# abmoRobotics/isaac_rover_orbit

Measured on NVIDIA B200. Metric: height_scan_rays_per_s, higher is better.
Workload: dtype f32

## Files before the change

include/rover_b200.h:

```cpp
#ifndef ROVER_B200_H
#define ROVER_B200_H

#include <stdint.h>

#ifdef __cplusplus
extern "C" {
#endif

#define ROVER_B200_ABI_VERSION 5
#define ROVER_MAX_LEVELS 12
#define ROVER_NUM_REWARD_TERMS 7
#define ROVER_NUM_TERMINATION_TERMS 4
#define ROVER_STATS_LEN 16

int rover_abi_version(void);
const char* rover_last_error(void);

typedef struct RoverScanLevel {
    float ox, oy;
    float cell;
    float inv_cell;
    int32_t ncx, ncy;
    int32_t start_offset;
    int32_t reserved;
} RoverScanLevel;

typedef struct RoverScanGrid {
    int32_t n_levels;
    int32_t span;
    RoverScanLevel level[ROVER_MAX_LEVELS];
    const int32_t* cell_start;
    const float* records;
    int32_t n_records;
    int32_t reserved;
} RoverScanGrid;

typedef struct RoverPlaneCells {
    const float* xs;
    const float* ys;
    const float* entries;
    int32_t nx, ny;
    float inv_dx, inv_dy;
    const float* entries_planar;
} RoverPlaneCells;

int rover_height_scan(const float* pos_w, const float* quat_w, int32_t n_envs, const float* ray_starts_local,
                      int32_t n_rays, const float* pattern_box , const RoverScanGrid* grid ,
                      const RoverPlaneCells* cells , float max_distance, float base_offset,
                      float* out_heights, int32_t out_stride, float* out_hits_w, int32_t variant, void* stream);

int rover_ray_cast(const float* pos_w, const float* quat_w, int32_t n_envs, const float* ray_starts_local,
                   const float* ray_dirs_local, int32_t n_rays, int32_t attach_yaw_only, const RoverScanGrid* grid ,
                   const RoverPlaneCells* cells , float max_distance, float base_offset, float* out_heights,
                   int32_t out_stride, float* out_hits_w, void* stream);

int64_t rover_height_scan_host_work_bytes(int32_t n_envs, int32_t out_stride);
int rover_height_scan_host(const float* pos_host, const float* quat_host, int32_t n_envs, const float* ray_starts_local,
                           int32_t n_rays, const float* pattern_box, const RoverScanGrid* grid, const RoverPlaneCells* cells,
                           float max_distance, float base_offset, float* out_host, int32_t out_stride, void* work,
                           int64_t work_bytes, int32_t n_slices, int32_t variant, void* stream);
int rover_height_scan_obs(const float* pos_w, const float* quat_w, int32_t n_envs, const float* ray_starts_local,
                          int32_t n_rays, const float* pattern_box , const RoverScanGrid* grid ,
                          const RoverPlaneCells* cells , float max_distance, float base_offset, float* obs,
                          int32_t obs_stride, int32_t head_cols, uint16_t* obs_bf16, int32_t bf16_stride, void* stream);
int rover_height_scan_obs_bf16(const float* pos_w, const float* quat_w, int32_t n_envs, const float* ray_starts_local,
                               int32_t n_rays, const float* pattern_box , const RoverScanGrid* grid,
                               const RoverPlaneCells* cells, float max_distance, float base_offset, const float* obs_head,
                               int32_t obs_stride, int32_t head_cols, uint16_t* obs_bf16, int32_t bf16_stride, void* stream);

int rover_ray_cast_obs(const float* pos_w, const float* quat_w, int32_t n_envs, const float* ray_starts_local,
                       const float* ray_dirs_local, int32_t n_rays, int32_t attach_yaw_only, const RoverScanGrid* grid ,
                       const RoverPlaneCells* cells , float max_distance, float base_offset, float* obs,
                       int32_t obs_stride, int32_t head_cols, uint16_t* obs_bf16, int32_t bf16_stride, void* stream);
int rover_ray_cast_obs_bf16(const float* pos_w, const float* quat_w, int32_t n_envs, const float* ray_starts_local,
                            const float* ray_dirs_local, int32_t n_rays, int32_t attach_yaw_only,
                            const RoverScanGrid* grid , const RoverPlaneCells* cells , float max_distance,
                            float base_offset, const float* obs_head, int32_t obs_stride, int32_t head_cols,
                            uint16_t* obs_bf16, int32_t bf16_stride, void* stream);
int rover_ray_cast_host(const float* pos_host, const float* quat_host, int32_t n_envs, const float* ray_starts_local,
                        const float* ray_dirs_local, int32_t n_rays, int32_t attach_yaw_only, const RoverScanGrid* grid,
                        const RoverPlaneCells* cells, float max_distance, float base_offset, float* out_host,
                        int32_t out_stride, void* work, int64_t work_bytes, int32_t n_slices, void* stream);

typedef struct RoverMdpParams {
    float scale_lin, scale_ang, offset_lin, offset_ang;
    float wheelbase_length, middle_wheel_distance, rear_and_front_wheel_distance, wheel_radius;
    float min_radius;
    float wheel_diameter;
    float weight[ROVER_NUM_REWARD_TERMS];
    float reached_threshold, far_threshold;
    float step_dt;
    int32_t max_episode_length;
    float obs_distance_scale, obs_heading_scale;
    float target_distance, resampling_time, heading_lo, heading_hi, spawn_z_offset;
    int32_t num_bodies;
    int32_t action_variant;
    float episode_length_s;
} RoverMdpParams;

typedef struct RoverMdpState {
    float* action;
    float* prev_action;
    float* pos_cmd_w;
    float* heading_cmd_w;
    float* pos_cmd_b;
    float* heading_cmd_b;
    float* time_left;
    int64_t* command_counter;
    int64_t* episode_length_buf;
    float* episode_sums;
    float* env_origins;
    float* err_pos;
    float* err_heading;
} RoverMdpState;

typedef struct RoverMdpOut {
    float* processed_actions;
    float* joint_pos;
    float* joint_vel;
    float* reward;
    float* term_rewards;
    float* term_values;
    uint8_t* terminated;
    uint8_t* truncated;
    uint8_t* term_flags;
    uint8_t* reset_flags;
    int32_t* block_reset_counts;
} RoverMdpOut;

#define ROVER_MDP_BLOCK 64

#define ROVER_PRE_ACTIONS 1
#define ROVER_PRE_TERMS 2
#define ROVER_PRE_ALL 3
int rover_mdp_pre_step(const float* new_actions, const float* force_matrix_w, int32_t n_envs,
                       const RoverMdpParams* params , const RoverMdpState* state ,
                       const RoverMdpOut* out , int32_t phases, void* stream);

int rover_ackermann(const float* actions , int32_t n_envs, const RoverMdpParams* params ,
                    float* processed , float* joint_pos , float* joint_vel ,
                    void* stream);

typedef struct RoverTerrainTables {
    const float* heightmap;
    const uint8_t* safe_mask;
    int32_t height, width;
    float offset_x, offset_y;
    float resolution;
    const float* spawn_table;
    int32_t n_spawns;
    int32_t reserved;
} RoverTerrainTables;

#define ROVER_PHASE_SPAWN 1
#define ROVER_PHASE_MANAGERS 2
#define ROVER_PHASE_RESAMPLE 4
#define ROVER_PHASE_METRICS 8
#define ROVER_PHASE_TIME 16
#define ROVER_PHASE_COMMAND 32
#define ROVER_PHASE_OBS 64
#define ROVER_PHASE_ALL 127

int rover_mdp_post_step(float* root_pos_w, float* root_quat_w, int32_t n_envs, const RoverMdpParams* params,
                        const RoverMdpState* state, const RoverMdpOut* out, const RoverTerrainTables* tables,
                        const int64_t* spawn_perm, const float* yaw_u, const float* heading_u, const float* theta_u,
                        int32_t n_rounds, int64_t* out_spawn_index , float* stats,
                        float* scratch ,
                        float* obs, int32_t obs_stride, int32_t phases, void* stream);

typedef struct RoverResetVariates {
    const int64_t* spawn_perm;
    const float* yaw_u;
    const float* heading_u;
    const float* theta_u;
    int32_t n_rounds;
    int32_t reserved;
    uint64_t* rng_state;
} RoverResetVariates;

int rover_mdp_post_step_v3(float* root_pos_w, float* root_quat_w, int32_t n_envs, const RoverMdpParams* params,
                           const RoverMdpState* state, const RoverMdpOut* out, const RoverTerrainTables* tables,
                           const RoverResetVariates* variates , int64_t* out_spawn_index, float* stats,
                           float* scratch, float* log_out, float* obs, int32_t obs_stride, int32_t phases,
                           const struct RoverStatsExchange* xchg , void* stream);
int rover_rng_variates(uint64_t seed, uint64_t step, int32_t n_envs, int32_t n_rounds, int32_t n_spawns,
                       int64_t* spawn_by_env, float* yaw_u, float* heading_u, float* theta_u);
int rover_philox4x32_10(const uint32_t counter[4], const uint32_t key[2], uint32_t out[4]);

int rover_mdp_step(const float* new_actions, const float* force_matrix_w, float* root_pos_w, float* root_quat_w,
                   int32_t n_envs, const RoverMdpParams* params, const RoverMdpState* state, const RoverMdpOut* out,
                   const RoverTerrainTables* tables, const int64_t* spawn_perm, const float* yaw_u, const float* heading_u,
                   const float* theta_u, int32_t n_rounds, int64_t* out_spawn_index, float* stats, float* scratch,
                   uint64_t* lookback, float* obs, int32_t obs_stride, int32_t pre_phases, int32_t phases,
                   const struct RoverStatsExchange* xchg , void* stream);
int rover_mdp_step_v3(const float* new_actions, const float* force_matrix_w, float* root_pos_w, float* root_quat_w,
                      int32_t n_envs, const RoverMdpParams* params, const RoverMdpState* state, const RoverMdpOut* out,
// ... 86 lines not shown
```

isaac_rover_orbit_b200/_lib.py:

```python
from __future__ import annotations

import ctypes as C
import os

import torch

_HERE = os.path.dirname(os.path.abspath(__file__))
LIB_PATH = os.environ.get("ROVER_B200_LIB") or os.path.join(_HERE, "librover_b200.so")

MAX_LEVELS = 12
NUM_REWARD_TERMS = 7
NUM_TERMINATION_TERMS = 4
STATS_LEN = 16
MDP_BLOCK = 64
ABI_VERSION = 5

SYMBOLS = ("rover_abi_version", "rover_last_error", "rover_height_scan", "rover_height_scan_obs", "rover_mdp_pre_step",
           "rover_mdp_post_step", "rover_mdp_post_step_x", "rover_mdp_post_step_v3", "rover_mdp_step", "rover_mdp_step_v3",
           "rover_rng_variates", "rover_philox4x32_10", "rover_stats_read", "rover_p2p_alloc", "rover_p2p_free",
           "rover_p2p_export", "rover_p2p_open", "rover_p2p_close",
           "rover_ackermann",
           "rover_height_scan_host", "rover_height_scan_host_work_bytes", "rover_stats_publish", "rover_height_scan_obs_bf16", "rover_policy_pack", "rover_policy_forward", "rover_value_forward", "rover_policy_value_forward", "rover_policy_forward_bf16",
           "rover_value_forward_bf16", "rover_gaussian_act", "rover_mesh_to_heightmap", "rover_steep_mask",
           "rover_policy_pack_fused", "rover_scan_encoder_fused", "rover_policy_mlp_forward", "rover_morph_box",
           "rover_fill_holes", "rover_step_fused", "rover_ray_cast", "rover_ray_cast_obs", "rover_ray_cast_obs_bf16",
           "rover_ray_cast_host", "rover_ppo_gae", "rover_ppo_gae_work_bytes")


class ScanLevel(C.Structure):
    _fields_ = [("ox", C.c_float), ("oy", C.c_float), ("cell", C.c_float), ("inv_cell", C.c_float),
                ("ncx", C.c_int32), ("ncy", C.c_int32), ("start_offset", C.c_int32), ("reserved", C.c_int32)]


class ScanGrid(C.Structure):
    _fields_ = [("n_levels", C.c_int32), ("span", C.c_int32), ("level", ScanLevel * MAX_LEVELS),
                ("cell_start", C.c_void_p), ("records", C.c_void_p), ("n_records", C.c_int32),
                ("reserved", C.c_int32)]


class PlaneCells(C.Structure):
    _fields_ = [("xs", C.c_void_p), ("ys", C.c_void_p), ("entries", C.c_void_p), ("nx", C.c_int32), ("ny", C.c_int32),
                ("inv_dx", C.c_float), ("inv_dy", C.c_float), ("entries_planar", C.c_void_p)]


class StatsExchange(C.Structure):
    _fields_ = [("peer_mailbox", C.c_void_p), ("cumulative", C.c_void_p), ("sequence", C.c_void_p),
                ("rank", C.c_int32), ("world", C.c_int32)]


MAILBOX_SLOT_BYTES = 512


class MdpParams(C.Structure):
    _fields_ = [("scale_lin", C.c_float), ("scale_ang", C.c_float), ("offset_lin", C.c_float),
                ("offset_ang", C.c_float), ("wheelbase_length", C.c_float), ("middle_wheel_distance", C.c_float),
                ("rear_and_front_wheel_distance", C.c_float), ("wheel_radius", C.c_float), ("min_radius", C.c_float),
                ("wheel_diameter", C.c_float),
                ("weight", C.c_float * NUM_REWARD_TERMS), ("reached_threshold", C.c_float),
                ("far_threshold", C.c_float), ("step_dt", C.c_float), ("max_episode_length", C.c_int32),
                ("obs_distance_scale", C.c_float), ("obs_heading_scale", C.c_float), ("target_distance", C.c_float),
                ("resampling_time", C.c_float), ("heading_lo", C.c_float), ("heading_hi", C.c_float),
                ("spawn_z_offset", C.c_float), ("num_bodies", C.c_int32), ("action_variant", C.c_int32),
                ("episode_length_s", C.c_float)]


class ResetVariates(C.Structure):

    _fields_ = [("spawn_perm", C.c_void_p), ("yaw_u", C.c_void_p), ("heading_u", C.c_void_p), ("theta_u", C.c_void_p),
                ("n_rounds", C.c_int32), ("reserved", C.c_int32), ("rng_state", C.c_void_p)]


_STATE_FIELDS = ("action", "prev_action", "pos_cmd_w", "heading_cmd_w", "pos_cmd_b", "heading_cmd_b", "time_left",
                 "command_counter", "episode_length_buf", "episode_sums", "env_origins", "err_pos", "err_heading")
_OUT_FIELDS = ("processed_actions", "joint_pos", "joint_vel", "reward", "term_rewards", "term_values", "terminated",
               "truncated", "term_flags", "reset_flags", "block_reset_counts")

PHASE_SPAWN, PHASE_MANAGERS, PHASE_RESAMPLE, PHASE_METRICS, PHASE_TIME, PHASE_COMMAND, PHASE_OBS = 1, 2, 4, 8, 16, 32, 64
PHASE_ALL = 127
PRE_ACTIONS, PRE_TERMS, PRE_ALL = 1, 2, 3


class MdpState(C.Structure):
    _fields_ = [(n, C.c_void_p) for n in _STATE_FIELDS]


class MdpOut(C.Structure):
    _fields_ = [(n, C.c_void_p) for n in _OUT_FIELDS]


class TerrainTables(C.Structure):
    _fields_ = [("heightmap", C.c_void_p), ("safe_mask", C.c_void_p), ("height", C.c_int32), ("width", C.c_int32),
                ("offset_x", C.c_float), ("offset_y", C.c_float), ("resolution", C.c_float),
                ("spawn_table", C.c_void_p), ("n_spawns", C.c_int32), ("reserved", C.c_int32)]


class PolicyWeights(C.Structure):
    _fields_ = [("w", C.c_void_p * 6), ("b", C.c_void_p * 6), ("in_dim", C.c_int32 * 6), ("out_dim", C.c_int32 * 6)]


_lib = None


def load() -> C.CDLL:
    global _lib
    if _lib is not None:
        return _lib
    if not os.path.exists(LIB_PATH):
        raise RuntimeError(
            f"{LIB_PATH} is missing: run `python __graft_entry__.py` (nvcc, sm_100a). There is no CPU fallback.")
    lib = C.CDLL(LIB_PATH)
    missing = [s for s in SYMBOLS if not hasattr(lib, s)]
    if missing:
        raise RuntimeError(f"librover_b200.so does not export {missing}")
    lib.rover_abi_version.restype = C.c_int
    lib.rover_last_error.restype = C.c_char_p
    if lib.rover_abi_version() != ABI_VERSION:
        raise RuntimeError(f"librover_b200.so ABI {lib.rover_abi_version()} != expected {ABI_VERSION}")
    vp, i32, f32 = C.c_void_p, C.c_int32, C.c_float
    lib.rover_height_scan.restype = C.c_int
    lib.rover_height_scan.argtypes = [vp, vp, i32, vp, i32, C.POINTER(C.c_float * 4), C.POINTER(ScanGrid),
                                      C.POINTER(PlaneCells), f32, f32, vp, i32, vp, i32, vp]
    lib.rover_ray_cast.restype = C.c_int
    lib.rover_ray_cast.argtypes = [vp, vp, i32, vp, vp, i32, i32, C.POINTER(ScanGrid), C.POINTER(PlaneCells), f32, f32, vp,
                                   i32, vp, vp]
    for fn in (lib.rover_ray_cast_obs, lib.rover_ray_cast_obs_bf16):
        fn.restype = C.c_int
        fn.argtypes = [vp, vp, i32, vp, vp, i32, i32, C.POINTER(ScanGrid), C.POINTER(PlaneCells), f32, f32, vp, i32, i32, vp,
                       i32, vp]
    lib.rover_ray_cast_host.restype = C.c_int
    lib.rover_ray_cast_host.argtypes = [vp, vp, i32, vp, vp, i32, i32, C.POINTER(ScanGrid), C.POINTER(PlaneCells), f32, f32,
                                        vp, i32, vp, C.c_int64, i32, vp]
    lib.rover_mdp_pre_step.restype = C.c_int
    lib.rover_mdp_pre_step.argtypes = [vp, vp, i32, C.POINTER(MdpParams), C.POINTER(MdpState), C.POINTER(MdpOut), i32,
                                       vp]
    lib.rover_mdp_post_step.restype = C.c_int
    lib.rover_mdp_post_step.argtypes = [vp, vp, i32, C.POINTER(MdpParams), C.POINTER(MdpState), C.POINTER(MdpOut),
                                        C.POINTER(TerrainTables), vp, vp, vp, vp, i32, vp, vp, vp, vp, i32, i32, vp]
    lib.rover_mdp_post_step_x.restype = C.c_int
    lib.rover_mdp_post_step_x.argtypes = [vp, vp, i32, C.POINTER(MdpParams), C.POINTER(MdpState), C.POINTER(MdpOut),
                                          C.POINTER(TerrainTables), vp, vp, vp, vp, i32, vp, vp, vp, vp, i32, i32,
                                          C.POINTER(StatsExchange), vp]
    lib.rover_mdp_post_step_v3.restype = C.c_int
    lib.rover_mdp_post_step_v3.argtypes = [vp, vp, i32, C.POINTER(MdpParams), C.POINTER(MdpState), C.POINTER(MdpOut),
                                           C.POINTER(TerrainTables), C.POINTER(ResetVariates), vp, vp, vp, vp, vp, i32, i32,
                                           C.POINTER(StatsExchange), vp]
    lib.rover_mdp_step_v3.restype = C.c_int
    lib.rover_mdp_step_v3.argtypes = [vp, vp, vp, vp, i32, C.POINTER(MdpParams), C.POINTER(MdpState), C.POINTER(MdpOut),
                                      C.POINTER(TerrainTables), C.POINTER(ResetVariates), vp, vp, vp, vp, vp, vp, i32, i32,
                                      i32, C.POINTER(StatsExchange), vp]
    lib.rover_step_fused.restype = C.c_int
    lib.rover_step_fused.argtypes = [vp, vp, vp, vp, i32, C.POINTER(MdpParams), C.POINTER(MdpState), C.POINTER(MdpOut),
                                     C.POINTER(TerrainTables), vp, i32, vp, vp, vp, i32, vp, vp, i32, i32, i32,
                                     C.POINTER(StatsExchange), vp, i32, C.POINTER(C.c_float * 4), C.POINTER(ScanGrid),
                                     C.POINTER(PlaneCells), f32, f32, vp]
    lib.rover_rng_variates.restype = C.c_int
    lib.rover_rng_variates.argtypes = [C.c_uint64, C.c_uint64, i32, i32, i32, vp, vp, vp, vp]
    lib.rover_philox4x32_10.restype = C.c_int
    lib.rover_philox4x32_10.argtypes = [C.POINTER(C.c_uint32 * 4), C.POINTER(C.c_uint32 * 2), C.POINTER(C.c_uint32 * 4)]
    lib.rover_mdp_step.restype = C.c_int
    lib.rover_mdp_step.argtypes = [vp, vp, vp, vp, i32, C.POINTER(MdpParams), C.POINTER(MdpState), C.POINTER(MdpOut),
                                   C.POINTER(TerrainTables), vp, vp, vp, vp, i32, vp, vp, vp, vp, vp, i32, i32, i32,
                                   C.POINTER(StatsExchange), vp]
    lib.rover_mesh_to_heightmap.restype = C.c_int
    lib.rover_mesh_to_heightmap.argtypes = [vp, vp, i32, C.c_float, C.c_float, C.c_float, C.c_float, i32, i32, vp, vp, vp]
    lib.rover_steep_mask.restype = C.c_int
    lib.rover_steep_mask.argtypes = [vp, i32, i32, C.c_double, vp, vp]
    lib.rover_morph_box.restype = C.c_int
    lib.rover_morph_box.argtypes = [vp, i32, i32, i32, i32, vp, vp, vp]
    lib.rover_fill_holes.restype = C.c_int
    lib.rover_fill_holes.argtypes = [vp, i32, i32, vp, vp, vp, vp]
    lib.rover_stats_read.restype = C.c_int
    lib.rover_stats_read.argtypes = [vp, i32, vp, vp]
    lib.rover_p2p_alloc.restype = C.c_int
    lib.rover_p2p_alloc.argtypes = [C.POINTER(C.c_void_p), C.c_int64]
    lib.rover_p2p_export.restype = C.c_int
    lib.rover_p2p_export.argtypes = [vp, C.POINTER(C.c_uint8 * 64)]
    lib.rover_p2p_open.restype = C.c_int
    lib.rover_p2p_open.argtypes = [C.POINTER(C.c_uint8 * 64), C.POINTER(C.c_void_p)]
    for fn in (lib.rover_p2p_free, lib.rover_p2p_close):
        fn.restype = C.c_int
        fn.argtypes = [vp]
    lib.rover_ackermann.restype = C.c_int
    lib.rover_ackermann.argtypes = [vp, i32, C.POINTER(MdpParams), vp, vp, vp, vp]
    lib.rover_policy_pack.restype = C.c_int64
    lib.rover_policy_pack.argtypes = [C.POINTER(PolicyWeights), vp, vp]
    lib.rover_stats_publish.restype = C.c_int
    lib.rover_stats_publish.argtypes = [C.POINTER(StatsExchange), vp]
    lib.rover_height_scan_host_work_bytes.restype = C.c_int64
    lib.rover_height_scan_host_work_bytes.argtypes = [i32, i32]
    lib.rover_height_scan_host.restype = C.c_int
    lib.rover_height_scan_host.argtypes = [vp, vp, i32, vp, i32, C.POINTER(C.c_float * 4), C.POINTER(ScanGrid),
                                           C.POINTER(PlaneCells), f32, f32, vp, i32, vp, C.c_int64, i32, i32, vp]
    for fn in (lib.rover_height_scan_obs, lib.rover_height_scan_obs_bf16):
        fn.restype = C.c_int
        fn.argtypes = [vp, vp, i32, vp, i32, C.POINTER(C.c_float * 4), C.POINTER(ScanGrid), C.POINTER(PlaneCells), f32, f32, vp,
# ... 67 lines not shown
```

isaac_rover_orbit_b200/csrc/fused_scan_policy.cu:

```cuda
#include "policy_common.cuh"
#include "scan_paired.cuh"

namespace rover {

constexpr int kFuConsumerWarps = 12;
constexpr int kFuWarps = 20;
constexpr int kFuThreads = 32 * kFuWarps;
constexpr int kFuStages = 4, kFuFullBars = 8;
constexpr int kFuBatch = 16;
constexpr int kFuRays = 961, kFuChunks = 4;
constexpr int kFuK0 = 976;
constexpr int kFuObsBytes = (kFuK0 / 8) * kOperandLbo;
constexpr int kFuActBytes = (80 / 8) * kOperandLbo;
constexpr int kFuW0Cols = kFuK0 / 2;
constexpr int kFuAccCol = kFuW0Cols;
constexpr int kFuTmemCols = 512;
constexpr int kFuEncCols = 64;
constexpr int kFuBiasFloats = 80 + 64;
constexpr int kFuW0Bytes = kFuW0Cols * 128 * 4;
constexpr int kFuW1Bytes = 10 * 64 * 16, kFuW1Lbo = 64 * 16, kFuW1Slack = 1024;
constexpr int kFuW1Ofs = kFuW0Bytes, kFuBiasOfs = kFuW0Bytes + kFuW1Bytes;
constexpr int kFuPackedBytes = kFuBiasOfs + kFuBiasFloats * 4;
constexpr int kFuRegsLaunch = 96, kFuRegsConsumer = 120, kFuRegsUtil = 64, kFuRegsEpilogue = 56;
static_assert(128 * (3 * kFuRegsConsumer + kFuRegsUtil + kFuRegsEpilogue) <= kFuThreads * kFuRegsLaunch,
              "setmaxnreg: the re-balanced budgets must fit the pool the CTA was launched with");
static_assert(kFuFullBars == 2 * kFuStages && 8 * kFuChunks - kFuConsumerWarps > 4 * kFuChunks, "phase aliasing argument");

struct FuPackArgs {
    const float* w0;
    const float* b0;
    const float* w1;
    const float* b1;
    int in0, in1;
};

__global__ void fused_pack_kernel(const __grid_constant__ FuPackArgs a, unsigned char* __restrict__ packed) {
    const int tid = blockIdx.x * blockDim.x + threadIdx.x, nthr = gridDim.x * blockDim.x;
    uint32_t* w0t = reinterpret_cast<uint32_t*>(packed);
    for (int idx = tid; idx < kFuW0Cols * 128; idx += nthr) {
        const int j = idx >> 7, t = idx & 127;
        float v[2] = {0.f, 0.f};
#pragma unroll
        for (int h = 0; h < 2; ++h) {
            const int src_k = 2 * j + h - kEncInOffset;
            if (t < 80 && src_k >= 0 && src_k < kEncIn) v[h] = a.w0[(size_t)t * a.in0 + src_k];
        }
        w0t[idx] = pack_bf16(v[0], v[1]);
    }
    __nv_bfloat16* w1 = reinterpret_cast<__nv_bfloat16*>(packed + kFuW1Ofs);
    for (int idx = tid; idx < kFuW1Bytes / 2; idx += nthr) {
        const int jj = idx & 7, r = (idx >> 3) & 63, plane = idx >> 9;
        const int k = plane * 8 + jj;
        w1[idx] = __float2bfloat16_rn((r < 60 && k < 80) ? a.w1[(size_t)r * a.in1 + k] : 0.f);
    }
    float* bias = reinterpret_cast<float*>(packed + kFuBiasOfs);
    for (int n = tid; n < kFuBiasFloats; n += nthr) bias[n] = n < 80 ? a.b0[n] : (n - 80 < 60 ? a.b1[n - 80] : 0.f);
}

struct __align__(128) FuSmem {
    PairStage stage[kFuStages];
    float vx[kPairMaxRays], vy[kPairMaxRays];
    LinePair2 xpair[kPairMaxLines], ypair[kPairMaxLines];
    unsigned char obs[2][kFuObsBytes];
    unsigned char act[kFuActBytes];
    unsigned char w1[kFuW1Bytes + kFuW1Slack];
    float bias[kFuBiasFloats];
    unsigned long long full_bar[kFuFullBars], empty_bar[kFuStages];
    unsigned long long obs_full[2], obs_empty[2];
    unsigned long long w1_full, w0_ready, acc_full, act_ready, batch_done;
    uint32_t tmem_base;
    int next_chunk;
    float vz0;
    __nv_bfloat16 head[kFuBatch][4];
};
static_assert(sizeof(FuSmem) <= 227 * 1024, "FuSmem exceeds the shared memory of one SM");
__device__ __forceinline__ float sm_vz(const FuSmem& sm, int) { return sm.vz0; }

__device__ __forceinline__ void fu_arrive(unsigned long long* b) {
    asm volatile("mbarrier.arrive.shared::cta.b64 _, [%0];" ::"r"(sptr(b)) : "memory");
}
__device__ __forceinline__ void fu_epi_sync() { asm volatile("bar.sync 1, 128;" ::: "memory"); }
__device__ __forceinline__ void fu_wait_relaxed(unsigned long long* bar, uint32_t parity) {
    uint32_t done = 0;
    while (true) {
        asm volatile(
            "{\n\t.reg .pred p;\n\tmbarrier.try_wait.parity.shared::cta.b64 p, [%1], %2;\n\tselp.u32 %0, 1, 0, p;\n\t}"
            : "=r"(done)
            : "r"(sptr(bar)), "r"(parity)
            : "memory");
        if (done) break;
        __nanosleep(256);
    }
}
__device__ __forceinline__ void fu_tmem_ld16(uint32_t taddr, uint32_t (&r)[16]) {
    asm volatile(
        "tcgen05.ld.sync.aligned.32x32b.x16.b32 {%0, %1, %2, %3, %4, %5, %6, %7, %8, %9, %10, %11, %12, %13, %14, %15}, [%16];"
        : "=r"(r[0]), "=r"(r[1]), "=r"(r[2]), "=r"(r[3]), "=r"(r[4]), "=r"(r[5]), "=r"(r[6]), "=r"(r[7]), "=r"(r[8]),
          "=r"(r[9]), "=r"(r[10]), "=r"(r[11]), "=r"(r[12]), "=r"(r[13]), "=r"(r[14]), "=r"(r[15])
        : "r"(taddr));
    asm volatile("tcgen05.wait::ld.sync.aligned;" ::: "memory");
}
__device__ __forceinline__ void fu_tmem_st8(uint32_t taddr, const uint32_t (&r)[8]) {
    asm volatile("tcgen05.st.sync.aligned.32x32b.x8.b32 [%0], {%1, %2, %3, %4, %5, %6, %7, %8};" ::"r"(taddr), "r"(r[0]),
                 "r"(r[1]), "r"(r[2]), "r"(r[3]), "r"(r[4]), "r"(r[5]), "r"(r[6]), "r"(r[7])
                 : "memory");
}
__device__ __forceinline__ void umma_ts(uint32_t d_tmem, uint32_t a_tmem, uint64_t bdesc, uint32_t idesc, bool accumulate) {
    asm volatile(
        "{\n\t.reg .pred p;\n\tsetp.ne.b32 p, %4, 0;\n\t"
        "tcgen05.mma.cta_group::1.kind::f16 [%0], [%1], %2, %3, p;\n\t}" ::"r"(d_tmem),
        "r"(a_tmem), "l"(bdesc), "r"(idesc), "r"((uint32_t)accumulate)
        : "memory");
}
template <int kRegs>
__device__ __forceinline__ void reg_dec() {
    asm volatile("setmaxnreg.dec.sync.aligned.u32 %0;" ::"n"(kRegs));
}
template <int kRegs>
__device__ __forceinline__ void reg_inc() {
    asm volatile("setmaxnreg.inc.sync.aligned.u32 %0;" ::"n"(kRegs));
}
__device__ __forceinline__ unsigned char* operand_at(unsigned char* base, int e, int k) {
    return base + (k >> 3) * kOperandLbo + (e >> 3) * 128 + (e & 7) * 16 + (k & 7) * 2;
}

template <bool kWriteObs>
__global__ void __launch_bounds__(kFuThreads, 1)
fused_scan_encoder_kernel(const float* __restrict__ pos_w, const float* __restrict__ quat_w, int n_envs,
                          const float* __restrict__ ray_local, const __grid_constant__ ScanGridDev g,
                          const __grid_constant__ PlaneCellsDev pc, const __grid_constant__ CUtensorMap tmap,
                          float pattern_radius, float max_d, float base_offset, float* __restrict__ obs, int obs_stride,
                          const unsigned char* __restrict__ packed, __nv_bfloat16* __restrict__ enc) {
    extern __shared__ __align__(128) unsigned char smem_raw[];
    FuSmem& sm = *reinterpret_cast<FuSmem*>(smem_raw);
    const int warp = threadIdx.x >> 5, lane = threadIdx.x & 31;
    const int n_iter = (n_envs - (int)blockIdx.x + (int)gridDim.x - 1) / (int)gridDim.x;
    const int n_batches = (n_iter + kFuBatch - 1) / kFuBatch;
    const bool lines_in_smem = (pc.nx <= kPairMaxLines) && (pc.ny <= kPairMaxLines);
    constexpr int n_rays = kFuRays;

    ProducerEnv cur, nxt;
    if (warp == 0) {
        producer_load(cur, lane, n_iter, pos_w, quat_w);
        if (lane == 0) {
            asm volatile("prefetch.tensormap [%0];" ::"l"(reinterpret_cast<uint64_t>(&tmap)) : "memory");
            for (int s = 0; s < kFuFullBars; ++s) bar_init(&sm.full_bar[s], 2);
            for (int s = 0; s < kFuStages; ++s) bar_init(&sm.empty_bar[s], (uint32_t)kFuChunks);
            asm volatile("fence.mbarrier_init.release.cluster;" ::: "memory");
        }
        __syncwarp();
        producer_window(cur, pc, pattern_radius);
        if (lane < n_iter && lane < kFuStages) {
            bar_arrive_expect_tx(&sm.full_bar[lane], kPairStageBytes);
            tma_load_window_planar(sm.stage[lane].p, &tmap, cur.ic0, cur.jr0, &sm.full_bar[lane]);
        }
        producer_frame(cur);
    } else if (warp == 1) {
        if (lane == 0) {
            for (int i = 0; i < 2; ++i) {
                mb_init(&sm.obs_full[i], kFuBatch * kFuChunks);
                mb_init(&sm.obs_empty[i], 1);
            }
            mb_init(&sm.w1_full, 1);
            mb_init(&sm.w0_ready, 1);
            mb_init(&sm.acc_full, 1);
            mb_init(&sm.act_ready, 1);
            mb_init(&sm.batch_done, 1);
            sm.next_chunk = 0;
            sm.vz0 = __ldg(ray_local + 2);
            asm volatile("fence.mbarrier_init.release.cluster;" ::: "memory");
            mb_expect_tx(&sm.w1_full, kFuW1Bytes);
            bulk_g2s(sm.w1, packed + kFuW1Ofs, kFuW1Bytes, &sm.w1_full);
        }
        __syncwarp();
        asm volatile("tcgen05.alloc.cta_group::1.sync.aligned.shared::cta.b32 [%0], %1;" ::"r"(sptr(&sm.tmem_base)),
                     "r"((uint32_t)kFuTmemCols)
                     : "memory");
        asm volatile("tcgen05.relinquish_alloc_permit.cta_group::1.sync.aligned;" ::: "memory");
    } else if (warp >= 4) {
        constexpr int kFill = 32 * (kFuWarps - 4);
        constexpr int kPatLoads = (2 * kPairMaxRays + kFill - 1) / kFill;
        constexpr int kLineLoads = (kPairMaxLines + kFill - 1) / kFill;
        const int ct = threadIdx.x - 128;
        float* pat_flat = sm.vx;
        float pat[kPatLoads], xl[kLineLoads], xh[kLineLoads], yl[kLineLoads], yh[kLineLoads];
#pragma unroll
        for (int k = 0; k < kPatLoads; ++k) {
            const int i = ct + k * kFill;
            const int comp = i / kPairMaxRays, r = ray_of_slot(i - comp * kPairMaxRays);
            pat[k] = (i < 2 * kPairMaxRays && r < n_rays) ? __ldg(ray_local + 3 * r + comp) : 0.f;
        }
#pragma unroll
        for (int k = 0; k < kLineLoads; ++k) {
            const int i = ct + k * kFill;
            const bool okx = lines_in_smem && i < pc.nx, oky = lines_in_smem && i < pc.ny;
            xl[k] = okx ? __ldg(pc.xs + i) : 0.f;
            xh[k] = okx ? __ldg(pc.xs + i + 1) : 0.f;
            yl[k] = oky ? __ldg(pc.ys + i) : 0.f;
            yh[k] = oky ? __ldg(pc.ys + i + 1) : 0.f;
        }
#pragma unroll
        for (int k = 0; k < kPatLoads; ++k) {
            const int i = ct + k * kFill;
            if (i < 2 * kPairMaxRays) pat_flat[i] = pat[k];
        }
#pragma unroll
        for (int k = 0; k < kLineLoads; ++k) {
            const int i = ct + k * kFill;
            if (lines_in_smem && i < pc.nx) sm.xpair[i] = {xl[k], xh[k]};
            if (lines_in_smem && i < pc.ny) sm.ypair[i] = {yl[k], yh[k]};
        }
        uint4* z = reinterpret_cast<uint4*>(&sm.obs[0][0]);
        for (int i = ct; i < 2 * kFuObsBytes / 16; i += kFill) z[i] = make_uint4(0u, 0u, 0u, 0u);
        for (int i = ct; i < kFuBiasFloats; i += kFill)
            sm.bias[i] = __ldg(reinterpret_cast<const float*>(packed + kFuBiasOfs) + i);
        fence_async_smem();
    }
    tc_fence_before();
    __syncthreads();
    tc_fence_after();
    const uint32_t tmem = sm.tmem_base;

    if (warp < 4) {
        reg_dec<kFuRegsUtil>();
        if (warp == 0) {
            for (int base = 0; base < n_iter; base += 32) {
                if (base > 0) cur = nxt;
                producer_verdict(cur, sm, pc, pattern_radius, lines_in_smem);
                const int n_here = min(32, n_iter - base);
                for (int k = 0; k < n_here; ++k) {
                    if (k == kFuStages && base + 32 < n_iter) {
                        producer_load(nxt, base + 32 + lane, n_iter, pos_w, quat_w);
                        producer_window(nxt, pc, pattern_radius);
                        producer_frame(nxt);
                    }
                    if (lane == k) {
                        const int it = base + k;
                        const int s = it % kFuStages;
                        unsigned long long* full = &sm.full_bar[it % kFuFullBars];
                        PairStage& st = sm.stage[s];
                        if (it >= kFuStages) {
                            bar_wait(&sm.empty_bar[s], ((uint32_t)(it / kFuStages) & 1u) ^ 1u);
                            if (cur.ok) {
                                bar_arrive_expect_tx(full, kPairStageBytes);
                                tma_load_window_planar(st.p, &tmap, cur.ic0, cur.jr0, full);
                            } else {
                                bar_arrive(full);
                            }
                        }
                        st.hdr = {cur.cw, cur.sz, cur.px, cur.py, cur.pz, cur.ic0, cur.jr0, cur.ncols, cur.nrows,
                                  cur.ok ? 1 : 0, 0, 0};
                        bar_arrive(full);
                    }
                    __syncwarp();
                }
            }
        } else if (warp == 2 && lane == 0) {
            const uint32_t idesc = make_idesc(kFuBatch);
            const uint32_t acc = tmem + kFuAccCol;
            fu_wait_relaxed(&sm.w1_full, 0u);
            fu_wait_relaxed(&sm.w0_ready, 0u);
            tc_fence_after();
            for (int b = 0; b < n_batches; ++b) {
                const int buf = b & 1;
                if (b == n_batches - 1) {
                    const int missing = (n_batches * kFuBatch - n_iter) * kFuChunks;
                    for (int i = 0; i < missing; ++i) fu_arrive(&sm.obs_full[buf]);
                }
                if (b > 0) fu_wait_relaxed(&sm.batch_done, (uint32_t)(b - 1) & 1u);
                fu_wait_relaxed(&sm.obs_full[buf], (uint32_t)(b >> 1) & 1u);
                tc_fence_after();
                const uint32_t b0 = sptr(sm.obs[buf]);
                for (int ks = 0; ks < kFuK0 / 16; ++ks)
                    umma_ts(acc, tmem + ks * 8, make_desc(b0 + ks * 2 * kOperandLbo, kOperandLbo), idesc, ks != 0);
                umma_commit(&sm.acc_full);
                fu_wait_relaxed(&sm.act_ready, (uint32_t)b & 1u);
                tc_fence_after();
                const uint32_t a1 = sptr(sm.w1), b1 = sptr(sm.act);
                for (int j = 0; j < 80 / 16; ++j)
                    umma(acc, make_desc(a1 + j * 2 * kFuW1Lbo, kFuW1Lbo), make_desc(b1 + j * 2 * kOperandLbo, kOperandLbo), idesc,
                         j != 0);
                umma_commit(&sm.acc_full);
            }
        }
    } else if (warp < 4 + kFuConsumerWarps) {
        reg_inc<kFuRegsConsumer>();
        while (true) {
            int chunk_id = 0;
            if (lane == 0) chunk_id = atomicAdd(&sm.next_chunk, 1);
            chunk_id = __shfl_sync(0xffffffffu, chunk_id, 0);
            const int it = chunk_id / kFuChunks, c = chunk_id - it * kFuChunks;
            if (it >= n_iter) break;
            const int env = (int)blockIdx.x + it * (int)gridDim.x;
            const int s = it % kFuStages;
            const PairStage& st = sm.stage[s];
            const int batch = it / kFuBatch, slot = it - batch * kFuBatch, buf = batch & 1;
            if (batch >= 2) bar_wait(&sm.obs_empty[buf], (uint32_t)((batch >> 1) - 1) & 1u);
            bar_wait(&sm.full_bar[it % kFuFullBars], (uint32_t)(it / kFuFullBars) & 1u);
            const PairHeader h = st.hdr;
            float* __restrict__ obs_row = obs + (size_t)env * obs_stride;
            float* __restrict__ out_row = obs_row + kOperandHead;
            unsigned char* __restrict__ operand_row = sm.obs[buf] + (slot >> 3) * 128 + (slot & 7) * 16;
            const int r_begin = c * kPairChunk, r_end = min(r_begin + kPairChunk, n_rays);
            if (c == 0 && lane < kOperandHead)
                *reinterpret_cast<__nv_bfloat16*>(operand_row + lane * 2) = __float2bfloat16_rn(obs_row[lane]);
            if (h.mode == 1) {
                const float sz2 = __fmul_rn(h.sz, 2.f);
                const PairCtx cx = make_pair_ctx(h, sm, st, smem_raw, pc.inv_dx, pc.inv_dy, base_offset, max_d, sm.vz0,
                                                 n_envs >> 31);
                constexpr int kSink = kWriteObs ? kSinkOperandAndGlobal : kSinkOperand;
                for (int b0 = r_begin; b0 < r_end; b0 += kPairBatch) {
                    const int r = b0 + lane;
                    float* __restrict__ o = out_row + r;
                    unsigned defer;
                    if (b0 + kPairBatch <= n_rays) {
                        defer = resolve_pair<true, true, false, kSink>(smem_raw, sm, cx, b0 + 2 * lane, r, n_rays, o, nullptr,
                                                                       operand_row);
                        defer |= resolve_pair<true, true, false, kSink>(smem_raw, sm, cx, b0 + 64 + 2 * lane, r + 32, n_rays,
                                                                        o + 32, nullptr, operand_row) << 2;
                    } else {
                        defer = resolve_pair<false, true, false, kSink>(smem_raw, sm, cx, b0 + 2 * lane, r, n_rays, o, nullptr,
                                                                        operand_row);
                        defer |= resolve_pair<false, true, false, kSink>(smem_raw, sm, cx, b0 + 64 + 2 * lane, r + 32, n_rays,
                                                                         o + 32, nullptr, operand_row) << 2;
                    }
                    if (defer != 0u) {
                        for (int u = 0; u < 4; ++u) {
                            if (!((defer >> u) & 1u)) continue;
                            const int rr = r + (u >> 1) * 32 + (u & 1) * 64;
                            const int sl = b0 + (u >> 1) * 64 + 2 * lane + (u & 1);
                            const float vx = sm.vx[sl], vy = sm.vy[sl];
                            const float tx = -__fmul_rn(sz2, vy), ty = __fmul_rn(sz2, vx);
                            const float X = __fadd_rn(__fadd_rn(__fadd_rn(vx, __fmul_rn(h.cw, tx)), -__fmul_rn(h.sz, ty)), h.px);
                            const float Y = __fadd_rn(__fadd_rn(__fadd_rn(vy, __fmul_rn(h.cw, ty)), __fmul_rn(h.sz, tx)), h.py);
                            float hh;
                            pair_resolve_deferred_ray(&sm, &st, g, pc.inv_dx, pc.inv_dy, X, Y, __fadd_rn(sm.vz0, h.pz), h.pz,
                                                      max_d, base_offset, &hh, nullptr);
                            operand_store(operand_row, rr, hh);
                            if (kWriteObs) out_row[rr] = hh;
                        }
                    }
                }
            } else {
                pair_resolve_chunk_from_global(&sm, lane, r_begin, r_end, h, g, pc, max_d, base_offset, out_row, nullptr);
                __syncwarp();
                for (int r = r_begin + lane; r < r_end; r += 32) operand_store(operand_row, r, out_row[r]);
            }
            fence_async_smem();
            __syncwarp();
            if (lane == 0) {
                bar_arrive(&sm.empty_bar[s]);
                fu_arrive(&sm.obs_full[buf]);
            }
        }
    } else {
        reg_dec<kFuRegsEpilogue>();
        const int t = threadIdx.x - 32 * (4 + kFuConsumerWarps);
        const uint32_t t_lane = (uint32_t)((warp & 3) * 32) << 16;
        {
            const uint32_t* __restrict__ w0t = reinterpret_cast<const uint32_t*>(packed) + t;
            static_assert(kFuW0Cols % 8 == 0, "W0 is stored 8 columns at a time");
#pragma unroll 4
            for (int c0 = 0; c0 < kFuW0Cols; c0 += 8) {
                uint32_t r[8];
#pragma unroll
                for (int i = 0; i < 8; ++i) r[i] = __ldg(w0t + (size_t)(c0 + i) * 128);
                fu_tmem_st8(tmem + t_lane + c0, r);
            }
            asm volatile("tcgen05.wait::st.sync.aligned;" ::: "memory");
            tc_fence_before();
            fu_epi_sync();
            if (t == 0) fu_arrive(&sm.w0_ready);
        }
        const float bias0 = t < 80 ? sm.bias[t] : 0.f;
        const float bias1 = t < 60 ? sm.bias[80 + t] : 0.f;
        uint32_t acc_phase = 0;
        const uint32_t acc = tmem + t_lane + kFuAccCol;
        for (int b = 0; b < n_batches; ++b) {
            const int buf = b & 1;
            fu_wait_relaxed(&sm.acc_full, acc_phase);
            acc_phase ^= 1u;
            tc_fence_after();
            if (t >= 60 && t < 64) {
#pragma unroll
                for (int e = 0; e < kFuBatch; ++e)
                    sm.head[e][t - 60] = *reinterpret_cast<const __nv_bfloat16*>(operand_at(sm.obs[buf], e, t - 60));
            }
            {
                uint32_t r[16];
                fu_tmem_ld16(acc, r);
                if (t < 80) {
#pragma unroll
                    for (int e = 0; e < kFuBatch; ++e)
                        *reinterpret_cast<__nv_bfloat16*>(operand_at(sm.act, e, t)) =
                            __float2bfloat16_rn(leaky(__uint_as_float(r[e]) + bias0));
                }
            }
            tc_fence_before();
            fence_async_smem();
            fu_epi_sync();
            if (t == 0) {
                fu_arrive(&sm.obs_empty[buf]);
                fu_arrive(&sm.act_ready);
            }
            fu_wait_relaxed(&sm.acc_full, acc_phase);
            acc_phase ^= 1u;
            tc_fence_after();
            {
                uint32_t r[16];
                fu_tmem_ld16(acc, r);
                if (t < kFuEncCols) {
#pragma unroll
                    for (int e = 0; e < kFuBatch; ++e) {
                        const int it = b * kFuBatch + e;
                        if (it < n_iter) {
                            const size_t env = (size_t)blockIdx.x + (size_t)it * gridDim.x;
                            const __nv_bfloat16 v = t < 60 ? __float2bfloat16_rn(leaky(__uint_as_float(r[e]) + bias1))
                                                           : sm.head[e][t - 60];
                            enc[env * kFuEncCols + t] = v;
                        }
                    }
                }
            }
            tc_fence_before();
            fu_epi_sync();
            if (t == 0) fu_arrive(&sm.batch_done);
        }
    }

    tc_fence_before();
    __syncthreads();
    if (warp == 1) {
        asm volatile("tcgen05.dealloc.cta_group::1.sync.aligned.b32 %0, %1;" ::"r"(tmem), "r"((uint32_t)kFuTmemCols) : "memory");
    }
}

}

extern "C" int64_t rover_policy_pack_fused(const RoverPolicyWeights* weights, void* packed, void* stream) {
    using namespace rover;
    if (packed == nullptr) return kFuPackedBytes;
    if (weights == nullptr) {
        fail("rover_policy_pack_fused: weights is NULL");
        return -1;
    }
    for (int l = 0; l < 2; ++l) {
        if (!weights->w[l] || !weights->b[l] || weights->in_dim[l] < layer_k_real(l) || weights->out_dim[l] != layer_n_real(l)) {
            fail("rover_policy_pack_fused: layer %d has shape [%d,%d], expected [%d,%d]", l, weights->out_dim[l],
                 weights->in_dim[l], layer_n_real(l), layer_k_real(l));
            return -1;
        }
    }
    FuPackArgs a{weights->w[0], weights->b[0], weights->w[1], weights->b[1], weights->in_dim[0], weights->in_dim[1]};
    fused_pack_kernel<<<64, 256, 0, static_cast<cudaStream_t>(stream)>>>(a, static_cast<unsigned char*>(packed));
    return check_launch("fused_pack_kernel") ? -1 : kFuPackedBytes;
}

extern "C" int rover_scan_encoder_fused(const float* pos_w, const float* quat_w, int32_t n_envs,
                                        const float* ray_starts_local, int32_t n_rays, const float* pattern_box,
                                        const RoverScanGrid* grid, const RoverPlaneCells* cells, float max_distance,
                                        float base_offset, float* obs, int32_t obs_stride, int32_t write_obs,
                                        const void* packed_fused, uint16_t* enc_bf16, void* stream) {
    using namespace rover;
    ROVER_CHECK(n_envs >= 0, "rover_scan_encoder_fused: negative n_envs");
    if (n_envs == 0) return 0;
    ROVER_CHECK(pos_w && quat_w && ray_starts_local && pattern_box && grid && cells && obs && packed_fused && enc_bf16,
                "rover_scan_encoder_fused: NULL argument");
    ROVER_CHECK(n_rays == kFuRays, "rover_scan_encoder_fused: the encoder reads a 961-ray scan (31 x 31 grid), got %d rays", n_rays);
    ROVER_CHECK(obs_stride >= kOperandHead + kFuRays, "rover_scan_encoder_fused: obs_stride %d < 965", obs_stride);
    ROVER_CHECK(cells->xs && cells->ys && cells->entries && cells->entries_planar && cells->nx > 0 && cells->ny > 0,
                "rover_scan_encoder_fused: needs the plane-cell table with its planar copy");
    ROVER_CHECK((reinterpret_cast<uintptr_t>(packed_fused) & 15) == 0, "rover_scan_encoder_fused: packed image not 16B aligned");
    static int n_sms = 0;
    if (n_sms == 0) {
        int dev = 0;
        ROVER_CUDA(cudaGetDevice(&dev));
        ROVER_CUDA(cudaDeviceGetAttribute(&n_sms, cudaDevAttrMultiProcessorCount, dev));
        ROVER_CUDA(cudaFuncSetAttribute(fused_scan_encoder_kernel<false>, cudaFuncAttributeMaxDynamicSharedMemorySize,
                                        (int)sizeof(FuSmem)));
        ROVER_CUDA(cudaFuncSetAttribute(fused_scan_encoder_kernel<true>, cudaFuncAttributeMaxDynamicSharedMemorySize,
                                        (int)sizeof(FuSmem)));
    }
    ScanGridDev g;
    g.n_levels = grid->n_levels;
    g.span = grid->span;
    ROVER_CHECK(grid->n_levels >= 0 && grid->n_levels <= ROVER_MAX_LEVELS, "rover_scan_encoder_fused: bad grid");
    for (int l = 0; l < grid->n_levels; ++l) {
        const RoverScanLevel& L = grid->level[l];
        g.level[l] = ScanLevelDev{L.ox, L.oy, L.cell, L.inv_cell, L.ncx, L.ncy, L.start_offset, 0};
    }
    g.cell_start = grid->cell_start;
    g.rec = reinterpret_cast<const float4*>(grid->records);
    alignas(64) CUtensorMap tmap;
    if (const int rc = encode_planar_tensor_map(&tmap, cells, kPairPitch, kPairWin, "rover_scan_encoder_fused")) return rc;
    PlaneCellsDev pc{cells->xs, cells->ys, reinterpret_cast<const float4*>(cells->entries), cells->nx, cells->ny,
                     cells->inv_dx, cells->inv_dy};
    const float rx = fmaxf(fabsf(pattern_box[0]), fabsf(pattern_box[1])), ry = fmaxf(fabsf(pattern_box[2]), fabsf(pattern_box[3]));
    const float radius = sqrtf(rx * rx + ry * ry) * 1.0001f + 1.0e-3f;
    const int grid_dim = n_envs < n_sms ? n_envs : n_sms;
    cudaStream_t s = static_cast<cudaStream_t>(stream);
    __nv_bfloat16* enc = reinterpret_cast<__nv_bfloat16*>(enc_bf16);
    if (write_obs)
        fused_scan_encoder_kernel<true><<<grid_dim, kFuThreads, sizeof(FuSmem), s>>>(
            pos_w, quat_w, n_envs, ray_starts_local, g, pc, tmap, radius, max_distance, base_offset, obs, obs_stride,
            static_cast<const unsigned char*>(packed_fused), enc);
    else
        fused_scan_encoder_kernel<false><<<grid_dim, kFuThreads, sizeof(FuSmem), s>>>(
            pos_w, quat_w, n_envs, ray_starts_local, g, pc, tmap, radius, max_distance, base_offset, obs, obs_stride,
            static_cast<const unsigned char*>(packed_fused), enc);
    return check_launch("fused_scan_encoder_kernel");
}
```

isaac_rover_orbit_b200/csrc/height_scan.cu:

```cuda
#include <cuda_bf16.h>

#include "scan_common.cuh"

namespace rover {

__device__ __forceinline__ float cast_down(const ScanGridDev& g, float X, float Y, float Z, float max_d) {
    float best = -INFINITY;
    for (int l = 0; l < g.n_levels; ++l) {
        const ScanLevelDev& L = g.level[l];
        const int i = cell_of(X, L.ox, L.inv_cell);
        const int j = cell_of(Y, L.oy, L.inv_cell);
        const int j0 = max(j - g.span, 0), j1 = min(j, L.ncy - 1);
        const int i0 = max(i - g.span, 0), i1 = min(i, L.ncx - 1);
        for (int jj = j0; jj <= j1; ++jj) {
            const float ly = __fsub_rn(Y, __fadd_rn(L.oy, __fmul_rn((float)jj, L.cell)));
            const int* __restrict__ row = g.cell_start + L.start_offset + jj * L.ncx;
            for (int ii = i0; ii <= i1; ++ii) {
                const float lx = __fsub_rn(X, __fadd_rn(L.ox, __fmul_rn((float)ii, L.cell)));
                const int b = __ldg(row + ii), e = __ldg(row + ii + 1);
                for (int r = b; r < e; ++r) {
                    const float4 r0 = __ldg(g.rec + 3 * r);
                    const float4 r1 = __ldg(g.rec + 3 * r + 1);
                    const float4 r2 = __ldg(g.rec + 3 * r + 2);
                    test_record(r0, r1, r2, lx, ly, Z, max_d, best);
// ... 135 lines not shown
        const size_t e = k / cols;
        const int c = (int)(k - e * cols);
        dst[e * dst_stride + c] = __float2bfloat16_rn(obs[e * obs_stride + c]);
    }
}

}

extern "C" int rover_height_scan(const float* pos_w, const float* quat_w, int32_t n_envs,
                                 const float* ray_starts_local, int32_t n_rays, const float* pattern_box,
                                 const RoverScanGrid* grid, const RoverPlaneCells* cells, float max_distance,
                                 float base_offset, float* out_heights, int32_t out_stride, float* out_hits_w,
                                 int32_t variant, void* stream) {
    using namespace rover;
    ROVER_CHECK(n_envs >= 0 && n_rays >= 0, "rover_height_scan: negative sizes");
    if (n_envs == 0 || n_rays == 0) return 0;
    ROVER_CHECK(pos_w && quat_w && ray_starts_local && out_heights, "rover_height_scan: NULL tensor");
    ROVER_CHECK(out_stride >= n_rays, "rover_height_scan: out_stride %d < n_rays %d", out_stride, n_rays);
    ScanGridDev g;
    if (int rc = make_dev_grid(grid, g)) return rc;
    cudaStream_t s = static_cast<cudaStream_t>(stream);
    if (variant == 0) {
        height_scan_direct_kernel<<<n_envs, kScanThreads, 0, s>>>(pos_w, quat_w, ray_starts_local, n_rays, g,
                                                                   max_distance, base_offset, out_heights, out_stride,
                                                                   out_hits_w);
        return check_launch("height_scan_direct_kernel");
    }
    ROVER_CHECK(variant != 1 && variant != 3, "rover_height_scan: variant %d was retired (use 0, 2, 4 or 5)", variant);
    if (variant == 2 || variant == 4 || variant == 5) {
        ROVER_CHECK(cells != nullptr, "rover_height_scan: variants 2, 4, 5 need the plane-cell table");
        ROVER_CHECK(cells->xs && cells->ys && cells->entries && cells->nx > 0 && cells->ny > 0,
                    "rover_height_scan: bad plane-cell table");
        ROVER_CHECK((reinterpret_cast<uintptr_t>(cells->entries) & 15) == 0,
                    "rover_height_scan: plane-cell entries not 16B aligned");
        if (variant == 5 && n_rays <= 1024) {
            ROVER_CHECK(pattern_box != nullptr, "rover_height_scan: variant 5 needs pattern_box (host, 4 floats)");
            const float4 box = make_float4(pattern_box[0], pattern_box[1], pattern_box[2], pattern_box[3]);
            return launch_height_scan_paired(pos_w, quat_w, n_envs, ray_starts_local, n_rays, g, cells, box,
                                             max_distance, base_offset, out_heights, out_stride, out_hits_w, nullptr, 0, 0, s);
        }
        if (variant >= 4 && n_rays <= 1024) {
            ROVER_CHECK(pattern_box != nullptr, "rover_height_scan: variant 4 needs pattern_box (host, 4 floats)");
            const float4 box = make_float4(pattern_box[0], pattern_box[1], pattern_box[2], pattern_box[3]);
            return launch_height_scan_pipelined(pos_w, quat_w, n_envs, ray_starts_local, n_rays, g, cells, box,
                                                max_distance, base_offset, out_heights, out_stride, out_hits_w, s);
        }
        PlaneCellsDev pc{cells->xs, cells->ys, reinterpret_cast<const float4*>(cells->entries), cells->nx, cells->ny,
                         cells->inv_dx, cells->inv_dy};
        height_scan_cells_kernel<<<n_envs, kScanThreads, 0, s>>>(pos_w, quat_w, ray_starts_local, n_rays, g, pc,
                                                                  max_distance, base_offset, out_heights, out_stride,
                                                                  out_hits_w);
        return check_launch("height_scan_cells_kernel");
    }
    return fail("rover_height_scan: unknown variant %d", variant);
}

namespace rover {
struct HostScanStreams {
    cudaStream_t copy = nullptr;
    cudaEvent_t scanned[64] = {};
    cudaEvent_t done = nullptr;
    int device = -1;
};
static inline int64_t host_scan_pose_bytes(int64_t n_envs) { return ((7 * n_envs * 4 + 65535) / 65536) * 65536; }

static int host_scan_streams(HostScanStreams*& out) {
    static HostScanStreams per_device[64];
    int dev = 0;
    ROVER_CUDA(cudaGetDevice(&dev));
    ROVER_CHECK(dev >= 0 && dev < 64, "rover_height_scan_host: device ordinal %d out of range", dev);
    HostScanStreams& h = per_device[dev];
    if (h.device != dev) {
        ROVER_CUDA(cudaStreamCreateWithFlags(&h.copy, cudaStreamNonBlocking));
        for (auto& e : h.scanned) ROVER_CUDA(cudaEventCreateWithFlags(&e, cudaEventDisableTiming));
        ROVER_CUDA(cudaEventCreateWithFlags(&h.done, cudaEventDisableTiming));
        h.device = dev;
    }
    out = &h;
    return 0;
}
}

int rover::host_scan_sliced(const char* what, const float* pos_host, const float* quat_host, int n_envs, int n_rays,
                            float* out_host, int out_stride, void* work, int64_t work_bytes, int n_slices, cudaStream_t s,
                            const HostSliceScan& scan) {
    ROVER_CHECK(n_envs >= 0 && n_rays >= 0, "%s: negative sizes", what);
    const int64_t need = rover_height_scan_host_work_bytes(n_envs, out_stride);
    if (n_envs == 0 || n_rays == 0) return 0;
    ROVER_CHECK(pos_host && quat_host && out_host && work, "%s: NULL buffer", what);
    ROVER_CHECK(out_stride >= n_rays, "%s: out_stride %d < n_rays %d", what, out_stride, n_rays);
    ROVER_CHECK(work_bytes >= need && (reinterpret_cast<uintptr_t>(work) & 255) == 0,
                "%s: work area of %lld bytes (256-byte aligned) needed, got %lld", what, (long long)need,
                (long long)work_bytes);
    ROVER_CHECK(n_slices >= 1 && n_slices <= 64, "%s: n_slices %d not in [1, 64]", what, n_slices);
    HostScanStreams* hs = nullptr;
    if (int rc = host_scan_streams(hs)) return rc;
    float* d_pos = static_cast<float*>(work);
    float* d_quat = d_pos + 3 * (size_t)n_envs;
    float* d_out = reinterpret_cast<float*>(static_cast<unsigned char*>(work) + host_scan_pose_bytes(n_envs));
    ROVER_CUDA(cudaMemcpyAsync(d_pos, pos_host, 12 * (size_t)n_envs, cudaMemcpyHostToDevice, s));
    ROVER_CUDA(cudaMemcpyAsync(d_quat, quat_host, 16 * (size_t)n_envs, cudaMemcpyHostToDevice, s));
    const int slices = n_slices < n_envs ? n_slices : n_envs;
    if (slices == 1) {
        if (int rc = scan(d_pos, d_quat, n_envs, d_out, s)) return rc;
        ROVER_CUDA(cudaMemcpyAsync(out_host, d_out, (size_t)n_envs * out_stride * 4, cudaMemcpyDeviceToHost, s));
        return 0;
    }
    for (int k = 0; k < slices; ++k) {
        const int e0 = (int)((int64_t)n_envs * k / slices), e1 = (int)((int64_t)n_envs * (k + 1) / slices);
        if (int rc = scan(d_pos + 3 * (size_t)e0, d_quat + 4 * (size_t)e0, e1 - e0, d_out + (size_t)e0 * out_stride, s))
            return rc;
        ROVER_CUDA(cudaEventRecord(hs->scanned[k], s));
        ROVER_CUDA(cudaStreamWaitEvent(hs->copy, hs->scanned[k], 0));
        ROVER_CUDA(cudaMemcpyAsync(out_host + (size_t)e0 * out_stride, d_out + (size_t)e0 * out_stride,
                                   (size_t)(e1 - e0) * out_stride * 4, cudaMemcpyDeviceToHost, hs->copy));
    }
    ROVER_CUDA(cudaEventRecord(hs->done, hs->copy));
    ROVER_CUDA(cudaStreamWaitEvent(s, hs->done, 0));
    return 0;
}

extern "C" int rover_height_scan_host(const float* pos_host, const float* quat_host, int32_t n_envs,
                                      const float* ray_starts_local, int32_t n_rays, const float* pattern_box,
                                      const RoverScanGrid* grid, const RoverPlaneCells* cells, float max_distance,
                                      float base_offset, float* out_host, int32_t out_stride, void* work, int64_t work_bytes,
                                      int32_t n_slices, int32_t variant, void* stream) {
    using namespace rover;
    return host_scan_sliced("rover_height_scan_host", pos_host, quat_host, n_envs, n_rays, out_host, out_stride, work,
                            work_bytes, n_slices, static_cast<cudaStream_t>(stream),
                            [&](const float* pos, const float* quat, int n, float* out, cudaStream_t s) {
                                return rover_height_scan(pos, quat, n, ray_starts_local, n_rays, pattern_box, grid, cells,
                                                         max_distance, base_offset, out, out_stride, nullptr, variant, s);
                            });
}

extern "C" int64_t rover_height_scan_host_work_bytes(int32_t n_envs, int32_t out_stride) {
    if (n_envs < 0 || out_stride < 0) return -1;
    return rover::host_scan_pose_bytes(n_envs) + (int64_t)n_envs * out_stride * 4;
}

static int height_scan_obs_impl(const float* pos_w, const float* quat_w, int32_t n_envs, const float* ray_starts_local,
                                int32_t n_rays, const float* pattern_box, const RoverScanGrid* grid,
                                const RoverPlaneCells* cells, float max_distance, float base_offset, float* obs,
                                int32_t obs_stride, int32_t head_cols, uint16_t* obs_bf16, int32_t bf16_stride, void* stream,
                                bool bf16_only) {
    using namespace rover;
    ROVER_CHECK(n_envs >= 0 && n_rays >= 0 && head_cols >= 0, "rover_height_scan_obs: negative sizes");
    if (n_envs == 0) return 0;
    ROVER_CHECK(obs && obs_bf16, "rover_height_scan_obs: NULL observation buffer");
    ROVER_CHECK(obs_stride >= head_cols + n_rays && bf16_stride >= head_cols + n_rays,
                "rover_height_scan_obs: row strides %d / %d < head_cols + n_rays = %d", obs_stride, bf16_stride,
                head_cols + n_rays);
    cudaStream_t s = static_cast<cudaStream_t>(stream);
    const bool fused = cells != nullptr && cells->entries_planar != nullptr && n_rays >= 1 && n_rays <= 1024 &&
                       head_cols <= 32 && pattern_box != nullptr;
    if (fused) {
        ROVER_CHECK(pos_w && quat_w && ray_starts_local, "rover_height_scan_obs: NULL tensor");
        ROVER_CHECK(cells->xs && cells->ys && cells->entries && cells->nx > 0 && cells->ny > 0,
                    "rover_height_scan_obs: bad plane-cell table");
        ScanGridDev g;
        if (int rc = make_dev_grid(grid, g)) return rc;
        const float4 box = make_float4(pattern_box[0], pattern_box[1], pattern_box[2], pattern_box[3]);
        return launch_height_scan_paired(pos_w, quat_w, n_envs, ray_starts_local, n_rays, g, cells, box, max_distance,
                                         base_offset, obs + head_cols, obs_stride, nullptr, obs_bf16, bf16_stride, head_cols,
                                         s, bf16_only);
    }
    const int variant = cells != nullptr ? 2 : 0;
    if (int rc = rover_height_scan(pos_w, quat_w, n_envs, ray_starts_local, n_rays, pattern_box, grid, cells, max_distance,
                                   base_offset, obs + head_cols, obs_stride, nullptr, variant, stream))
        return rc;
    obs_to_bf16_kernel<<<1184, 256, 0, s>>>(obs, obs_stride, n_envs, head_cols + n_rays,
                                            reinterpret_cast<__nv_bfloat16*>(obs_bf16), bf16_stride);
    return check_launch("obs_to_bf16_kernel");
}

extern "C" int rover_height_scan_obs(const float* pos_w, const float* quat_w, int32_t n_envs,
                                     const float* ray_starts_local, int32_t n_rays, const float* pattern_box,
                                     const RoverScanGrid* grid, const RoverPlaneCells* cells, float max_distance,
                                     float base_offset, float* obs, int32_t obs_stride, int32_t head_cols,
                                     uint16_t* obs_bf16, int32_t bf16_stride, void* stream) {
    return height_scan_obs_impl(pos_w, quat_w, n_envs, ray_starts_local, n_rays, pattern_box, grid, cells, max_distance,
                                base_offset, obs, obs_stride, head_cols, obs_bf16, bf16_stride, stream, false);
}

extern "C" int rover_height_scan_obs_bf16(const float* pos_w, const float* quat_w, int32_t n_envs,
                                          const float* ray_starts_local, int32_t n_rays, const float* pattern_box,
                                          const RoverScanGrid* grid, const RoverPlaneCells* cells, float max_distance,
                                          float base_offset, const float* obs_head, int32_t obs_stride, int32_t head_cols,
                                          uint16_t* obs_bf16, int32_t bf16_stride, void* stream) {
    return height_scan_obs_impl(pos_w, quat_w, n_envs, ray_starts_local, n_rays, pattern_box, grid, cells, max_distance,
                                base_offset, const_cast<float*>(obs_head), obs_stride, head_cols, obs_bf16, bf16_stride,
                                stream, true);
}
```

isaac_rover_orbit_b200/csrc/height_scan_paired.cu:

```cuda
#include "scan_paired.cuh"

#ifndef ROVER_PAIR_CTX_FROM_PRODUCER
#define ROVER_PAIR_CTX_FROM_PRODUCER 0
#endif
#ifndef ROVER_PAIR_DYNAMIC
#define ROVER_PAIR_DYNAMIC 0
#endif

namespace rover {

template <int kBf16>
__global__ void __launch_bounds__(kPairThreads, 1)
height_scan_paired_kernel(const float* __restrict__ pos_w, const float* __restrict__ quat_w, int n_envs,
                          const float* __restrict__ ray_local, int n_rays, const __grid_constant__ ScanGridDev g,
                          const __grid_constant__ PlaneCellsDev pc, const __grid_constant__ CUtensorMap tmap,
                          float pattern_radius, float max_d, float base_offset, float* __restrict__ out,
                          int out_stride, __nv_bfloat16* __restrict__ obs_bf16, int bf16_stride, int head_cols) {
    extern __shared__ __align__(128) unsigned char smem_raw[];
    PairSmem& sm = *reinterpret_cast<PairSmem*>(smem_raw);
    const int warp = threadIdx.x >> 5, lane = threadIdx.x & 31;
    const int n_iter = (n_envs - (int)blockIdx.x + (int)gridDim.x - 1) / (int)gridDim.x;
    const int n_chunks = (n_rays + kPairChunk - 1) / kPairChunk;
    const bool lines_in_smem = (pc.nx <= kPairMaxLines) && (pc.ny <= kPairMaxLines);
#if ROVER_SCAN_DBG == 3
    const long long dbg_t0 = clock64();
    if (threadIdx.x == 0 && blockIdx.x < 256) {
        g_scan_cta[0][blockIdx.x] = dbg_globaltimer();
        g_scan_cta[1][blockIdx.x] = 0;
    }
#endif

    ProducerEnv cur, nxt;
    int my_flat_z = 1;
    grid_dependency_trigger();
    if (warp == 0) {
        if (lane == 0) {
            asm volatile("prefetch.tensormap [%0];" ::"l"(reinterpret_cast<uint64_t>(&tmap)) : "memory");
            for (int s = 0; s < kPairFullBars; ++s) bar_init(&sm.full_bar[s], 2);
            for (int s = 0; s < kPairStages; ++s) bar_init(&sm.empty_bar[s], (uint32_t)n_chunks);
            sm.next_chunk = 0;
            asm volatile("fence.mbarrier_init.release.cluster;" ::: "memory");
        }
        grid_dependency_wait();
        producer_load(cur, lane, n_iter, pos_w, quat_w);
        __syncwarp();
        producer_window(cur, pc, pattern_radius);
        if (lane < n_iter && lane < kPairEarly && ROVER_SCAN_DBG != 4) {
            bar_arrive_expect_tx(&sm.full_bar[lane], kPairStageBytes);
            tma_load_window_planar(sm.stage[lane].p, &tmap, cur.ic0, cur.jr0, &sm.full_bar[lane]);
            DBG_STAMP_ANY(16 + lane);
        }
        producer_frame(cur);
        DBG_STAMP(1);
    } else {
        constexpr int kFill = 32 * kPairConsumerWarps;
        constexpr int kPatLoads = (3 * kPairMaxRays + kFill - 1) / kFill;
        constexpr int kLineLoads = (kPairMaxLines + kFill - 1) / kFill;
        const int ct = threadIdx.x - 32;
        static_assert(offsetof(PairSmem, vy) == offsetof(PairSmem, vx) + 4 * kPairMaxRays &&
                          offsetof(PairSmem, vz) == offsetof(PairSmem, vx) + 8 * kPairMaxRays,
                      "vx, vy, vz are filled as one array");
        float* pat_flat = sm.vx;
        float pat[kPatLoads], xl[kLineLoads], xh[kLineLoads], yl[kLineLoads], yh[kLineLoads];
        const float vz0 = __ldg(ray_local + 2);
#pragma unroll
        for (int k = 0; k < kPatLoads; ++k) {
            const int i = ct + k * kFill;
            const int comp = i / kPairMaxRays, r = ray_of_slot(i - comp * kPairMaxRays);
            pat[k] = (i < 3 * kPairMaxRays && r < n_rays) ? __ldg(ray_local + 3 * r + comp) : 0.f;
            if (comp == 2 && r < n_rays && pat[k] != vz0) my_flat_z = 0;
        }
#pragma unroll
        for (int k = 0; k < kLineLoads; ++k) {
            const int i = ct + k * kFill;
            const bool okx = lines_in_smem && i < pc.nx, oky = lines_in_smem && i < pc.ny;
            xl[k] = okx ? __ldg(pc.xs + i) : 0.f;
            xh[k] = okx ? __ldg(pc.xs + i + 1) : 0.f;
            yl[k] = oky ? __ldg(pc.ys + i) : 0.f;
            yh[k] = oky ? __ldg(pc.ys + i + 1) : 0.f;
        }
#pragma unroll
        for (int k = 0; k < kPatLoads; ++k) {
            const int i = ct + k * kFill;
            if (i < 3 * kPairMaxRays) pat_flat[i] = pat[k];
        }
#pragma unroll
        for (int k = 0; k < kLineLoads; ++k) {
            const int i = ct + k * kFill;
            if (lines_in_smem && i < pc.nx) sm.xpair[i] = {xl[k], xh[k]};
            if (lines_in_smem && i < pc.ny) sm.ypair[i] = {yl[k], yh[k]};
        }
    }
    if (warp == 1) DBG_STAMP(3);
    if (warp != 0) grid_dependency_wait();
    const bool flat_z = __syncthreads_and(my_flat_z) != 0;
    if (warp == 0) DBG_STAMP(0);

    if (warp == 0) {
        for (int base = 0; base < n_iter; base += 32) {
            if (base > 0) cur = nxt;
            producer_verdict(cur, sm, pc, pattern_radius, lines_in_smem);
            const int n_here = min(32, n_iter - base);
            for (int k = 0; k < n_here; ++k) {
                if (k == kPairStages && base + 32 < n_iter) {
                    producer_load(nxt, base + 32 + lane, n_iter, pos_w, quat_w);
                    producer_window(nxt, pc, pattern_radius);
                    producer_frame(nxt);
                }
                if (lane == k) {
                    const int it = base + k;
                    const int s = it % kPairStages;
                    unsigned long long* full = &sm.full_bar[it % kPairFullBars];
                    PairStage& st = sm.stage[s];
                    const bool first_pass = it < kPairEarly && ROVER_SCAN_DBG != 4;
                    if (!first_pass) {
                        bar_wait(&sm.empty_bar[s], ((uint32_t)(it / kPairStages) & 1u) ^ 1u);
                        if (cur.ok && ROVER_SCAN_DBG != 2) {
                            bar_arrive_expect_tx(full, kPairStageBytes);
                            tma_load_window_planar(st.p, &tmap, cur.ic0, cur.jr0, full);
                        } else {
                            bar_arrive(full);
                        }
                        DBG_STAMP_ANY(16 + it);
                    }
                    st.hdr = {cur.cw, cur.sz, cur.px, cur.py, cur.pz, cur.ic0, cur.jr0, cur.ncols, cur.nrows,
                              cur.ok ? 1 : 0, 0, 0};
#if ROVER_PAIR_CTX_FROM_PRODUCER
                    if (cur.ok)
                        st.ctx = make_pair_ctx(st.hdr, sm, st, smem_raw, pc.inv_dx, pc.inv_dy, base_offset, max_d, sm.vz[0],
                                               n_envs >> 31);
#endif
                    bar_arrive(full);
                }
                __syncwarp();
            }
        }
        DBG_STAMP(2);
    } else {
#if ROVER_PAIR_DYNAMIC
        int it = 0, c = 0;
        auto next_unit = [&]() {
            int k = 0;
            if (lane == 0) k = atomicAdd(&sm.next_chunk, 1);
            k = __shfl_sync(0xffffffffu, k, 0);
            it = k / n_chunks;
            c = k - it * n_chunks;
        };
        next_unit();
#else
        const int w = warp - 1;
        const int step_it = kPairConsumerWarps / n_chunks, step_c = kPairConsumerWarps % n_chunks;
        int it = w / n_chunks, c = w % n_chunks;
#endif
#if ROVER_SCAN_DBG == 3
        int dbg_j = 0;
#endif
        while (it < n_iter) {
            const int env = (int)blockIdx.x + it * (int)gridDim.x;
            const int s = it % kPairStages;
            const PairStage& st = sm.stage[s];
#if ROVER_SCAN_DBG == 3
            const int dbg_slot = (w == 0 ? 64 : w == 13 ? 128 : w == 6 ? 192 : 100000) + 4 * dbg_j;
            ++dbg_j;
#endif
            DBG_STAMP(dbg_slot);
            bar_wait(&sm.full_bar[it % kPairFullBars], (uint32_t)(it / kPairFullBars) & 1u);
            DBG_STAMP(dbg_slot + 1);
            const PairHeader h = st.hdr;
            float* __restrict__ out_row = out + (size_t)env * out_stride;
            __nv_bfloat16* __restrict__ bf_row = kBf16 ? obs_bf16 + (size_t)env * bf16_stride + head_cols : nullptr;
            const int r_begin = c * kPairChunk, r_end = min(r_begin + kPairChunk, n_rays);
            if (kBf16 && c == 0 && lane < head_cols)
                bf_row[lane - head_cols] = __float2bfloat16_rn(out_row[lane - head_cols]);
            if (ROVER_SCAN_DBG == 1) {
            } else if (h.mode == 1) {
#if ROVER_PAIR_CTX_FROM_PRODUCER
                const PairCtx cx = st.ctx;
#else
                const PairCtx cx = make_pair_ctx(h, sm, st, smem_raw, pc.inv_dx, pc.inv_dy, base_offset, max_d, sm.vz[0],
                                                 n_envs >> 31);
#endif
                const float sz2 = __fmul_rn(h.sz, 2.f);
                for (int b0 = r_begin; b0 < r_end; b0 += kPairBatch) {
                    const int r = b0 + lane;
                    float* __restrict__ o = out_row + r;
                    __nv_bfloat16* __restrict__ ob = kBf16 ? bf_row + r : nullptr;
                    unsigned defer;
                    if (flat_z && b0 + kPairBatch <= n_rays) {
                        defer = resolve_pair<true, true, kBf16>(smem_raw, sm, cx, b0 + 2 * lane, r, n_rays, o, ob);
                        defer |= resolve_pair<true, true, kBf16>(smem_raw, sm, cx, b0 + 64 + 2 * lane, r + 32, n_rays, o + 32,
                                                                 ob + 32) << 2;
                    } else {
                        defer = resolve_pair<false, false, kBf16>(smem_raw, sm, cx, b0 + 2 * lane, r, n_rays, o, ob);
                        defer |= resolve_pair<false, false, kBf16>(smem_raw, sm, cx, b0 + 64 + 2 * lane, r + 32, n_rays, o + 32,
                                                                   ob + 32) << 2;
                    }
                    if (defer != 0u) {
                        for (int u = 0; u < 4; ++u) {
                            if (!((defer >> u) & 1u)) continue;
                            const int rr = r + (u >> 1) * 32 + (u & 1) * 64;
                            const int sl = b0 + (u >> 1) * 64 + 2 * lane + (u & 1);
                            const float vx = sm.vx[sl], vy = sm.vy[sl];
                            const float tx = -__fmul_rn(sz2, vy), ty = __fmul_rn(sz2, vx);
                            const float X = __fadd_rn(__fadd_rn(__fadd_rn(vx, __fmul_rn(h.cw, tx)), -__fmul_rn(h.sz, ty)), h.px);
                            const float Y = __fadd_rn(__fadd_rn(__fadd_rn(vy, __fmul_rn(h.cw, ty)), __fmul_rn(h.sz, tx)), h.py);
                            pair_resolve_deferred_ray(&sm, &st, g, pc.inv_dx, pc.inv_dy, X, Y, __fadd_rn(sm.vz[sl], h.pz),
                                                      h.pz, max_d, base_offset, kBf16 == 2 ? nullptr : out_row + rr,
                                                      kBf16 ? bf_row + rr : nullptr);
                        }
                    }
                }
            } else {
                pair_resolve_chunk_from_global(&sm, lane, r_begin, r_end, h, g, pc, max_d, base_offset,
                                               kBf16 == 2 ? nullptr : out_row, bf_row);
            }
            __syncwarp();
            DBG_STAMP(dbg_slot + 2);
            if (lane == 0) bar_arrive(&sm.empty_bar[s]);
#if ROVER_PAIR_DYNAMIC
            next_unit();
#else
            it += step_it;
            c += step_c;
            if (c >= n_chunks) {
                c -= n_chunks;
                ++it;
            }
#endif
        }
    }
#if ROVER_SCAN_DBG == 3
    if (lane == 0 && blockIdx.x < 256) atomicMax(&g_scan_cta[1][blockIdx.x], dbg_globaltimer());
#endif
}

int launch_height_scan_pipelined(const float* pos_w, const float* quat_w, int n_envs, const float* ray_local,
                                 int n_rays, const ScanGridDev& g, const RoverPlaneCells* cells, float4 pattern_box,
                                 float max_d, float base_offset, float* out, int out_stride, float* hits,
                                 cudaStream_t stream);

int launch_height_scan_paired(const float* pos_w, const float* quat_w, int n_envs, const float* ray_local, int n_rays,
                              const ScanGridDev& g, const RoverPlaneCells* cells, float4 pattern_box, float max_d,
                              float base_offset, float* out, int out_stride, float* hits, uint16_t* obs_bf16,
                              int bf16_stride, int head_cols, cudaStream_t stream, bool bf16_only) {
    if (obs_bf16 == nullptr && (hits != nullptr || cells->entries_planar == nullptr))
        return launch_height_scan_pipelined(pos_w, quat_w, n_envs, ray_local, n_rays, g, cells, pattern_box, max_d,
                                            base_offset, out, out_stride, hits, stream);
    ROVER_CHECK(n_rays >= 1 && n_rays <= kPairMaxRays, "height_scan_paired: pattern of %d rays (1..%d supported)", n_rays,
                kPairMaxRays);
    ROVER_CHECK(cells->entries_planar != nullptr && hits == nullptr, "height_scan_paired: bf16 mirror needs the planar table");
    ROVER_CHECK(head_cols >= 0 && head_cols <= 32, "height_scan_paired: head_cols %d out of range", head_cols);
    static int n_sms = 0;
    static bool configured = false;
    if (!configured) {
        int dev = 0;
        ROVER_CUDA(cudaGetDevice(&dev));
        ROVER_CUDA(cudaDeviceGetAttribute(&n_sms, cudaDevAttrMultiProcessorCount, dev));
        ROVER_CUDA(cudaFuncSetAttribute(height_scan_paired_kernel<0>, cudaFuncAttributeMaxDynamicSharedMemorySize,
                                        (int)sizeof(PairSmem)));
        ROVER_CUDA(cudaFuncSetAttribute(height_scan_paired_kernel<1>, cudaFuncAttributeMaxDynamicSharedMemorySize,
                                        (int)sizeof(PairSmem)));
        ROVER_CUDA(cudaFuncSetAttribute(height_scan_paired_kernel<2>, cudaFuncAttributeMaxDynamicSharedMemorySize,
                                        (int)sizeof(PairSmem)));
        configured = true;
    }
    alignas(64) CUtensorMap tmap;
    if (const int rc = encode_planar_tensor_map(&tmap, cells, kPairPitch, kPairWin, "height_scan_paired")) return rc;
    PlaneCellsDev pc{cells->xs, cells->ys, reinterpret_cast<const float4*>(cells->entries), cells->nx, cells->ny,
                     cells->inv_dx, cells->inv_dy};
    const float rx = fmaxf(fabsf(pattern_box.x), fabsf(pattern_box.y)), ry = fmaxf(fabsf(pattern_box.z), fabsf(pattern_box.w));
    const float radius = sqrtf(rx * rx + ry * ry) * 1.0001f + 1.0e-3f;
    const int grid = n_envs < n_sms ? n_envs : n_sms;
    ROVER_CHECK(!bf16_only || obs_bf16 != nullptr, "height_scan_paired: bf16-only output needs the bf16 buffer");
    if (obs_bf16 != nullptr && bf16_only)
        ROVER_CUDA(launch_overlapped(height_scan_paired_kernel<2>, dim3(grid), dim3(kPairThreads), sizeof(PairSmem), stream,
                                     pos_w, quat_w, n_envs, ray_local, n_rays, g, pc, tmap, radius, max_d, base_offset, out,
                                     out_stride, reinterpret_cast<__nv_bfloat16*>(obs_bf16), bf16_stride, head_cols));
    else if (obs_bf16 != nullptr)
        ROVER_CUDA(launch_overlapped(height_scan_paired_kernel<1>, dim3(grid), dim3(kPairThreads), sizeof(PairSmem), stream,
                                     pos_w, quat_w, n_envs, ray_local, n_rays, g, pc, tmap, radius, max_d, base_offset, out,
                                     out_stride, reinterpret_cast<__nv_bfloat16*>(obs_bf16), bf16_stride, head_cols));
    else
        ROVER_CUDA(launch_overlapped(height_scan_paired_kernel<0>, dim3(grid), dim3(kPairThreads), sizeof(PairSmem), stream,
                                     pos_w, quat_w, n_envs, ray_local, n_rays, g, pc, tmap, radius, max_d, base_offset, out,
                                     out_stride, nullptr, 0, 0));
    return check_launch("height_scan_paired_kernel");
}

}

#if ROVER_SCAN_DBG == 3
extern "C" int rover_debug_scan_timeline(unsigned long long* host_dst) {
    return (int)cudaMemcpyFromSymbol(host_dst, rover::g_scan_dbg, sizeof(rover::g_scan_dbg));
}
extern "C" int rover_debug_scan_ctas(unsigned long long* host_dst) {
    return (int)cudaMemcpyFromSymbol(host_dst, rover::g_scan_cta, sizeof(rover::g_scan_cta));
}
#endif
```

isaac_rover_orbit_b200/csrc/height_scan_step.cu:

```cuda
#include "mdp_env.cuh"
#include "scan_paired.cuh"

namespace rover {

constexpr int kStepWorkerWarps = 15;
constexpr int kStepMdpWarps = 4;
constexpr int kStepThreads = 32 * (1 + kStepWorkerWarps);
constexpr int kStepLead = 96;
static_assert(kStepThreads == 512, "16 warps x 128 registers = the register file");
static_assert(kPairFullBars >= kStepWorkerWarps + kPairStages, "full barriers: phase-aliasing note in scan_paired.cuh");

struct StepSmem {
    PairStage stage[kPairStages];
    float vx[kPairMaxRays], vy[kPairMaxRays], vz[kPairMaxRays];
    LinePair2 xpair[kPairMaxLines], ypair[kPairMaxLines];
    unsigned long long full_bar[kPairFullBars];
    unsigned long long empty_bar[kPairStages];
    unsigned long long pose_full[kStepMdpWarps], pose_empty[kStepMdpWarps];
    float pose[kStepMdpWarps][32][8];
    float part[kStepMdpWarps][ROVER_STATS_LEN];
    int next_chunk;
    int mdp_done;
};
static_assert(sizeof(StepSmem) <= 227 * 1024, "StepSmem exceeds the shared memory of one SM");
__device__ __forceinline__ float sm_vz(const StepSmem& sm, int slot) { return sm.vz[slot]; }

struct PoseToScan {
    float* slot;
    unsigned long long* full;
    unsigned long long* empty;
    int wait_parity;
    __device__ __forceinline__ void operator()(float px, float py, float pz, const float4& q) const {
        if (wait_parity >= 0) bar_wait(empty, (uint32_t)wait_parity);
        slot[0] = px, slot[1] = py, slot[2] = pz;
        slot[3] = q.x, slot[4] = q.y, slot[5] = q.z, slot[6] = q.w;
        bar_arrive(full);
    }
};

__global__ void __launch_bounds__(kStepThreads, 1)
height_scan_step_kernel(const float* __restrict__ new_actions, const float* __restrict__ force,
                        float* __restrict__ root_pos_w, float* __restrict__ root_quat_w, int n_envs,
                        const __grid_constant__ RoverMdpParams P, const __grid_constant__ RoverMdpState S,
                        const __grid_constant__ RoverMdpOut O, const __grid_constant__ Tables T,
                        const __grid_constant__ VariatesDev V, long long* __restrict__ out_spawn_index,
                        float* __restrict__ cta_stats, unsigned int* __restrict__ done_counter, float* __restrict__ stats,
                        float* __restrict__ log_out, int pre_phases, int phases, const __grid_constant__ StatsExchangeDev X,
                        const float* __restrict__ ray_local, int n_rays, const __grid_constant__ ScanGridDev g,
                        const __grid_constant__ PlaneCellsDev pc, const __grid_constant__ CUtensorMap tmap,
                        float pattern_radius, float max_d, float base_offset, float* __restrict__ obs, int obs_stride) {
    extern __shared__ __align__(128) unsigned char smem_raw[];
    StepSmem& sm = *reinterpret_cast<StepSmem*>(smem_raw);
    const int warp = threadIdx.x >> 5, lane = threadIdx.x & 31;
    const int n_iter = (n_envs - (int)blockIdx.x + (int)gridDim.x - 1) / (int)gridDim.x;
    const int n_batches = (n_iter + 31) / 32;
    const int n_chunks = (n_rays + kPairChunk - 1) / kPairChunk;
    const bool lines_in_smem = (pc.nx <= kPairMaxLines) && (pc.ny <= kPairMaxLines);
    float* __restrict__ out = obs + 4;
    const int out_stride = obs_stride;

    int my_flat_z = 1;
    if (warp == 0) {
        if (lane == 0) {
            asm volatile("prefetch.tensormap [%0];" ::"l"(reinterpret_cast<uint64_t>(&tmap)) : "memory");
            for (int s = 0; s < kPairFullBars; ++s) bar_init(&sm.full_bar[s], 2);
            for (int s = 0; s < kPairStages; ++s) bar_init(&sm.empty_bar[s], (uint32_t)n_chunks);
            for (int s = 0; s < kStepMdpWarps; ++s) {
                bar_init(&sm.pose_full[s], 32);
                bar_init(&sm.pose_empty[s], 1);
            }
            sm.next_chunk = 0;
            sm.mdp_done = 0;
            asm volatile("fence.mbarrier_init.release.cluster;" ::: "memory");
        }
    } else {
        constexpr int kFill = 32 * kStepWorkerWarps;
        constexpr int kPatLoads = (3 * kPairMaxRays + kFill - 1) / kFill;
        constexpr int kLineLoads = (kPairMaxLines + kFill - 1) / kFill;
        const int ct = threadIdx.x - 32;
        float* pat_flat = sm.vx;
        float pat[kPatLoads], xl[kLineLoads], xh[kLineLoads], yl[kLineLoads], yh[kLineLoads];
        const float vz0 = __ldg(ray_local + 2);
#pragma unroll
        for (int k = 0; k < kPatLoads; ++k) {
            const int i = ct + k * kFill;
            const int comp = i / kPairMaxRays, r = ray_of_slot(i - comp * kPairMaxRays);
            pat[k] = (i < 3 * kPairMaxRays && r < n_rays) ? __ldg(ray_local + 3 * r + comp) : 0.f;
            if (comp == 2 && r < n_rays && pat[k] != vz0) my_flat_z = 0;
        }
#pragma unroll
        for (int k = 0; k < kLineLoads; ++k) {
            const int i = ct + k * kFill;
            const bool okx = lines_in_smem && i < pc.nx, oky = lines_in_smem && i < pc.ny;
            xl[k] = okx ? __ldg(pc.xs + i) : 0.f;
            xh[k] = okx ? __ldg(pc.xs + i + 1) : 0.f;
            yl[k] = oky ? __ldg(pc.ys + i) : 0.f;
            yh[k] = oky ? __ldg(pc.ys + i + 1) : 0.f;
        }
#pragma unroll
        for (int k = 0; k < kPatLoads; ++k) {
            const int i = ct + k * kFill;
            if (i < 3 * kPairMaxRays) pat_flat[i] = pat[k];
        }
#pragma unroll
        for (int k = 0; k < kLineLoads; ++k) {
            const int i = ct + k * kFill;
            if (lines_in_smem && i < pc.nx) sm.xpair[i] = {xl[k], xh[k]};
            if (lines_in_smem && i < pc.ny) sm.ypair[i] = {yl[k], yh[k]};
        }
    }
    const bool flat_z = __syncthreads_and(my_flat_z) != 0;

    if (warp == 0) {
        ProducerEnv cur;
        for (int b = 0; b < n_batches; ++b) {
            const int base = b * 32, pb = b % kStepMdpWarps;
            bar_wait(&sm.pose_full[pb], (uint32_t)(b / kStepMdpWarps) & 1u);
            {
                const float* row = &sm.pose[pb][lane][0];
                cur.have = base + lane < n_iter;
#pragma unroll
                for (int k = 0; k < 3; ++k) cur.pv[k] = cur.have ? row[k] : 0.f;
#pragma unroll
                for (int k = 0; k < 4; ++k) cur.qv[k] = cur.have ? row[3 + k] : (k == 0 ? 1.f : 0.f);
                cur.px = cur.pv[0], cur.py = cur.pv[1], cur.pz = cur.pv[2];
            }
            __syncwarp();
            if (lane == 0) bar_arrive(&sm.pose_empty[pb]);
            producer_window(cur, pc, pattern_radius);
            producer_frame(cur);
            producer_verdict(cur, sm, pc, pattern_radius, lines_in_smem);
            const int n_here = min(32, n_iter - base);
            for (int k = 0; k < n_here; ++k) {
                if (lane == k) {
                    const int it = base + k;
                    const int s = it % kPairStages;
                    unsigned long long* full = &sm.full_bar[it % kPairFullBars];
                    PairStage& st = sm.stage[s];
                    if (it >= kPairStages) bar_wait(&sm.empty_bar[s], ((uint32_t)(it / kPairStages) & 1u) ^ 1u);
                    if (cur.ok) {
                        bar_arrive_expect_tx(full, kPairStageBytes);
                        tma_load_window_planar(st.p, &tmap, cur.ic0, cur.jr0, full);
                    } else {
                        bar_arrive(full);
                    }
                    st.hdr = {cur.cw, cur.sz, cur.px, cur.py, cur.pz, cur.ic0, cur.jr0, cur.ncols, cur.nrows, cur.ok ? 1 : 0, 0, 0};
                    bar_arrive(full);
                }
                __syncwarp();
            }
        }
    } else {
        const int w = warp - 1;
        const bool mdp_warp = w < kStepMdpWarps;
        const int n_mdp_active = min(kStepMdpWarps, n_batches);
        int my_next = mdp_warp ? w : n_batches;
        RngKey key = make_rng_key(0ull, 0ull);
        if (mdp_warp) key = make_rng_key(V.rng[0], *reinterpret_cast<volatile unsigned long long*>(V.rng + 1));
        float acc = 0.f;
        bool have_chunk = false, draining = false;
        int it = 0, c = 0;
        while (true) {
            bool run_mdp = false;
            if (my_next < n_batches) {
                if (draining) run_mdp = true;
                else if (have_chunk) run_mdp = my_next <= it / 32 + 1;
                else run_mdp = my_next * 32 <= *reinterpret_cast<volatile int*>(&sm.next_chunk) / n_chunks + kStepLead;
            }
            if (run_mdp) {
                const int b = my_next;
                const int eit = b * 32 + lane;
                const bool valid = eit < n_iter;
                const int i = valid ? (int)blockIdx.x + eit * (int)gridDim.x : n_envs;
                if (valid) {
                    asm volatile("prefetch.global.L2 [%0];" ::"l"(root_pos_w + 3 * (size_t)i));
                    asm volatile("prefetch.global.L2 [%0];" ::"l"(root_quat_w + 4 * (size_t)i));
                    asm volatile("prefetch.global.L2 [%0];" ::"l"(S.pos_cmd_w + 3 * (size_t)i));
                }
                const bool reset = pre_step_env(i, new_actions, force, n_envs, P, S, O, pre_phases);
                EnvRegs er;
                post_env_load<true>(i, valid, root_pos_w, root_quat_w, S, V, er);
                float st[kStats];
                const int use = b / kStepMdpWarps;
                const PoseToScan hook{&sm.pose[w][lane][0], &sm.pose_full[w], &sm.pose_empty[w], use > 0 ? ((use - 1) & 1) : -1};
                if (!valid) hook(0.f, 0.f, 0.f, make_float4(1.f, 0.f, 0.f, 0.f));
                post_env_work<true>(i, valid, valid && reset, 0, er, root_pos_w, root_quat_w, P, S, O, T, V, key, out_spawn_index,
                                    obs, obs_stride, phases, st, hook);
#pragma unroll
                for (int k = 0; k < kStats; ++k) {
                    float v = st[k];
                    for (int o = 16; o > 0; o >>= 1) v += __shfl_down_sync(0xffffffffu, v, o);
                    v = __shfl_sync(0xffffffffu, v, 0);
                    if (lane == k) acc += v;
                }
                my_next += kStepMdpWarps;
                if (my_next >= n_batches) {
                    if (lane < kStats) sm.part[w][lane] = acc;
                    __threadfence_block();
                    __syncwarp();
                    int done = 0;
                    if (lane == 0) done = atomicAdd(&sm.mdp_done, 1);
                    done = __shfl_sync(0xffffffffu, done, 0);
                    if (done == n_mdp_active - 1) {
                        __threadfence_block();
                        float cta = 0.f;
                        if (lane < kStats)
                            for (int q = 0; q < n_mdp_active; ++q) cta += *reinterpret_cast<volatile float*>(&sm.part[q][lane]);
                        if (lane < kStats) cta_stats[(size_t)blockIdx.x * kStats + lane] = cta;
                        __threadfence();
                        __syncwarp();
                        unsigned ticket = 0;
                        if (lane == 0) ticket = atomicAdd(done_counter, 1u);
                        ticket = __shfl_sync(0xffffffffu, ticket, 0);
                        if (ticket == gridDim.x - 1u) {
                            __threadfence();
                            float t = 0.f;
                            if (lane < kStats)
                                for (unsigned cc = 0; cc < gridDim.x; ++cc) t += __ldcg(cta_stats + (size_t)cc * kStats + lane);
                            const float cnt = __shfl_sync(0xffffffffu, t, 13);
                            double total = 0.0;
                            if (lane < kStats) {
                                stats[lane] += t;
                                if (log_out != nullptr && (phases & ROVER_PHASE_MANAGERS) && cnt > 0.f) {
                                    float v = t;
                                    if (lane < ROVER_NUM_REWARD_TERMS) v = __fdiv_rn(__fdiv_rn(t, cnt), P.episode_length_s);
                                    else if (lane == 11 || lane == 12) v = __fdiv_rn(t, cnt);
                                    log_out[lane] = v;
                                }
                                if (X.world > 0) {
                                    total = X.cumulative[lane] + (double)t;
                                    X.cumulative[lane] = total;
                                }
                            }
                            if (lane == 0) {
                                *done_counter = 0u;
                                V.rng[1] = V.rng[1] + 1ull;
                            }
                            if (X.world > 0) {
                                const unsigned long long seq = *X.sequence + 1ull;
                                for (int e0 = 0; e0 < X.world * kStats; e0 += 32) {
                                    const int e = e0 + lane;
                                    const double v = __shfl_sync(0xffffffffu, total, e % kStats);
                                    if (e < X.world * kStats) {
                                        unsigned char* slot = static_cast<unsigned char*>(X.peer_mailbox[e / kStats]) +
                                                              (size_t)X.rank * ROVER_MAILBOX_SLOT_BYTES;
                                        reinterpret_cast<volatile double*>(slot + 8)[(seq & 1ull) * kStats + (e % kStats)] = v;
                                    }
                                }
                                __threadfence_system();
                                __syncwarp();
                                for (int p = lane; p < X.world; p += 32) {
                                    unsigned char* slot = static_cast<unsigned char*>(X.peer_mailbox[p]) + (size_t)X.rank * ROVER_MAILBOX_SLOT_BYTES;
                                    *reinterpret_cast<volatile unsigned long long*>(slot) = seq;
                                }
                                __syncwarp();
                                if (lane == 0) *X.sequence = seq;
                            }
                        }
                    }
                }
                continue;
            }
            if (draining) break;
            if (!have_chunk) {
                int k = 0;
                if (lane == 0) k = atomicAdd(&sm.next_chunk, 1);
                k = __shfl_sync(0xffffffffu, k, 0);
                it = k / n_chunks;
                c = k - it * n_chunks;
                if (it >= n_iter) {
                    draining = true;
                    continue;
                }
                have_chunk = true;
                continue;
            }
            have_chunk = false;
            const int env = (int)blockIdx.x + it * (int)gridDim.x;
            const int s = it % kPairStages;
            const PairStage& st = sm.stage[s];
            bar_wait(&sm.full_bar[it % kPairFullBars], (uint32_t)(it / kPairFullBars) & 1u);
            const PairHeader h = st.hdr;
            float* __restrict__ out_row = out + (size_t)env * out_stride;
            const int r_begin = c * kPairChunk, r_end = min(r_begin + kPairChunk, n_rays);
            if (h.mode == 1) {
                const float sz2 = __fmul_rn(h.sz, 2.f);
                const PairCtx cx = make_pair_ctx(h, sm, st, smem_raw, pc.inv_dx, pc.inv_dy, base_offset, max_d, sm.vz[0],
                                                 n_envs >> 31);
                for (int b0 = r_begin; b0 < r_end; b0 += kPairBatch) {
                    const int r = b0 + lane;
                    float* __restrict__ o = out_row + r;
                    unsigned defer;
                    if (flat_z && b0 + kPairBatch <= n_rays) {
                        defer = resolve_pair<true, true, false>(smem_raw, sm, cx, b0 + 2 * lane, r, n_rays, o, nullptr);
                        defer |= resolve_pair<true, true, false>(smem_raw, sm, cx, b0 + 64 + 2 * lane, r + 32, n_rays, o + 32, nullptr) << 2;
                    } else {
                        defer = resolve_pair<false, false, false>(smem_raw, sm, cx, b0 + 2 * lane, r, n_rays, o, nullptr);
                        defer |= resolve_pair<false, false, false>(smem_raw, sm, cx, b0 + 64 + 2 * lane, r + 32, n_rays, o + 32, nullptr) << 2;
                    }
                    if (defer != 0u) {
                        for (int u = 0; u < 4; ++u) {
                            if (!((defer >> u) & 1u)) continue;
                            const int rr = r + (u >> 1) * 32 + (u & 1) * 64;
                            const int sl = b0 + (u >> 1) * 64 + 2 * lane + (u & 1);
                            const float vx = sm.vx[sl], vy = sm.vy[sl];
                            const float tx = -__fmul_rn(sz2, vy), ty = __fmul_rn(sz2, vx);
                            const float X0 = __fadd_rn(__fadd_rn(__fadd_rn(vx, __fmul_rn(h.cw, tx)), -__fmul_rn(h.sz, ty)), h.px);
                            const float Y0 = __fadd_rn(__fadd_rn(__fadd_rn(vy, __fmul_rn(h.cw, ty)), __fmul_rn(h.sz, tx)), h.py);
                            pair_resolve_deferred_ray(&sm, &st, g, pc.inv_dx, pc.inv_dy, X0, Y0, __fadd_rn(sm.vz[sl], h.pz), h.pz,
                                                      max_d, base_offset, out_row + rr, nullptr);
                        }
                    }
                }
            } else {
                pair_resolve_chunk_from_global(&sm, lane, r_begin, r_end, h, g, pc, max_d, base_offset, out_row, nullptr);
            }
            __syncwarp();
            if (lane == 0) bar_arrive(&sm.empty_bar[s]);
        }
    }
}

int make_dev_grid(const RoverScanGrid* grid, ScanGridDev& g);

}

extern "C" int rover_step_fused(const float* new_actions, const float* force_matrix_w, float* root_pos_w, float* root_quat_w,
                                int32_t n_envs, const RoverMdpParams* params, const RoverMdpState* state,
                                const RoverMdpOut* out, const RoverTerrainTables* tables, uint64_t* rng_state,
                                int32_t n_rounds, int64_t* out_spawn_index, float* stats, float* scratch,
                                int32_t scratch_floats, float* log_out, float* obs, int32_t obs_stride, int32_t pre_phases,
                                int32_t phases, const RoverStatsExchange* xchg, const float* ray_starts_local, int32_t n_rays,
                                const float* pattern_box, const RoverScanGrid* grid, const RoverPlaneCells* cells,
                                float max_distance, float base_offset, void* stream) {
    using namespace rover;
    ROVER_CHECK(n_envs >= 0, "rover_step_fused: negative n_envs");
    if (n_envs == 0) return 0;
    ROVER_CHECK(params && state && out && tables && rng_state && stats && scratch && obs && root_pos_w && root_quat_w &&
                    ray_starts_local && pattern_box && grid && cells,
                "rover_step_fused: NULL argument");
    ROVER_CHECK((new_actions || !(pre_phases & ROVER_PRE_ACTIONS)) && (force_matrix_w || !(pre_phases & ROVER_PRE_TERMS)),
                "rover_step_fused: NULL actions / contact forces");
    ROVER_CHECK(params->num_bodies >= 0 && params->max_episode_length > 0 && n_rounds >= 1 && n_rounds <= 4096,
                "rover_step_fused: bad params");
    ROVER_CHECK(params->resampling_time > params->step_dt, "rover_step_fused: resampling_time must exceed step_dt");
    ROVER_CHECK(tables->heightmap && tables->safe_mask && tables->spawn_table && tables->height > 0 && tables->width > 0 &&
                    tables->n_spawns >= n_envs && tables->resolution > 0.f,
                "rover_step_fused: bad terrain tables (the spawn table needs >= n_envs rows)");
    ROVER_CHECK((reinterpret_cast<uintptr_t>(root_quat_w) & 15) == 0, "rover_step_fused: root_quat_w not 16B aligned");
    ROVER_CHECK(n_rays >= 1 && n_rays <= kPairMaxRays, "rover_step_fused: pattern of %d rays (1..%d supported)", n_rays, kPairMaxRays);
    ROVER_CHECK(obs_stride >= 4 + n_rays, "rover_step_fused: obs_stride %d < 4 + n_rays", obs_stride);
    ROVER_CHECK(cells->xs && cells->ys && cells->entries && cells->entries_planar && cells->nx > 0 && cells->ny > 0,
                "rover_step_fused: needs the plane-cell table with its planar copy");
    ROVER_CHECK(state->action && state->prev_action && state->pos_cmd_w && state->heading_cmd_w && state->pos_cmd_b &&
                    state->heading_cmd_b && state->time_left && state->command_counter && state->episode_length_buf &&
                    state->episode_sums && state->env_origins && state->err_pos && state->err_heading,
                "rover_step_fused: NULL pointer in RoverMdpState");
    ROVER_CHECK(out->processed_actions && out->joint_pos && out->joint_vel && out->reward && out->term_rewards &&
                    out->terminated && out->truncated && out->term_flags && out->reset_flags && out->term_values,
                "rover_step_fused: NULL pointer in RoverMdpOut");
    static int n_sms = 0;
    if (n_sms == 0) {
        int dev = 0;
        ROVER_CUDA(cudaGetDevice(&dev));
        ROVER_CUDA(cudaDeviceGetAttribute(&n_sms, cudaDevAttrMultiProcessorCount, dev));
        ROVER_CUDA(cudaFuncSetAttribute(height_scan_step_kernel, cudaFuncAttributeMaxDynamicSharedMemorySize, (int)sizeof(StepSmem)));
    }
    const int grid_dim = n_envs < n_sms ? n_envs : n_sms;
    ROVER_CHECK(scratch_floats >= grid_dim * ROVER_STATS_LEN + 1, "rover_step_fused: scratch needs %d floats", grid_dim * ROVER_STATS_LEN + 1);
    StatsExchangeDev X{nullptr, nullptr, nullptr, 0, 0};
    if (xchg != nullptr) {
        ROVER_CHECK(xchg->peer_mailbox && xchg->cumulative && xchg->sequence && xchg->world >= 1 && xchg->rank >= 0 &&
                        xchg->rank < xchg->world,
                    "rover_step_fused: bad RoverStatsExchange");
        X = StatsExchangeDev{xchg->peer_mailbox, xchg->cumulative, reinterpret_cast<unsigned long long*>(xchg->sequence),
                             xchg->rank, xchg->world};
    }
    Tables T{tables->heightmap, tables->safe_mask, tables->height,   tables->width,   tables->offset_x,
             tables->offset_y,  tables->resolution, tables->spawn_table, tables->n_spawns};
    VariatesDev V{nullptr, nullptr, nullptr, nullptr, reinterpret_cast<unsigned long long*>(rng_state), n_rounds};
    ScanGridDev g;
    if (int rc = make_dev_grid(grid, g)) return rc;
    alignas(64) CUtensorMap tmap;
    if (const int rc = encode_planar_tensor_map(&tmap, cells, kPairPitch, kPairWin, "rover_step_fused")) return rc;
    PlaneCellsDev pc{cells->xs, cells->ys, reinterpret_cast<const float4*>(cells->entries), cells->nx, cells->ny,
                     cells->inv_dx, cells->inv_dy};
    const float rx = fmaxf(fabsf(pattern_box[0]), fabsf(pattern_box[1])), ry = fmaxf(fabsf(pattern_box[2]), fabsf(pattern_box[3]));
    const float radius = sqrtf(rx * rx + ry * ry) * 1.0001f + 1.0e-3f;
    unsigned int* counter = reinterpret_cast<unsigned int*>(scratch + scratch_floats - 1);
    height_scan_step_kernel<<<grid_dim, kStepThreads, sizeof(StepSmem), static_cast<cudaStream_t>(stream)>>>(
        new_actions, force_matrix_w, root_pos_w, root_quat_w, n_envs, *params, *state, *out, T, V,
        reinterpret_cast<long long*>(out_spawn_index), scratch, counter, stats, log_out, pre_phases, phases, X,
        ray_starts_local, n_rays, g, pc, tmap, radius, max_distance, base_offset, obs, obs_stride);
    return check_launch("height_scan_step_kernel");
}
```

isaac_rover_orbit_b200/csrc/scan_common.cuh:

```cuda
#pragma once
#include <functional>

#include "common.cuh"

namespace rover {

struct ScanLevelDev {
    float ox, oy, cell, inv_cell;
    int ncx, ncy, start_offset, pad;
};

struct ScanGridDev {
    int n_levels;
    int span;
    ScanLevelDev level[ROVER_MAX_LEVELS];
    const int* __restrict__ cell_start;
    const float4* __restrict__ rec;
};

struct PlaneCellsDev {
    const float* __restrict__ xs;
    const float* __restrict__ ys;
    const float4* __restrict__ ent;
    int nx, ny;
    float inv_dx, inv_dy;
};

struct SensorFrame {
    float cw, sz;
    float px, py, pz;
};

__device__ __forceinline__ SensorFrame make_frame(const float* __restrict__ pos, const float* __restrict__ q) {
    const float w = q[0], x = q[1], y = q[2], z = q[3];
    const float siny = __fmul_rn(2.f, __fadd_rn(__fmul_rn(w, z), __fmul_rn(x, y)));
    const float cosy = __fsub_rn(1.f, __fmul_rn(2.f, __fadd_rn(__fmul_rn(y, y), __fmul_rn(z, z))));
    const float half = __fdiv_rn(atan2f(siny, cosy), 2.f);
    const float s = sinf(half), c = cosf(half);
    const float n = fmaxf(sqrtf(__fadd_rn(__fmul_rn(c, c), __fmul_rn(s, s))), 1e-9f);
    SensorFrame f;
    f.cw = __fdiv_rn(c, n);
    f.sz = __fdiv_rn(s, n);
    f.px = pos[0];
    f.py = pos[1];
    f.pz = pos[2];
    return f;
}

__device__ __forceinline__ void ray_origin(const SensorFrame& f, float vx, float vy, float vz, float& X, float& Y,
                                           float& Z) {
    const float tx = __fmul_rn(-__fmul_rn(f.sz, vy), 2.f);
    const float ty = __fmul_rn(__fmul_rn(f.sz, vx), 2.f);
    const float rx = __fadd_rn(__fadd_rn(vx, __fmul_rn(f.cw, tx)), -__fmul_rn(f.sz, ty));
    const float ry = __fadd_rn(__fadd_rn(vy, __fmul_rn(f.cw, ty)), __fmul_rn(f.sz, tx));
    X = __fadd_rn(rx, f.px);
    Y = __fadd_rn(ry, f.py);
    Z = __fadd_rn(vz, f.pz);
}

__device__ __forceinline__ int cell_of(float x, float o, float inv) {
    const float f = floorf(__fmul_rn(__fsub_rn(x, o), inv));
    return (int)fminf(fmaxf(f, -1.0e9f), 1.0e9f);
}

__device__ __forceinline__ void test_record(const float4 r0, const float4 r1, const float4 r2, float lx, float ly,
                                            float Z, float max_d, float& best) {
    const float e0 = fmaf(r0.x, lx, fmaf(r0.y, ly, r0.z));
    const float e1 = fmaf(r0.w, lx, fmaf(r1.x, ly, r1.y));
    const float e2 = fmaf(r1.z, lx, fmaf(r1.w, ly, r2.x));
    const float z = fmaf(r2.y, lx, fmaf(r2.z, ly, r2.w));
    const float t = Z - z;
    if (fminf(e0, fminf(e1, e2)) >= 0.f && t >= 0.f && t < max_d) best = fmaxf(best, z);
}

using HostSliceScan = std::function<int(const float* pos, const float* quat, int n_envs, float* out, cudaStream_t s)>;
int host_scan_sliced(const char* what, const float* pos_host, const float* quat_host, int n_envs, int n_rays,
                     float* out_host, int out_stride, void* work, int64_t work_bytes, int n_slices, cudaStream_t s,
                     const HostSliceScan& scan);

}
```

isaac_rover_orbit_b200/csrc/scan_paired.cuh:

```cuda
#pragma once
#include <cuda_bf16.h>

#include "scan_pipe.cuh"

#ifndef ROVER_SCAN_DBG
#define ROVER_SCAN_DBG 0
#endif

namespace rover {

#if ROVER_SCAN_DBG == 3
__device__ unsigned long long g_scan_dbg[2][512];
__device__ unsigned long long g_scan_cta[2][256];
__device__ __forceinline__ unsigned long long dbg_globaltimer() {
    unsigned long long t;
    asm volatile("mov.u64 %0, %globaltimer;" : "=l"(t));
    return t;
}
#define DBG_STAMP(slot)                                                                             \
    do {                                                                                            \
        if (lane == 0 && (blockIdx.x == 0 || blockIdx.x == 100) && (slot) < 512)                    \
            g_scan_dbg[blockIdx.x != 0][slot] = (unsigned long long)(clock64() - dbg_t0);           \
    } while (0)
#define DBG_STAMP_ANY(slot)                                                                         \
    do {                                                                                            \
        if ((blockIdx.x == 0 || blockIdx.x == 100) && (slot) < 512)                                 \
            g_scan_dbg[blockIdx.x != 0][slot] = (unsigned long long)(clock64() - dbg_t0);           \
    } while (0)
#else
#define DBG_STAMP(slot) \
    do {                \
    } while (0)
#define DBG_STAMP_ANY(slot) \
    do {                    \
    } while (0)
#endif

#ifndef ROVER_PAIR_WARPS
#define ROVER_PAIR_WARPS 15
#endif
constexpr int kPairConsumerWarps = ROVER_PAIR_WARPS;
constexpr int kPairThreads = 32 * (1 + kPairConsumerWarps);
constexpr int kPairStages = 8;
#ifndef ROVER_PAIR_EARLY
#define ROVER_PAIR_EARLY 8
#endif
constexpr int kPairEarly = ROVER_PAIR_EARLY;
constexpr int kPairFullBars = 32;
constexpr int kPairWin = 26;
constexpr int kPairPitch = 27;
constexpr int kPairPlane = kPairWin * kPairPitch;
constexpr uint32_t kPairStageBytes = 2u * kPairPlane * 16u;
#ifndef ROVER_PAIR_CHUNK
#define ROVER_PAIR_CHUNK 256
#endif
constexpr int kPairBatch = 128;
constexpr int kPairChunk = ROVER_PAIR_CHUNK;
static_assert(kPairChunk % kPairBatch == 0, "a chunk is a whole number of batches");
constexpr int kPairMaxRays = 1024;
constexpr int kPairMaxLines = 1024;
constexpr float kFloorMagic = 12582912.0f;
constexpr int kFloorMagicBits = 0x4B400000;

__host__ __device__ __forceinline__ int ray_of_slot(int s) {
    const int j = s & 127;
    return (s & ~127) + 64 * (j & 1) + 32 * (j >> 6) + ((j & 63) >> 1);
}
__host__ __device__ __forceinline__ int slot_of_ray(int r) {
    const int j = r & 127;
    return (r & ~127) + 64 * ((j >> 5) & 1) + 2 * (j & 31) + (j >> 6);
}

struct PairHeader {
    float cw, sz, px, py;
    float pz;
    int ic0, jr0, ncols;
    int nrows, mode, pad0, pad1;
};

typedef unsigned long long f32x2;

struct __align__(16) PairCtx {
    f32x2 CW, SZ, NSZ, S2, NS2, PX, PY, PZ, NWX0, NWY0, IDX, IDY, MAGIC, BASE, NEG0, ZFLAT;
    float pz, max_d;
    uint32_t xoff, yoff, eoff;
    uint32_t cmax, rmax;
    uint32_t pad;
};
static_assert(sizeof(PairCtx) == 160, "PairCtx is loaded as ten 16-byte words");

struct __align__(128) PairStage {
    float4 p[kPairPlane];
    float4 q[kPairPlane];
    PairHeader hdr;
    PairCtx ctx;
};
static_assert(offsetof(PairStage, q) == kPairPlane * 16, "planes must be contiguous: one 3-D TMA box fills both");

struct PairSmem {
    PairStage stage[kPairStages];
    float vx[kPairMaxRays], vy[kPairMaxRays], vz[kPairMaxRays];
    LinePair2 xpair[kPairMaxLines], ypair[kPairMaxLines];
    unsigned long long full_bar[kPairFullBars];
    unsigned long long empty_bar[kPairStages];
    int next_chunk;
};
static_assert(kPairFullBars >= kPairConsumerWarps + kPairStages, "full barriers: see the phase-aliasing note");

static_assert(sizeof(PairSmem) <= 227 * 1024, "PairSmem exceeds the shared memory of one SM");
__device__ __forceinline__ float sm_vz(const PairSmem& sm, int slot) { return sm.vz[slot]; }

constexpr int kSinkGlobal = 0, kSinkOperand = 1, kSinkOperandAndGlobal = 2;
constexpr int kOperandLbo = 272;
constexpr int kOperandHead = 4;
constexpr int kOperandDropK = 964;
__device__ __forceinline__ void operand_store(unsigned char* __restrict__ row, int ray, float h) {
    const int k = kOperandHead + ray;
    const __nv_bfloat16 v = __float2bfloat16_rn(k == kOperandDropK ? 0.f : h);
    *reinterpret_cast<__nv_bfloat16*>(row + (k >> 3) * kOperandLbo + (k & 7) * 2) = v;
}

__device__ __forceinline__ void tma_load_window_planar(void* dst, const CUtensorMap* tmap, int col, int row,
                                                       unsigned long long* bar) {
    asm volatile(
        "cp.async.bulk.tensor.3d.shared::cluster.global.tile.mbarrier::complete_tx::bytes [%0], [%1, {%2, %3, %4}], [%5];" ::
            "r"(s_addr(dst)),
        "l"(reinterpret_cast<uint64_t>(tmap)), "r"(col * 4), "r"(row), "r"(0), "r"(s_addr(bar))
        : "memory");
}

__device__ __forceinline__ f32x2 pk(float lo, float hi) {
    f32x2 r;
    asm("mov.b64 %0, {%1, %2};" : "=l"(r) : "f"(lo), "f"(hi));
    return r;
}
__device__ __forceinline__ f32x2 dup(float v) { return pk(v, v); }
__device__ __forceinline__ float lo_of(f32x2 v) {
    return __uint_as_float((unsigned)(v & 0xffffffffull));
}
__device__ __forceinline__ float hi_of(f32x2 v) {
    return __uint_as_float((unsigned)(v >> 32));
}
__device__ __forceinline__ f32x2 add2(f32x2 a, f32x2 b) {
    f32x2 r;
    asm("add.rn.f32x2 %0, %1, %2;" : "=l"(r) : "l"(a), "l"(b));
    return r;
}
__device__ __forceinline__ f32x2 sub2(f32x2 a, f32x2 b) {
    f32x2 r;
    asm("sub.rn.f32x2 %0, %1, %2;" : "=l"(r) : "l"(a), "l"(b));
    return r;
}
__device__ __forceinline__ f32x2 mul2(f32x2 a, f32x2 b) {
    f32x2 r;
    asm("mul.rn.f32x2 %0, %1, %2;" : "=l"(r) : "l"(a), "l"(b));
    return r;
}
__device__ __forceinline__ f32x2 mul2_unfused(f32x2 a, f32x2 b, f32x2 nz) {
    f32x2 r;
    asm("fma.rn.f32x2 %0, %1, %2, %3;" : "=l"(r) : "l"(a), "l"(b), "l"(nz));
    return r;
}
__device__ __forceinline__ f32x2 add2_rm(f32x2 a, f32x2 b) {
    f32x2 r;
    asm("add.rm.f32x2 %0, %1, %2;" : "=l"(r) : "l"(a), "l"(b));
    return r;
}

template <class SM>
__device__ __forceinline__ PairCtx make_pair_ctx(const PairHeader& h, const SM& sm, const PairStage& st,
                                                 const unsigned char* smem_base, float inv_dx, float inv_dy, float base_offset,
                                                 float max_d, float vz0, int opaque_zero) {
    PairCtx cx;
    const float sz2 = __fmul_rn(h.sz, 2.f);
    const float wx0 = sm.xpair[h.ic0].lo, wy0 = sm.ypair[h.jr0].lo;
    cx.CW = dup(h.cw), cx.SZ = dup(h.sz), cx.NSZ = dup(-h.sz), cx.S2 = dup(sz2), cx.NS2 = dup(-sz2);
    cx.PX = dup(h.px), cx.PY = dup(h.py), cx.PZ = dup(h.pz);
    cx.NWX0 = dup(-wx0), cx.NWY0 = dup(-wy0), cx.IDX = dup(inv_dx), cx.IDY = dup(inv_dy);
    cx.MAGIC = dup(kFloorMagic), cx.BASE = dup(base_offset);
    cx.NEG0 = dup(__uint_as_float(0x80000000u | (unsigned)opaque_zero));
    cx.pz = h.pz, cx.max_d = max_d;
    cx.ZFLAT = dup(__fadd_rn(vz0, h.pz));
    cx.cmax = (uint32_t)(h.ncols - 1), cx.rmax = (uint32_t)(h.nrows - 1);
    cx.xoff = (uint32_t)(reinterpret_cast<const unsigned char*>(sm.xpair + h.ic0) - smem_base);
    cx.yoff = (uint32_t)(reinterpret_cast<const unsigned char*>(sm.ypair + h.jr0) - smem_base);
    cx.eoff = (uint32_t)(reinterpret_cast<const unsigned char*>(st.p) - smem_base);
    cx.pad = 0u;
    return cx;
}

template <class SM>
static __device__ __noinline__ void pair_resolve_deferred_ray(const SM* sm, const PairStage* st, const ScanGridDev& g,
                                                              float inv_dx, float inv_dy, float X, float Y, float Z, float pz,
                                                              float max_d, float base_offset, float* __restrict__ out,
                                                              __nv_bfloat16* __restrict__ out_bf) {
    const PairHeader& h = st->hdr;
    const int cmax = h.ncols - 1, rmax = h.nrows - 1;
    const LinePair2* xp = sm->xpair + h.ic0;
    const LinePair2* yp = sm->ypair + h.jr0;
    const float wx0 = xp[0].lo, wy0 = yp[0].lo, wx1 = xp[cmax].hi, wy1 = yp[rmax].hi;
    float zhit = -INFINITY;
    if (X >= wx0 && X <= wx1 && Y >= wy0 && Y <= wy1) {
        int ci = min(max(__float2int_rd((X - wx0) * inv_dx), 0), cmax);
        int cj = min(max(__float2int_rd((Y - wy0) * inv_dy), 0), rmax);
        while (ci > 0 && X < xp[ci].lo) --ci;
        while (ci < cmax && X >= xp[ci].hi) ++ci;
        while (cj > 0 && Y < yp[cj].lo) --cj;
        while (cj < rmax && Y >= yp[cj].hi) ++cj;
        const int e = cj * kPairPitch + ci;
        const float4 q = st->q[e];
        zhit = (q.w == 0.f) ? eval_cell(st->p[e], q, __fsub_rn(X, xp[ci].lo), __fsub_rn(Y, yp[cj].lo), Z, max_d)
                            : walk_home_grid(g, X, Y, Z, max_d);
    }
    float height;
    store_result(pz, X, Y, Z, zhit, base_offset, &height, nullptr);
    if (out != nullptr) *out = height;
    if (out_bf != nullptr) *out_bf = __float2bfloat16_rn(height);
}

template <class SM>
static __device__ __noinline__ void pair_resolve_chunk_from_global(const SM* sm, int lane, int r_begin, int r_end,
                                                                   const PairHeader h, const ScanGridDev& g,
                                                                   const PlaneCellsDev& pc, float max_d, float base_offset,
                                                                   float* __restrict__ out_row,
                                                                   __nv_bfloat16* __restrict__ bf_row) {
    const float sz2 = __fmul_rn(h.sz, 2.f);
    for (int r = r_begin + lane; r < r_end; r += 32) {
        const int sl = slot_of_ray(r);
        const float vx = sm->vx[sl], vy = sm->vy[sl];
        const float tx = -__fmul_rn(sz2, vy), ty = __fmul_rn(sz2, vx);
        const float X = __fadd_rn(__fadd_rn(__fadd_rn(vx, __fmul_rn(h.cw, tx)), -__fmul_rn(h.sz, ty)), h.px);
        const float Y = __fadd_rn(__fadd_rn(__fadd_rn(vy, __fmul_rn(h.cw, ty)), __fmul_rn(h.sz, tx)), h.py);
        const float Z = __fadd_rn(sm_vz(*sm, sl), h.pz);
        float height;
        store_result(h.pz, X, Y, Z, resolve_from_global(g, pc, X, Y, Z, max_d), base_offset, &height, nullptr);
        if (out_row != nullptr) out_row[r] = height;
        if (bf_row != nullptr) bf_row[r] = __float2bfloat16_rn(height);
    }
}

template <bool kFull, bool kFlatZ, int kBf, int kSink = kSinkGlobal, class SM = PairSmem>
__device__ __forceinline__ unsigned resolve_pair(const unsigned char* __restrict__ smem, const SM& sm,
                                                 const PairCtx& c, int slot, int ray_a, int n_rays,
                                                 float* __restrict__ o, __nv_bfloat16* __restrict__ ob,
                                                 unsigned char* __restrict__ operand_row = nullptr) {
    const bool valid0 = kFull || ray_a < n_rays, valid1 = kFull || ray_a + 64 < n_rays;
    const int idx = slot;
    const f32x2 VX = *reinterpret_cast<const f32x2*>(sm.vx + idx);
    const f32x2 VY = *reinterpret_cast<const f32x2*>(sm.vy + idx);
    const f32x2 TX = mul2(c.NS2, VY), TY = mul2(c.S2, VX);
    const f32x2 X = add2(add2(add2(VX, mul2_unfused(c.CW, TX, c.NEG0)), mul2_unfused(c.NSZ, TY, c.NEG0)), c.PX);
    const f32x2 Y = add2(add2(add2(VY, mul2_unfused(c.CW, TY, c.NEG0)), mul2_unfused(c.SZ, TX, c.NEG0)), c.PY);
    f32x2 Z = c.ZFLAT;
    if constexpr (!kFlatZ) Z = add2(*reinterpret_cast<const f32x2*>(sm.vz + idx), c.PZ);
    const f32x2 BX = add2_rm(mul2(add2(X, c.NWX0), c.IDX), c.MAGIC);
    const f32x2 BY = add2_rm(mul2(add2(Y, c.NWY0), c.IDY), c.MAGIC);
    float nz[2];
    unsigned defer = 0;
    bool keep[2];
#pragma unroll
    for (int k = 0; k < 2; ++k) {
        const float x = k ? hi_of(X) : lo_of(X), y = k ? hi_of(Y) : lo_of(Y);
        const uint32_t bi = min(__float_as_uint(k ? hi_of(BX) : lo_of(BX)) - (uint32_t)kFloorMagicBits, c.cmax);
        const uint32_t bj = min(__float_as_uint(k ? hi_of(BY) : lo_of(BY)) - (uint32_t)kFloorMagicBits, c.rmax);
        const float2 xp = *reinterpret_cast<const float2*>(smem + (c.xoff + bi * 8u));
        const float2 yp = *reinterpret_cast<const float2*>(smem + (c.yoff + bj * 8u));
#if ROVER_SCAN_DBG == 5
        const uint32_t e = c.eoff + ((threadIdx.x & 31) * 16u) + ((bj + bi) & 1u) * 1024u;
        const float4 q = *reinterpret_cast<const float4*>(smem + e + 512);
        const float4 p = *reinterpret_cast<const float4*>(smem + e);
        const bool fast = (x >= xp.x) & (x < xp.y) & (y >= yp.x) & (y < yp.y);
#else
        const uint32_t e = c.eoff + bj * (uint32_t)(kPairPitch * 16) + bi * 16u;
        const float4 q = *reinterpret_cast<const float4*>(smem + e + kPairPlane * 16);
        const float4 p = *reinterpret_cast<const float4*>(smem + e);
        const bool fast = (x >= xp.x) & (x < xp.y) & (y >= yp.x) & (y < yp.y) & (q.w == 0.f);
#endif
        const float lx = __fsub_rn(x, xp.x), ly = __fsub_rn(y, yp.x);
        const float E = fmaf(q.x, lx, fmaf(q.y, ly, q.z));
        nz[k] = fmaf(-p.w, fminf(E, 0.f), -fmaf(p.x, lx, fmaf(p.y, ly, p.z)));
        const bool valid = k ? valid1 : valid0;
        keep[k] = valid && fast;
        defer |= (valid && !fast) ? (1u << k) : 0u;
    }
    const f32x2 T = add2(Z, pk(nz[0], nz[1]));
    const f32x2 H = sub2(sub2(c.PZ, sub2(Z, T)), c.BASE);
    const float t0 = lo_of(T), t1 = hi_of(T);
    const float h0 = (t0 >= 0.f && t0 < c.max_d) ? lo_of(H) : -INFINITY;
    const float h1 = (t1 >= 0.f && t1 < c.max_d) ? hi_of(H) : -INFINITY;
    if (kSink != kSinkOperand && kBf != 2) {
        if (keep[0]) o[0] = h0;
        if (keep[1]) o[64] = h1;
    }
    if (kBf) {
        if (keep[0]) ob[0] = __float2bfloat16_rn(h0);
        if (keep[1]) ob[64] = __float2bfloat16_rn(h1);
    }
    if (kSink != kSinkGlobal) {
        if (keep[0]) operand_store(operand_row, ray_a, h0);
        if (keep[1]) operand_store(operand_row, ray_a + 64, h1);
    }
    return defer;
}

struct ProducerEnv {
    float pv[3], qv[4];
    float cw, sz, px, py, pz;
    int ic0, jr0, ncols, nrows;
    bool have, ok;
};

__device__ __forceinline__ void producer_load(ProducerEnv& e, int it, int n_iter, const float* __restrict__ pos_w,
                                              const float* __restrict__ quat_w) {
    e.have = it < n_iter;
    const size_t env = (size_t)blockIdx.x + (size_t)(e.have ? it : 0) * gridDim.x;
#pragma unroll
    for (int k = 0; k < 3; ++k) e.pv[k] = __ldg(pos_w + 3 * env + k);
#pragma unroll
    for (int k = 0; k < 4; ++k) e.qv[k] = __ldg(quat_w + 4 * env + k);
    e.px = e.pv[0], e.py = e.pv[1], e.pz = e.pv[2];
}

__device__ __forceinline__ void producer_window(ProducerEnv& e, const PlaneCellsDev& pc, float radius) {
    const float gx_lo = __ldg(pc.xs), gy_lo = __ldg(pc.ys);
    const int ic1 = min(max(guess_col(e.px + radius, gx_lo, pc.inv_dx) + 1, 0), pc.nx - 1);
    const int jr1 = min(max(guess_col(e.py + radius, gy_lo, pc.inv_dy) + 1, 0), pc.ny - 1);
    e.ic0 = min(max(guess_col(e.px - radius, gx_lo, pc.inv_dx) - 1, 0), pc.nx - 1);
    e.jr0 = min(max(guess_col(e.py - radius, gy_lo, pc.inv_dy) - 1, 0), pc.ny - 1);
    e.ncols = ic1 - e.ic0 + 1;
    e.nrows = jr1 - e.jr0 + 1;
}

__device__ __forceinline__ void producer_frame(ProducerEnv& e) {
    const SensorFrame f = make_frame(e.pv, e.qv);
    e.cw = f.cw, e.sz = f.sz;
}

template <class SM>
__device__ __forceinline__ void producer_verdict(ProducerEnv& e, const SM& sm, const PlaneCellsDev& pc,
                                                 float radius, bool lines_in_smem) {
    bool ok = lines_in_smem && (e.ncols <= kPairWin) && (e.nrows <= kPairWin);
    if (ok) {
        const float gx_lo = sm.xpair[0].lo, gx_hi = sm.xpair[pc.nx - 1].hi;
        const float gy_lo = sm.ypair[0].lo, gy_hi = sm.ypair[pc.ny - 1].hi;
        ok = (sm.xpair[e.ic0].lo <= fmaxf(e.px - radius, gx_lo)) &&
             (sm.xpair[e.ic0 + e.ncols - 1].hi >= fminf(e.px + radius, gx_hi)) &&
             (sm.ypair[e.jr0].lo <= fmaxf(e.py - radius, gy_lo)) &&
             (sm.ypair[e.jr0 + e.nrows - 1].hi >= fminf(e.py + radius, gy_hi));
    }
    e.ok = ok;
}

}
```

isaac_rover_orbit_b200/csrc/scan_pipe.cuh:

```cuda
#pragma once
#include <cuda.h>

#include "scan_common.cuh"

namespace rover {

struct LinePair2 {
    float lo, hi;
};

struct StageHeader {
    float cw, sz, px, py, pz;
    int ncols, nrows;
    int mode;
};

__device__ __forceinline__ uint32_t s_addr(const void* p) { return (uint32_t)__cvta_generic_to_shared(p); }

__device__ __forceinline__ void bar_init(unsigned long long* bar, uint32_t count) {
    asm volatile("mbarrier.init.shared::cta.b64 [%0], %1;" ::"r"(s_addr(bar)), "r"(count) : "memory");
}
__device__ __forceinline__ void bar_arrive(unsigned long long* bar) {
    asm volatile("mbarrier.arrive.shared::cta.b64 _, [%0];" ::"r"(s_addr(bar)) : "memory");
}
__device__ __forceinline__ void bar_arrive_expect_tx(unsigned long long* bar, uint32_t bytes) {
    asm volatile("mbarrier.arrive.expect_tx.shared::cta.b64 _, [%0], %1;" ::"r"(s_addr(bar)), "r"(bytes) : "memory");
}
__device__ __forceinline__ void bar_wait(unsigned long long* bar, uint32_t parity) {
    uint32_t done = 0;
    while (!done) {
        asm volatile(
            "{\n\t.reg .pred p;\n\t"
            "mbarrier.try_wait.parity.shared::cta.b64 p, [%1], %2;\n\t"
            "selp.u32 %0, 1, 0, p;\n\t}"
            : "=r"(done)
            : "r"(s_addr(bar)), "r"(parity)
            : "memory");
    }
}
__device__ __forceinline__ void tma_load_window(void* dst, const CUtensorMap* tmap, int col, int row,
                                                unsigned long long* bar) {
    asm volatile(
        "cp.async.bulk.tensor.2d.shared::cluster.global.tile.mbarrier::complete_tx::bytes [%0], [%1, {%2, %3}], [%4];" ::
            "r"(s_addr(dst)),
        "l"(reinterpret_cast<uint64_t>(tmap)), "r"(col * 8), "r"(row), "r"(s_addr(bar))
        : "memory");
}

__device__ __forceinline__ int guess_col(float v, float lo, float inv_d) {
    return (int)fminf(fmaxf(floorf((v - lo) * inv_d), -1.0e6f), 1.0e6f);
}

__device__ __forceinline__ float eval_cell(const float4 p, const float4 q, float lx, float ly, float Z, float max_d) {
    const float E = fmaf(q.x, lx, fmaf(q.y, ly, q.z));
    const float z = fmaf(p.w, fminf(E, 0.f), fmaf(p.x, lx, fmaf(p.y, ly, p.z)));
    const float t = Z - z;
    return (t >= 0.f && t < max_d) ? z : -INFINITY;
}

__device__ __forceinline__ void store_result(float pz, float X, float Y, float Z, float zhit, float base_offset,
                                             float* __restrict__ out, float* __restrict__ hit3) {
    float h = -INFINITY, hx = INFINITY, hy = INFINITY, hz = INFINITY;
    if (zhit != -INFINITY) {
        const float t = __fsub_rn(Z, zhit);
        hz = __fsub_rn(Z, t);
        hx = X;
        hy = Y;
        h = __fsub_rn(__fsub_rn(pz, hz), base_offset);
    }
    *out = h;
    if (hit3) {
        hit3[0] = hx;
        hit3[1] = hy;
        hit3[2] = hz;
    }
}

static __device__ __noinline__ float walk_home_grid(const ScanGridDev& g, float X, float Y, float Z, float max_d) {
    float best = -INFINITY;
    for (int l = 0; l < g.n_levels; ++l) {
        const ScanLevelDev& L = g.level[l];
        const int i = cell_of(X, L.ox, L.inv_cell);
        const int j = cell_of(Y, L.oy, L.inv_cell);
        const int j0 = max(j - g.span, 0), j1 = min(j, L.ncy - 1);
        const int i0 = max(i - g.span, 0), i1 = min(i, L.ncx - 1);
        for (int jj = j0; jj <= j1; ++jj) {
            const float ly = __fsub_rn(Y, __fadd_rn(L.oy, __fmul_rn((float)jj, L.cell)));
            const int* __restrict__ row = g.cell_start + L.start_offset + jj * L.ncx;
            for (int ii = i0; ii <= i1; ++ii) {
                const float lx = __fsub_rn(X, __fadd_rn(L.ox, __fmul_rn((float)ii, L.cell)));
                const int b = __ldg(row + ii), e = __ldg(row + ii + 1);
                for (int r = b; r < e; ++r)
                    test_record(__ldg(g.rec + 3 * r), __ldg(g.rec + 3 * r + 1), __ldg(g.rec + 3 * r + 2), lx, ly, Z,
                                max_d, best);
            }
        }
    }
    return best;
}

static __device__ __noinline__ float resolve_from_global(const ScanGridDev& g, const PlaneCellsDev& pc, float X, float Y,
                                                   float Z, float max_d) {
    const float gx_lo = __ldg(pc.xs), gx_hi = __ldg(pc.xs + pc.nx), gy_lo = __ldg(pc.ys), gy_hi = __ldg(pc.ys + pc.ny);
    if (!((X >= gx_lo) && (X <= gx_hi) && (Y >= gy_lo) && (Y <= gy_hi))) return -INFINITY;
    int i = min(max(guess_col(X, gx_lo, pc.inv_dx), 0), pc.nx - 1);
    int j = min(max(guess_col(Y, gy_lo, pc.inv_dy), 0), pc.ny - 1);
    while (i > 0 && X < __ldg(pc.xs + i)) --i;
    while (i < pc.nx - 1 && X >= __ldg(pc.xs + i + 1)) ++i;
    while (j > 0 && Y < __ldg(pc.ys + j)) --j;
    while (j < pc.ny - 1 && Y >= __ldg(pc.ys + j + 1)) ++j;
    const float4* __restrict__ e = pc.ent + 2 * ((size_t)j * pc.nx + i);
    const float4 p = __ldg(e), q = __ldg(e + 1);
    if (q.w != 0.f) return walk_home_grid(g, X, Y, Z, max_d);
    return eval_cell(p, q, __fsub_rn(X, __ldg(pc.xs + i)), __fsub_rn(Y, __ldg(pc.ys + j)), Z, max_d);
}

typedef CUresult (*TensorMapEncodeTiledFn)(CUtensorMap*, CUtensorMapDataType, cuuint32_t, void*, const cuuint64_t*,
                                           const cuuint64_t*, const cuuint32_t*, const cuuint32_t*,
                                           CUtensorMapInterleave, CUtensorMapSwizzle, CUtensorMapL2promotion,
                                           CUtensorMapFloatOOBfill);

inline int encode_cells_tensor_map(CUtensorMap* tmap, const RoverPlaneCells* cells, int win, const char* who) {
    static TensorMapEncodeTiledFn encode = nullptr;
    if (encode == nullptr) {
        void* fn = nullptr;
        cudaDriverEntryPointQueryResult qres;
        ROVER_CUDA(cudaGetDriverEntryPoint("cuTensorMapEncodeTiled", &fn, cudaEnableDefault, &qres));
        ROVER_CHECK(fn != nullptr && qres == cudaDriverEntryPointSuccess,
                    "%s: cuTensorMapEncodeTiled is not available in this driver", who);
        encode = reinterpret_cast<TensorMapEncodeTiledFn>(fn);
    }
    const cuuint64_t gdim[2] = {(cuuint64_t)cells->nx * 8ull, (cuuint64_t)cells->ny};
    const cuuint64_t gstride[1] = {(cuuint64_t)cells->nx * 32ull};
    const cuuint32_t box[2] = {(cuuint32_t)win * 8u, (cuuint32_t)win};
    const cuuint32_t estride[2] = {1u, 1u};
    const CUresult rc = encode(tmap, CU_TENSOR_MAP_DATA_TYPE_FLOAT32, 2, const_cast<float*>(cells->entries), gdim, gstride,
                               box, estride, CU_TENSOR_MAP_INTERLEAVE_NONE, CU_TENSOR_MAP_SWIZZLE_NONE,
                               CU_TENSOR_MAP_L2_PROMOTION_L2_128B, CU_TENSOR_MAP_FLOAT_OOB_FILL_NONE);
    ROVER_CHECK(rc == CUDA_SUCCESS, "%s: cuTensorMapEncodeTiled failed (%d)", who, (int)rc);
    return 0;
}

inline int encode_planar_tensor_map(CUtensorMap* tmap, const RoverPlaneCells* cells, int win_cols, int win_rows,
                                    const char* who) {
    static TensorMapEncodeTiledFn encode = nullptr;
    if (encode == nullptr) {
        void* fn = nullptr;
        cudaDriverEntryPointQueryResult qres;
        ROVER_CUDA(cudaGetDriverEntryPoint("cuTensorMapEncodeTiled", &fn, cudaEnableDefault, &qres));
        ROVER_CHECK(fn != nullptr && qres == cudaDriverEntryPointSuccess,
                    "%s: cuTensorMapEncodeTiled is not available in this driver", who);
        encode = reinterpret_cast<TensorMapEncodeTiledFn>(fn);
    }
    ROVER_CHECK((reinterpret_cast<uintptr_t>(cells->entries_planar) & 15) == 0, "%s: entries_planar not 16B aligned", who);
    const cuuint64_t gdim[3] = {(cuuint64_t)cells->nx * 4ull, (cuuint64_t)cells->ny, 2ull};
    const cuuint64_t gstride[2] = {(cuuint64_t)cells->nx * 16ull, (cuuint64_t)cells->nx * 16ull * (cuuint64_t)cells->ny};
    const cuuint32_t box[3] = {(cuuint32_t)win_cols * 4u, (cuuint32_t)win_rows, 2u};
    const cuuint32_t estride[3] = {1u, 1u, 1u};
    const CUresult rc = encode(tmap, CU_TENSOR_MAP_DATA_TYPE_FLOAT32, 3, const_cast<float*>(cells->entries_planar), gdim,
                               gstride, box, estride, CU_TENSOR_MAP_INTERLEAVE_NONE, CU_TENSOR_MAP_SWIZZLE_NONE,
                               CU_TENSOR_MAP_L2_PROMOTION_L2_128B, CU_TENSOR_MAP_FLOAT_OOB_FILL_NONE);
    ROVER_CHECK(rc == CUDA_SUCCESS, "%s: cuTensorMapEncodeTiled (planar) failed (%d)", who, (int)rc);
    return 0;
}

}
```

isaac_rover_orbit_b200/ops.py:

```python
from __future__ import annotations

import ctypes as C
from dataclasses import dataclass

import numpy as np
import torch

from . import _lib, torch_ops
from .config import RoverEnvCfg
from .plane_cells import PlaneCells, build_plane_cells, build_plane_cells_torch
from .scan_grid import ScanGrid, build_scan_grid


class ScanGridHandle:

    def __init__(self, grid: ScanGrid | None, device, cells: PlaneCells | None = None, mesh=None):
        self.device = torch.device(device)
        if self.device.type != "cuda":
            raise RuntimeError("ScanGridHandle needs a CUDA device; there is no CPU fallback")
        self._mesh = mesh
        self._home_grid_built = grid is not None
        if grid is None:
            if cells is None or cells.n_general != 0 or mesh is None:
                raise RuntimeError("ScanGridHandle: a deferred home grid needs the mesh and a table without general cells")
            grid = build_scan_grid(np.zeros((0, 3), np.float32), np.zeros((0, 3), np.int64))
        self.grid = grid
        self.cells = cells
        self.cells_struct = None
        if cells is not None:
            self.cells_xs = cells.xs.to(self.device).contiguous()
            self.cells_ys = cells.ys.to(self.device).contiguous()
            self.cells_entries = cells.entries.to(self.device).contiguous()
            self.cells_planar = self.cells_entries.view(cells.ny, cells.nx, 2, 4).permute(2, 0, 1, 3).contiguous()
            self.cells_struct = _lib.PlaneCells(self.cells_xs.data_ptr(), self.cells_ys.data_ptr(),
                                                self.cells_entries.data_ptr(), cells.nx, cells.ny, cells.inv_dx,
                                                cells.inv_dy, self.cells_planar.data_ptr())
        self.struct = _lib.ScanGrid()
        self._upload_home_grid(grid)
        self.desc = torch_ops.descriptor(self.struct)
        self.cells_desc = torch_ops.descriptor(self.cells_struct) if self.cells_struct is not None else None
        torch.cuda.current_stream(self.device).synchronize()

    def _upload_home_grid(self, grid: ScanGrid) -> None:
        self.grid = grid
        self.cell_start = grid.cell_start.to(self.device).contiguous()
        self.records = grid.records.to(self.device).contiguous()
        if grid.n_records == 0:
            self.records = torch.zeros(1, 12, device=self.device)
        s = self.struct
        s.n_levels = len(grid.levels)
        s.span = grid.span
        for i, lv in enumerate(grid.levels):
            s.level[i] = _lib.ScanLevel(lv.ox, lv.oy, lv.cell, lv.inv_cell, lv.ncx, lv.ncy, lv.start_offset, 0)
        s.cell_start = self.cell_start.data_ptr()
        s.records = self.records.data_ptr()
        s.n_records = grid.n_records

    @property
    def has_home_grid(self) -> bool:
        return self._home_grid_built

    def ensure_home_grid(self) -> None:
        if not self._home_grid_built:
            v, f = self._mesh
            self._upload_home_grid(build_scan_grid(v, f))
            self._home_grid_built = True

    @classmethod
    def from_mesh(cls, vertices, faces, device, cell_size=None, plane_cells: bool = True,
                  home_grid: bool | None = None) -> "ScanGridHandle":
        v = vertices.detach().cpu().numpy() if isinstance(vertices, torch.Tensor) else np.asarray(vertices)
        f = faces.detach().cpu().numpy() if isinstance(faces, torch.Tensor) else np.asarray(faces)
        if plane_cells and cell_size is None and not home_grid:
            cells = build_plane_cells_torch(v, f, device)
            if cells is None:
                cells = build_plane_cells(v, f)
            if cells.lattice and cells.n_general == 0:
                return cls(None, device, cells, mesh=(v, f))
        grid = build_scan_grid(v, f, cell_size=cell_size)
        cells = build_plane_cells(v, f, fallback_cell=grid.levels[0].cell) if plane_cells else None
        handle = cls(grid, device, cells)
        return handle

    def nbytes(self) -> int:
        return self.grid.nbytes() + (self.cells.nbytes() if self.cells is not None else 0)


def grid_pattern(resolution: float = 0.1, size=(3.0, 3.0), offset_pos=(0.0, 0.0, 10.0)) -> torch.Tensor:
    x = torch.arange(start=-size[0] / 2, end=size[0] / 2 + 1.0e-9, step=resolution)
    y = torch.arange(start=-size[1] / 2, end=size[1] / 2 + 1.0e-9, step=resolution)
    gx, gy = torch.meshgrid(x, y, indexing="xy")
    starts = torch.zeros(gx.numel(), 3, dtype=torch.float32)
    starts[:, 0] = gx.flatten()
    starts[:, 1] = gy.flatten()
    return starts + torch.tensor(offset_pos, dtype=torch.float32)


class RayPattern:

    def __init__(self, ray_starts_local: torch.Tensor, device, directions=None):
        cpu = ray_starts_local.detach().to("cpu", torch.float32).contiguous()
        if cpu.dim() != 2 or cpu.shape[1] != 3:
            raise RuntimeError(f"RayPattern: starts must be [R,3], got {list(cpu.shape)}")
        self.n_rays = cpu.shape[0]
        self.device = torch.device(device)
        self.starts = cpu.to(self.device)
        if directions is None:
            directions = (0.0, 0.0, -1.0)
        if isinstance(directions, (tuple, list)):
            d = torch.tensor(directions, dtype=torch.float64)
        else:
            d = torch.as_tensor(directions)
            if d.dtype not in (torch.float32, torch.float64):
                raise RuntimeError(f"RayPattern: directions must be fp32 or fp64, got {d.dtype}")
        d = d.detach().to("cpu", torch.float32)
        if d.shape == (3,):
            d = d.expand(self.n_rays, 3)
        if d.shape != (self.n_rays, 3):
            raise RuntimeError(f"RayPattern: directions must be [R,3] or [3] for R = {self.n_rays}, got {list(d.shape)}")
        d = d.contiguous()
        self.vertical_down = bool(((d[:, 0] == 0) & (d[:, 1] == 0) & (d[:, 2] == -1)).all())
        self.dirs = d.to(self.device)
        if self.n_rays:
            self.box = (C.c_float * 4)(float(cpu[:, 0].min()), float(cpu[:, 0].max()), float(cpu[:, 1].min()),
                                       float(cpu[:, 1].max()))
        else:
            self.box = (C.c_float * 4)(0.0, 0.0, 0.0, 0.0)
        self.box_t = torch.frombuffer(self.box, dtype=torch.float32)

    @classmethod
    def grid(cls, device, resolution: float = 0.1, size=(3.0, 3.0), offset_pos=(0.0, 0.0, 10.0),
             direction=(0.0, 0.0, -1.0), offset_rot=(1.0, 0.0, 0.0, 0.0)) -> "RayPattern":
        starts = grid_pattern(resolution, size, offset_pos)
        n = starts.shape[0]
        dirs = torch.tensor(direction, dtype=torch.float32).expand(n, 3)
        dirs = quat_apply(torch.tensor(offset_rot, dtype=torch.float32).expand(n, 4), dirs)
        return cls(starts, device, directions=dirs)


def quat_apply(quat: torch.Tensor, vec: torch.Tensor) -> torch.Tensor:
    xyz = quat[..., 1:]
    t = xyz.cross(vec, dim=-1) * 2
    return vec + quat[..., 0:1] * t + xyz.cross(t, dim=-1)


def require_vertical(what: str, rays: "RayPattern", attach_yaw_only: bool = True, takes_variant: bool = False) -> None:
    if not attach_yaw_only or not rays.vertical_down:
        hint = " or pass variant=6" if takes_variant else ""
        raise RuntimeError(f"{what}: only vertical rays (direction (0, 0, -1), attach_yaw_only=True) are supported; this "
                           f"pattern has attach_yaw_only={bool(attach_yaw_only)}, vertical_down={rays.vertical_down}: use "
                           f"height_scan(..., attach_yaw_only=...){hint}")


DEFAULT_SCAN_VARIANT = 5
RAY_CAST_VARIANT = 6


def height_scan(pos_w: torch.Tensor, quat_w: torch.Tensor, rays, grid: ScanGridHandle,
                max_distance: float = 100.0, base_offset: float = 0.26878, out: torch.Tensor | None = None,
                return_hits: bool = False, variant: int | None = None, attach_yaw_only: bool = True):
    if not isinstance(rays, RayPattern):
        rays = RayPattern(rays, pos_w.device)
    ray_starts_local = rays.starts
    general = not attach_yaw_only or not rays.vertical_down
    if variant is None:
        variant = RAY_CAST_VARIANT if general else DEFAULT_SCAN_VARIANT
    if variant == RAY_CAST_VARIANT:
        return _ray_cast(pos_w, quat_w, rays, grid, max_distance, base_offset, out, return_hits, attach_yaw_only)
    if general:
        raise RuntimeError(f"height_scan: variant {variant} casts vertical yaw-only rays only; this configuration "
                           f"(attach_yaw_only={bool(attach_yaw_only)}, vertical_down={rays.vertical_down}) needs variant 6")
    if variant == 0:
        grid.ensure_home_grid()
    dev = _lib.require_cuda(pos_w, quat_w, ray_starts_local)
    n, r = pos_w.shape[0], ray_starts_local.shape[0]
    if pos_w.dtype != torch.float32 or quat_w.dtype != torch.float32 or ray_starts_local.dtype != torch.float32:
        raise RuntimeError("height_scan: fp32 tensors required")
    if pos_w.shape != (n, 3) or quat_w.shape != (n, 4) or ray_starts_local.shape != (r, 3):
        raise RuntimeError("height_scan: bad shapes")
    if grid.device != dev:
        raise RuntimeError("height_scan: grid lives on another device")
    if variant in (2, 4, 5) and grid.cells_struct is None:
        raise RuntimeError("height_scan: variants 2, 4, 5 need a ScanGridHandle built with plane_cells=True")
    args = (pos_w, quat_w, ray_starts_local, rays.box_t, grid.desc, grid.cells_desc, float(max_distance),
            float(base_offset), int(variant))
    if return_hits:
        if out is not None:
            raise RuntimeError("height_scan: return_hits allocates its outputs (out= is not supported with it)")
        return torch.ops.rover_b200.height_scan_hits(*args)
# ... 427 lines not shown
```

isaac_rover_orbit_b200/plane_cells.py:

```python
from __future__ import annotations

from dataclasses import dataclass

import numpy as np
import torch

ENTRY_FLOATS = 8
MAX_PAIR_CELLS = 64_000_000


@dataclass
class PlaneCells:
    xs: torch.Tensor
    ys: torch.Tensor
    entries: torch.Tensor
    inv_dx: float
    inv_dy: float
    n_general: int = 0
    n_empty: int = 0
    lattice: bool = False

    @property
    def nx(self) -> int:
        return int(self.xs.numel() - 1)

    @property
    def ny(self) -> int:
        return int(self.ys.numel() - 1)

    def nbytes(self) -> int:
        return self.entries.numel() * 4 + self.xs.numel() * 4 + self.ys.numel() * 4


def _lattice_lines(coord: np.ndarray, n_vertices: int):
    u = np.unique(coord)
    if 2 <= len(u) <= 4 * int(np.sqrt(n_vertices)) + 16:
        return u.astype(np.float32)
    return None


def _uniform_lines(lo: float, hi: float, cell: float) -> np.ndarray:
    n = max(int(np.ceil((hi - lo) / cell)), 1)
    lines = (np.float64(lo) + np.arange(n + 1, dtype=np.float64) * (np.float64(hi) - np.float64(lo)) / n)
    lines = lines.astype(np.float32)
    lines[0], lines[-1] = np.float32(lo), np.float32(hi)
    return np.unique(lines)


def _edge_fn(p, q):
    A = -(q[..., 1] - p[..., 1])
    B = q[..., 0] - p[..., 0]
    C = -(A * p[..., 0] + B * p[..., 1])
    return A, B, C


def _tri_overlaps_open_cell(tri, x0, x1, y0, y1):
    tx, ty = tri[..., 0], tri[..., 1]
    ok = (tx.max(-1) > x0) & (tx.min(-1) < x1) & (ty.max(-1) > y0) & (ty.min(-1) < y1)
    for k in range(3):
        A, B, C = _edge_fn(tri[..., k, :], tri[..., (k + 1) % 3, :])
        m = np.maximum(np.maximum(A * x0 + B * y0, A * x1 + B * y0), np.maximum(A * x0 + B * y1, A * x1 + B * y1)) + C
        ok &= m > 0
    return ok


def build_plane_cells(vertices, faces, fallback_cell: float = 0.2) -> PlaneCells:
    v = np.ascontiguousarray(np.asarray(vertices, dtype=np.float32).reshape(-1, 3))
    f = np.ascontiguousarray(np.asarray(faces).astype(np.int64).reshape(-1, 3))
    if len(f) == 0 or len(v) == 0:
        z = torch.zeros
        ent = z(1, 1, ENTRY_FLOATS)
        ent[..., 2] = -float("inf")
        return PlaneCells(torch.tensor([0.0, 1.0]), torch.tensor([0.0, 1.0]), ent, 1.0, 1.0, 0, 1, False)
    tri = v[f].astype(np.float64)
    e1 = tri[:, 1, :2] - tri[:, 0, :2]
    e2 = tri[:, 2, :2] - tri[:, 0, :2]
    area2 = e1[:, 0] * e2[:, 1] - e1[:, 1] * e2[:, 0]
    keep = (area2 != 0.0) & np.isfinite(tri).all(axis=(1, 2))
    flip = area2 < 0.0
    tri[flip] = tri[flip][:, [0, 2, 1], :]
    tri = tri[keep]
    used = np.unique(f[keep])
    xs = _lattice_lines(v[used, 0], len(used)) if len(used) else None
    ys = _lattice_lines(v[used, 1], len(used)) if len(used) else None
    lattice = xs is not None and ys is not None
    if not lattice:
        lo = tri[:, :, :2].min(axis=(0, 1)) if len(tri) else np.zeros(2)
        hi = tri[:, :, :2].max(axis=(0, 1)) if len(tri) else np.ones(2)
        xs = _uniform_lines(lo[0], max(hi[0], lo[0] + fallback_cell), fallback_cell)
        ys = _uniform_lines(lo[1], max(hi[1], lo[1] + fallback_cell), fallback_cell)
    nx, ny = len(xs) - 1, len(ys) - 1
    xs64, ys64 = xs.astype(np.float64), ys.astype(np.float64)

    bx0, bx1 = tri[:, :, 0].min(1), tri[:, :, 0].max(1)
    by0, by1 = tri[:, :, 1].min(1), tri[:, :, 1].max(1)
    i0 = np.clip(np.searchsorted(xs64, bx0, side="right") - 1, 0, nx - 1)
    i1 = np.clip(np.searchsorted(xs64, bx1, side="left") - 1, 0, nx - 1)
    j0 = np.clip(np.searchsorted(ys64, by0, side="right") - 1, 0, ny - 1)
    j1 = np.clip(np.searchsorted(ys64, by1, side="left") - 1, 0, ny - 1)
    wi, wj = i1 - i0 + 1, j1 - j0 + 1
    npairs = int((wi * wj).sum())
    if npairs > MAX_PAIR_CELLS:
        raise RuntimeError(f"plane-cell build: {npairs} (triangle, cell) pairs; use a coarser fallback_cell")
    t_idx = np.repeat(np.arange(len(tri)), wi * wj)
    start = np.cumsum(wi * wj) - wi * wj
    local = np.arange(npairs) - np.repeat(start, wi * wj)
    wi_r = np.repeat(wi, wi * wj)
    ci = np.repeat(i0, wi * wj) + local % wi_r
    cj = np.repeat(j0, wi * wj) + local // wi_r
    ov = _tri_overlaps_open_cell(tri[t_idx], xs64[ci], xs64[ci + 1], ys64[cj], ys64[cj + 1])
    t_idx, ci, cj = t_idx[ov], ci[ov], cj[ov]
    cell_id = cj * nx + ci
    order = np.argsort(cell_id, kind="stable")
    cell_id, t_idx = cell_id[order], t_idx[order]
    count = np.bincount(cell_id, minlength=nx * ny)
    first = np.cumsum(count) - count

    ent = np.zeros((ny * nx, ENTRY_FLOATS), dtype=np.float64)
    ent[:, 2] = -np.inf
    ent[:, 6] = 1.0
    general = count > 2
    cx0 = np.tile(xs64[:-1], ny)
    cy0 = np.repeat(ys64[:-1], nx)
    cx1 = np.tile(xs64[1:], ny)
    cy1 = np.repeat(ys64[1:], nx)

    def plane(t, ox, oy):
        p = t.copy()
        p[:, :, 0] -= ox[:, None]
        p[:, :, 1] -= oy[:, None]
        u, w = p[:, 1] - p[:, 0], p[:, 2] - p[:, 0]
        nxn = u[:, 1] * w[:, 2] - u[:, 2] * w[:, 1]
        nyn = u[:, 2] * w[:, 0] - u[:, 0] * w[:, 2]
        nzn = u[:, 0] * w[:, 1] - u[:, 1] * w[:, 0]
        a, b = -nxn / nzn, -nyn / nzn
        return a, b, p[:, 0, 2] - a * p[:, 0, 0] - b * p[:, 0, 1], p

    def corners_inside(A, B, C, x0, y0, x1, y1):
        return ((A * x0 + B * y0 + C >= 0) & (A * x1 + B * y0 + C >= 0) & (A * x0 + B * y1 + C >= 0) &
                (A * x1 + B * y1 + C >= 0))

    one = np.nonzero(count == 1)[0]
    if len(one):
        t = tri[t_idx[first[one]]]
        a, b, c, p = plane(t, cx0[one], cy0[one])
        w_, h_ = cx1[one] - cx0[one], cy1[one] - cy0[one]
        inside = np.ones(len(one), dtype=bool)
        for k in range(3):
            A, B, C = _edge_fn(p[:, k, :2], p[:, (k + 1) % 3, :2])
            inside &= corners_inside(A, B, C, 0.0, 0.0, w_, h_)
        ent[one[inside], 0], ent[one[inside], 1], ent[one[inside], 2] = a[inside], b[inside], c[inside]
        general[one[~inside]] = True

    two = np.nonzero(count == 2)[0]
    if len(two):
        t1, t2 = tri[t_idx[first[two]]], tri[t_idx[first[two] + 1]]
        a1, b1, c1, p1 = plane(t1, cx0[two], cy0[two])
        a2, b2, c2, p2 = plane(t2, cx0[two], cy0[two])
        w_, h_ = cx1[two] - cx0[two], cy1[two] - cy0[two]
        good = np.zeros(len(two), dtype=bool)
        As, Bs, Cs = np.zeros(len(two)), np.zeros(len(two)), np.ones(len(two))
        for k in range(3):
            pa, pb = p1[:, k], p1[:, (k + 1) % 3]
            for m in range(3):
                qa, qb = p2[:, m], p2[:, (m + 1) % 3]
                shared = (pa == qb).all(-1) & (pb == qa).all(-1)
                if not shared.any():
                    continue
                ok = shared & ~good
                A, B, C = _edge_fn(pa[:, :2], pb[:, :2])
                for kk in (1, 2):
                    Ae, Be, Ce = _edge_fn(p1[:, (k + kk) % 3, :2], p1[:, (k + kk + 1) % 3, :2])
                    ok &= corners_inside(Ae, Be, Ce, 0.0, 0.0, w_, h_)
                for mm in (1, 2):
                    Ae, Be, Ce = _edge_fn(p2[:, (m + mm) % 3, :2], p2[:, (m + mm + 1) % 3, :2])
                    ok &= corners_inside(Ae, Be, Ce, 0.0, 0.0, w_, h_)
                As[ok], Bs[ok], Cs[ok] = A[ok], B[ok], C[ok]
                good |= ok
        with np.errstate(divide="ignore", invalid="ignore"):
            kx = np.where(np.abs(As) >= np.abs(Bs), (a2 - a1) / As, (b2 - b1) / Bs)
        good &= np.isfinite(kx)
        resid = np.abs(a1 + kx * As - a2) + np.abs(b1 + kx * Bs - b2) + np.abs(c1 + kx * Cs - c2)
        good &= resid <= 1e-9 * (1.0 + np.abs(a2) + np.abs(b2) + np.abs(c2))
        g = two[good]
        ent[g, 0], ent[g, 1], ent[g, 2], ent[g, 3] = a1[good], b1[good], c1[good], kx[good]
        ent[g, 4], ent[g, 5], ent[g, 6] = As[good], Bs[good], Cs[good]
        general[two[~good]] = True

    ent[general, 7] = 1.0
    ent[general, 2] = -np.inf
    span_x, span_y = float(xs64[-1] - xs64[0]), float(ys64[-1] - ys64[0])
    return PlaneCells(torch.from_numpy(xs.copy()), torch.from_numpy(ys.copy()),
                      torch.from_numpy(ent.astype(np.float32).reshape(ny, nx, ENTRY_FLOATS)),
                      nx / span_x, ny / span_y, int(general.sum()), int((count == 0).sum()), bool(lattice))


def _t_edge_fn(p, q):
    A = -(q[..., 1] - p[..., 1])
    B = q[..., 0] - p[..., 0]
    C = -(A * p[..., 0] + B * p[..., 1])
    return A, B, C


def _t_overlaps_open_cell(tri, x0, x1, y0, y1):
    tx, ty = tri[..., 0], tri[..., 1]
    ok = (tx.max(-1).values > x0) & (tx.min(-1).values < x1) & (ty.max(-1).values > y0) & (ty.min(-1).values < y1)
    mx = torch.maximum
    for k in range(3):
        A, B, C = _t_edge_fn(tri[..., k, :], tri[..., (k + 1) % 3, :])
        m = mx(mx(A * x0 + B * y0, A * x1 + B * y0), mx(A * x0 + B * y1, A * x1 + B * y1)) + C
        ok &= m > 0
    return ok


def _t_lattice_lines(coord: torch.Tensor, n_vertices: int):
    u = torch.unique(coord)
    if 2 <= u.numel() <= 4 * int(np.sqrt(n_vertices)) + 16:
        return u.to(torch.float32)
    return None


def build_plane_cells_torch(vertices, faces, device) -> PlaneCells | None:
    dev = torch.device(device)
    v = torch.as_tensor(np.ascontiguousarray(np.asarray(vertices, dtype=np.float32).reshape(-1, 3))).to(dev)
    f = torch.as_tensor(np.ascontiguousarray(np.asarray(faces).astype(np.int64).reshape(-1, 3))).to(dev)
    if f.numel() == 0 or v.numel() == 0:
        return None
    tri = v[f].to(torch.float64)
    e1 = tri[:, 1, :2] - tri[:, 0, :2]
    e2 = tri[:, 2, :2] - tri[:, 0, :2]
    area2 = e1[:, 0] * e2[:, 1] - e1[:, 1] * e2[:, 0]
    keep = (area2 != 0.0) & torch.isfinite(tri).all(dim=2).all(dim=1)
    flip = area2 < 0.0
    tri[flip] = tri[flip][:, [0, 2, 1], :]
    tri = tri[keep]
    used = torch.unique(f[keep])
    if used.numel() == 0:
        return None
    xs = _t_lattice_lines(v[used, 0], used.numel())
    ys = _t_lattice_lines(v[used, 1], used.numel())
    if xs is None or ys is None:
        return None
    nx, ny = xs.numel() - 1, ys.numel() - 1
    xs64, ys64 = xs.to(torch.float64), ys.to(torch.float64)

    bx0, bx1 = tri[:, :, 0].min(1).values, tri[:, :, 0].max(1).values
    by0, by1 = tri[:, :, 1].min(1).values, tri[:, :, 1].max(1).values
    ss = torch.searchsorted
    i0 = torch.clamp(ss(xs64, bx0.contiguous(), right=True) - 1, 0, nx - 1)
    i1 = torch.clamp(ss(xs64, bx1.contiguous(), right=False) - 1, 0, nx - 1)
    j0 = torch.clamp(ss(ys64, by0.contiguous(), right=True) - 1, 0, ny - 1)
    j1 = torch.clamp(ss(ys64, by1.contiguous(), right=False) - 1, 0, ny - 1)
    wi, wj = i1 - i0 + 1, j1 - j0 + 1
    per = wi * wj
    npairs = int(per.sum())
    if npairs > MAX_PAIR_CELLS:
        raise RuntimeError(f"plane-cell build: {npairs} (triangle, cell) pairs; use a coarser fallback_cell")
    rep = torch.repeat_interleave
    t_idx = rep(torch.arange(tri.shape[0], device=dev), per)
    start = torch.cumsum(per, 0) - per
    local = torch.arange(npairs, device=dev) - rep(start, per)
    wi_r = rep(wi, per)
    ci = rep(i0, per) + local % wi_r
    cj = rep(j0, per) + torch.div(local, wi_r, rounding_mode="floor")
    ov = _t_overlaps_open_cell(tri[t_idx], xs64[ci], xs64[ci + 1], ys64[cj], ys64[cj + 1])
    t_idx, ci, cj = t_idx[ov], ci[ov], cj[ov]
    cell_id = cj * nx + ci
    order = torch.sort(cell_id, stable=True).indices
    cell_id, t_idx = cell_id[order], t_idx[order]
    count = torch.bincount(cell_id, minlength=nx * ny)
    first = torch.cumsum(count, 0) - count

    ent = torch.zeros(ny * nx, ENTRY_FLOATS, dtype=torch.float64, device=dev)
    ent[:, 2] = -float("inf")
    ent[:, 6] = 1.0
    general = count > 2
    cx0 = xs64[:-1].repeat(ny)
    cy0 = rep(ys64[:-1], nx)
    cx1 = xs64[1:].repeat(ny)
    cy1 = rep(ys64[1:], nx)

    def plane(t, ox, oy):
        p = t.clone()
        p[:, :, 0] -= ox[:, None]
        p[:, :, 1] -= oy[:, None]
        u, w = p[:, 1] - p[:, 0], p[:, 2] - p[:, 0]
        nxn = u[:, 1] * w[:, 2] - u[:, 2] * w[:, 1]
        nyn = u[:, 2] * w[:, 0] - u[:, 0] * w[:, 2]
        nzn = u[:, 0] * w[:, 1] - u[:, 1] * w[:, 0]
        a, b = -nxn / nzn, -nyn / nzn
        return a, b, p[:, 0, 2] - a * p[:, 0, 0] - b * p[:, 0, 1], p

    def corners_inside(A, B, C, x0, y0, x1, y1):
        return ((A * x0 + B * y0 + C >= 0) & (A * x1 + B * y0 + C >= 0) & (A * x0 + B * y1 + C >= 0) &
                (A * x1 + B * y1 + C >= 0))

    one = torch.nonzero(count == 1).squeeze(-1)
    if one.numel():
        t = tri[t_idx[first[one]]]
        a, b, c, p = plane(t, cx0[one], cy0[one])
        w_, h_ = cx1[one] - cx0[one], cy1[one] - cy0[one]
        inside = torch.ones(one.numel(), dtype=torch.bool, device=dev)
        for k in range(3):
            A, B, C = _t_edge_fn(p[:, k, :2], p[:, (k + 1) % 3, :2])
            inside &= corners_inside(A, B, C, 0.0, 0.0, w_, h_)
        sel = one[inside]
        ent[sel, 0], ent[sel, 1], ent[sel, 2] = a[inside], b[inside], c[inside]
        general[one[~inside]] = True

    two = torch.nonzero(count == 2).squeeze(-1)
    if two.numel():
        t1, t2 = tri[t_idx[first[two]]], tri[t_idx[first[two] + 1]]
        a1, b1, c1, p1 = plane(t1, cx0[two], cy0[two])
        a2, b2, c2, p2 = plane(t2, cx0[two], cy0[two])
        w_, h_ = cx1[two] - cx0[two], cy1[two] - cy0[two]
        good = torch.zeros(two.numel(), dtype=torch.bool, device=dev)
        As = torch.zeros(two.numel(), dtype=torch.float64, device=dev)
        Bs = torch.zeros_like(As)
        Cs = torch.ones_like(As)
        for k in range(3):
            pa, pb = p1[:, k], p1[:, (k + 1) % 3]
            for m in range(3):
                qa, qb = p2[:, m], p2[:, (m + 1) % 3]
                shared = (pa == qb).all(-1) & (pb == qa).all(-1)
                if not bool(shared.any()):
                    continue
                ok = shared & ~good
                A, B, C = _t_edge_fn(pa[:, :2], pb[:, :2])
                for kk in (1, 2):
                    Ae, Be, Ce = _t_edge_fn(p1[:, (k + kk) % 3, :2], p1[:, (k + kk + 1) % 3, :2])
                    ok &= corners_inside(Ae, Be, Ce, 0.0, 0.0, w_, h_)
                for mm in (1, 2):
                    Ae, Be, Ce = _t_edge_fn(p2[:, (m + mm) % 3, :2], p2[:, (m + mm + 1) % 3, :2])
                    ok &= corners_inside(Ae, Be, Ce, 0.0, 0.0, w_, h_)
                As[ok], Bs[ok], Cs[ok] = A[ok], B[ok], C[ok]
                good |= ok
        kx = torch.where(As.abs() >= Bs.abs(), (a2 - a1) / As, (b2 - b1) / Bs)
        good &= torch.isfinite(kx)
        resid = (a1 + kx * As - a2).abs() + (b1 + kx * Bs - b2).abs() + (c1 + kx * Cs - c2).abs()
        good &= resid <= 1e-9 * (1.0 + a2.abs() + b2.abs() + c2.abs())
        g = two[good]
        ent[g, 0], ent[g, 1], ent[g, 2], ent[g, 3] = a1[good], b1[good], c1[good], kx[good]
        ent[g, 4], ent[g, 5], ent[g, 6] = As[good], Bs[good], Cs[good]
        general[two[~good]] = True

    ent[general, 7] = 1.0
    ent[general, 2] = -float("inf")
    span_x, span_y = float(xs64[-1] - xs64[0]), float(ys64[-1] - ys64[0])
    return PlaneCells(xs.clone(), ys.clone(), ent.to(torch.float32).reshape(ny, nx, ENTRY_FLOATS), nx / span_x, ny / span_y,
                      int(general.sum()), int((count == 0).sum()), True)
```

Before: 172.8 billion.

## Stage only four floats per plane cell and rebuild edge terms from grid lines

The TMA-staged cell window now carries only the first four entry floats per cell instead of the full planar two-half copy. The edge coefficients (A, B, C) are reconstructed on the fly from the cell widths and heights stored in shared memory, using a per-mesh sign convention (edge_form) detected on the host. Cells that do not match that convention are marked with NaN and fall back to the full table. This halves the bytes moved per stage, at the cost of extra arithmetic per ray and a fallback path for odd cells.

```diff
diff --git a/include/rover_b200.h b/include/rover_b200.h
--- a/include/rover_b200.h
+++ b/include/rover_b200.h
@@ -42,6 +42,9 @@
     int32_t nx, ny;
     float inv_dx, inv_dy;
     const float* entries_planar;
+    const float* cells_p;
+    int32_t edge_form;
+    int32_t reserved;
 } RoverPlaneCells;
 
 int rover_height_scan(const float* pos_w, const float* quat_w, int32_t n_envs, const float* ray_starts_local,
diff --git a/isaac_rover_orbit_b200/_lib.py b/isaac_rover_orbit_b200/_lib.py
--- a/isaac_rover_orbit_b200/_lib.py
+++ b/isaac_rover_orbit_b200/_lib.py
@@ -40,7 +40,8 @@
 
 class PlaneCells(C.Structure):
     _fields_ = [("xs", C.c_void_p), ("ys", C.c_void_p), ("entries", C.c_void_p), ("nx", C.c_int32), ("ny", C.c_int32),
-                ("inv_dx", C.c_float), ("inv_dy", C.c_float), ("entries_planar", C.c_void_p)]
+                ("inv_dx", C.c_float), ("inv_dy", C.c_float), ("entries_planar", C.c_void_p),
+                ("cells_p", C.c_void_p), ("edge_form", C.c_int32), ("reserved", C.c_int32)]
 
 
 class StatsExchange(C.Structure):
diff --git a/isaac_rover_orbit_b200/csrc/fused_scan_policy.cu b/isaac_rover_orbit_b200/csrc/fused_scan_policy.cu
--- a/isaac_rover_orbit_b200/csrc/fused_scan_policy.cu
+++ b/isaac_rover_orbit_b200/csrc/fused_scan_policy.cu
@@ -60,7 +60,7 @@
 struct __align__(128) FuSmem {
     PairStage stage[kFuStages];
     float vx[kPairMaxRays], vy[kPairMaxRays];
-    LinePair2 xpair[kPairMaxLines], ypair[kPairMaxLines];
+    LineLoW xpair[kPairMaxLines + 1], ypair[kPairMaxLines + 1];
     unsigned char obs[2][kFuObsBytes];
     unsigned char act[kFuActBytes];
     unsigned char w1[kFuW1Bytes + kFuW1Slack];
@@ -152,7 +152,7 @@
         producer_window(cur, pc, pattern_radius);
         if (lane < n_iter && lane < kFuStages) {
             bar_arrive_expect_tx(&sm.full_bar[lane], kPairStageBytes);
-            tma_load_window_planar(sm.stage[lane].p, &tmap, cur.ic0, cur.jr0, &sm.full_bar[lane]);
+            tma_load_window_p(sm.stage[lane], &tmap, cur.ic0, cur.jr0, &sm.full_bar[lane]);
         }
         producer_frame(cur);
     } else if (warp == 1) {
@@ -180,7 +180,7 @@
     } else if (warp >= 4) {
         constexpr int kFill = 32 * (kFuWarps - 4);
         constexpr int kPatLoads = (2 * kPairMaxRays + kFill - 1) / kFill;
-        constexpr int kLineLoads = (kPairMaxLines + kFill - 1) / kFill;
+        constexpr int kLineLoads = (kPairMaxLines + 1 + kFill - 1) / kFill;
         const int ct = threadIdx.x - 128;
         float* pat_flat = sm.vx;
         float pat[kPatLoads], xl[kLineLoads], xh[kLineLoads], yl[kLineLoads], yh[kLineLoads];
@@ -193,11 +193,11 @@
 #pragma unroll
         for (int k = 0; k < kLineLoads; ++k) {
             const int i = ct + k * kFill;
-            const bool okx = lines_in_smem && i < pc.nx, oky = lines_in_smem && i < pc.ny;
+            const bool okx = lines_in_smem && i <= pc.nx, oky = lines_in_smem && i <= pc.ny;
             xl[k] = okx ? __ldg(pc.xs + i) : 0.f;
-            xh[k] = okx ? __ldg(pc.xs + i + 1) : 0.f;
+            xh[k] = okx && i < pc.nx ? __ldg(pc.xs + i + 1) : xl[k];
             yl[k] = oky ? __ldg(pc.ys + i) : 0.f;
-            yh[k] = oky ? __ldg(pc.ys + i + 1) : 0.f;
+            yh[k] = oky && i < pc.ny ? __ldg(pc.ys + i + 1) : yl[k];
         }
 #pragma unroll
         for (int k = 0; k < kPatLoads; ++k) {
@@ -207,8 +207,8 @@
 #pragma unroll
         for (int k = 0; k < kLineLoads; ++k) {
             const int i = ct + k * kFill;
-            if (lines_in_smem && i < pc.nx) sm.xpair[i] = {xl[k], xh[k]};
-            if (lines_in_smem && i < pc.ny) sm.ypair[i] = {yl[k], yh[k]};
+            if (lines_in_smem && i <= pc.nx) sm.xpair[i] = {xl[k], __fmul_rn(edge_sign_x(pc.edge_form), __fsub_rn(xh[k], xl[k]))};
+            if (lines_in_smem && i <= pc.ny) sm.ypair[i] = {yl[k], __fmul_rn(edge_sign_y(pc.edge_form), __fsub_rn(yh[k], yl[k]))};
         }
         uint4* z = reinterpret_cast<uint4*>(&sm.obs[0][0]);
         for (int i = ct; i < 2 * kFuObsBytes / 16; i += kFill) z[i] = make_uint4(0u, 0u, 0u, 0u);
@@ -243,7 +243,7 @@
                             bar_wait(&sm.empty_bar[s], ((uint32_t)(it / kFuStages) & 1u) ^ 1u);
                             if (cur.ok) {
                                 bar_arrive_expect_tx(full, kPairStageBytes);
-                                tma_load_window_planar(st.p, &tmap, cur.ic0, cur.jr0, full);
+                                tma_load_window_p(st, &tmap, cur.ic0, cur.jr0, full);
                             } else {
                                 bar_arrive(full);
                             }
@@ -307,7 +307,7 @@
             if (h.mode == 1) {
                 const float sz2 = __fmul_rn(h.sz, 2.f);
                 const PairCtx cx = make_pair_ctx(h, sm, st, smem_raw, pc.inv_dx, pc.inv_dy, base_offset, max_d, sm.vz0,
-                                                 n_envs >> 31);
+                                                 n_envs >> 31, pc.edge_form);
                 constexpr int kSink = kWriteObs ? kSinkOperandAndGlobal : kSinkOperand;
                 for (int b0 = r_begin; b0 < r_end; b0 += kPairBatch) {
                     const int r = b0 + lane;
@@ -334,7 +334,7 @@
                             const float X = __fadd_rn(__fadd_rn(__fadd_rn(vx, __fmul_rn(h.cw, tx)), -__fmul_rn(h.sz, ty)), h.px);
                             const float Y = __fadd_rn(__fadd_rn(__fadd_rn(vy, __fmul_rn(h.cw, ty)), __fmul_rn(h.sz, tx)), h.py);
                             float hh;
-                            pair_resolve_deferred_ray(&sm, &st, g, pc.inv_dx, pc.inv_dy, X, Y, __fadd_rn(sm.vz0, h.pz), h.pz,
+                            pair_resolve_deferred_ray(&sm, &st, g, pc, X, Y, __fadd_rn(sm.vz0, h.pz), h.pz,
                                                       max_d, base_offset, &hh, nullptr);
                             operand_store(operand_row, rr, hh);
                             if (kWriteObs) out_row[rr] = hh;
@@ -468,8 +468,9 @@
                 "rover_scan_encoder_fused: NULL argument");
     ROVER_CHECK(n_rays == kFuRays, "rover_scan_encoder_fused: the encoder reads a 961-ray scan (31 x 31 grid), got %d rays", n_rays);
     ROVER_CHECK(obs_stride >= kOperandHead + kFuRays, "rover_scan_encoder_fused: obs_stride %d < 965", obs_stride);
-    ROVER_CHECK(cells->xs && cells->ys && cells->entries && cells->entries_planar && cells->nx > 0 && cells->ny > 0,
-                "rover_scan_encoder_fused: needs the plane-cell table with its planar copy");
+    ROVER_CHECK(cells->xs && cells->ys && cells->entries && cells->cells_p && cells->nx > 0 &&
+                    cells->ny > 0,
+                "rover_scan_encoder_fused: needs the plane-cell table with its staging plane");
     ROVER_CHECK((reinterpret_cast<uintptr_t>(packed_fused) & 15) == 0, "rover_scan_encoder_fused: packed image not 16B aligned");
     static int n_sms = 0;
     if (n_sms == 0) {
@@ -492,9 +493,9 @@
     g.cell_start = grid->cell_start;
     g.rec = reinterpret_cast<const float4*>(grid->records);
     alignas(64) CUtensorMap tmap;
-    if (const int rc = encode_planar_tensor_map(&tmap, cells, kPairPitch, kPairWin, "rover_scan_encoder_fused")) return rc;
+    if (const int rc = encode_stage_tensor_map(&tmap, cells, kPairPitch, kPairWin, "rover_scan_encoder_fused")) return rc;
     PlaneCellsDev pc{cells->xs, cells->ys, reinterpret_cast<const float4*>(cells->entries), cells->nx, cells->ny,
-                     cells->inv_dx, cells->inv_dy};
+                     cells->inv_dx, cells->inv_dy, cells->edge_form};
     const float rx = fmaxf(fabsf(pattern_box[0]), fabsf(pattern_box[1])), ry = fmaxf(fabsf(pattern_box[2]), fabsf(pattern_box[3]));
     const float radius = sqrtf(rx * rx + ry * ry) * 1.0001f + 1.0e-3f;
     const int grid_dim = n_envs < n_sms ? n_envs : n_sms;
diff --git a/isaac_rover_orbit_b200/csrc/height_scan.cu b/isaac_rover_orbit_b200/csrc/height_scan.cu
--- a/isaac_rover_orbit_b200/csrc/height_scan.cu
+++ b/isaac_rover_orbit_b200/csrc/height_scan.cu
@@ -311,7 +311,7 @@
                 "rover_height_scan_obs: row strides %d / %d < head_cols + n_rays = %d", obs_stride, bf16_stride,
                 head_cols + n_rays);
     cudaStream_t s = static_cast<cudaStream_t>(stream);
-    const bool fused = cells != nullptr && cells->entries_planar != nullptr && n_rays >= 1 && n_rays <= 1024 &&
+    const bool fused = cells != nullptr && cells->cells_p != nullptr && n_rays >= 1 && n_rays <= 1024 &&
                        head_cols <= 32 && pattern_box != nullptr;
     if (fused) {
         ROVER_CHECK(pos_w && quat_w && ray_starts_local, "rover_height_scan_obs: NULL tensor");
diff --git a/isaac_rover_orbit_b200/csrc/height_scan_paired.cu b/isaac_rover_orbit_b200/csrc/height_scan_paired.cu
--- a/isaac_rover_orbit_b200/csrc/height_scan_paired.cu
+++ b/isaac_rover_orbit_b200/csrc/height_scan_paired.cu
@@ -14,8 +14,7 @@
 height_scan_paired_kernel(const float* __restrict__ pos_w, const float* __restrict__ quat_w, int n_envs,
                           const float* __restrict__ ray_local, int n_rays, const __grid_constant__ ScanGridDev g,
                           const __grid_constant__ PlaneCellsDev pc, const __grid_constant__ CUtensorMap tmap,
-                          float pattern_radius, float max_d, float base_offset, float* __restrict__ out,
-                          int out_stride, __nv_bfloat16* __restrict__ obs_bf16, int bf16_stride, int head_cols) {
+                          float pattern_radius, float max_d, float base_offset, float* __restrict__ out, int out_stride, __nv_bfloat16* __restrict__ obs_bf16, int bf16_stride, int head_cols) {
     extern __shared__ __align__(128) unsigned char smem_raw[];
     PairSmem& sm = *reinterpret_cast<PairSmem*>(smem_raw);
     const int warp = threadIdx.x >> 5, lane = threadIdx.x & 31;
@@ -47,7 +46,7 @@
         producer_window(cur, pc, pattern_radius);
         if (lane < n_iter && lane < kPairEarly && ROVER_SCAN_DBG != 4) {
             bar_arrive_expect_tx(&sm.full_bar[lane], kPairStageBytes);
-            tma_load_window_planar(sm.stage[lane].p, &tmap, cur.ic0, cur.jr0, &sm.full_bar[lane]);
+            tma_load_window_p(sm.stage[lane], &tmap, cur.ic0, cur.jr0, &sm.full_bar[lane]);
             DBG_STAMP_ANY(16 + lane);
         }
         producer_frame(cur);
@@ -55,7 +54,7 @@
     } else {
         constexpr int kFill = 32 * kPairConsumerWarps;
         constexpr int kPatLoads = (3 * kPairMaxRays + kFill - 1) / kFill;
-        constexpr int kLineLoads = (kPairMaxLines + kFill - 1) / kFill;
+        constexpr int kLineLoads = (kPairMaxLines + 1 + kFill - 1) / kFill;
         const int ct = threadIdx.x - 32;
         static_assert(offsetof(PairSmem, vy) == offsetof(PairSmem, vx) + 4 * kPairMaxRays &&
                           offsetof(PairSmem, vz) == offsetof(PairSmem, vx) + 8 * kPairMaxRays,
@@ -73,11 +72,11 @@
 #pragma unroll
         for (int k = 0; k < kLineLoads; ++k) {
             const int i = ct + k * kFill;
-            const bool okx = lines_in_smem && i < pc.nx, oky = lines_in_smem && i < pc.ny;
+            const bool okx = lines_in_smem && i <= pc.nx, oky = lines_in_smem && i <= pc.ny;
             xl[k] = okx ? __ldg(pc.xs + i) : 0.f;
-            xh[k] = okx ? __ldg(pc.xs + i + 1) : 0.f;
+            xh[k] = okx && i < pc.nx ? __ldg(pc.xs + i + 1) : xl[k];
             yl[k] = oky ? __ldg(pc.ys + i) : 0.f;
-            yh[k] = oky ? __ldg(pc.ys + i + 1) : 0.f;
+            yh[k] = oky && i < pc.ny ? __ldg(pc.ys + i + 1) : yl[k];
         }
 #pragma unroll
         for (int k = 0; k < kPatLoads; ++k) {
@@ -87,8 +86,8 @@
 #pragma unroll
         for (int k = 0; k < kLineLoads; ++k) {
             const int i = ct + k * kFill;
-            if (lines_in_smem && i < pc.nx) sm.xpair[i] = {xl[k], xh[k]};
-            if (lines_in_smem && i < pc.ny) sm.ypair[i] = {yl[k], yh[k]};
+            if (lines_in_smem && i <= pc.nx) sm.xpair[i] = {xl[k], __fmul_rn(edge_sign_x(pc.edge_form), __fsub_rn(xh[k], xl[k]))};
+            if (lines_in_smem && i <= pc.ny) sm.ypair[i] = {yl[k], __fmul_rn(edge_sign_y(pc.edge_form), __fsub_rn(yh[k], yl[k]))};
         }
     }
     if (warp == 1) DBG_STAMP(3);
@@ -117,7 +116,7 @@
                         bar_wait(&sm.empty_bar[s], ((uint32_t)(it / kPairStages) & 1u) ^ 1u);
                         if (cur.ok && ROVER_SCAN_DBG != 2) {
                             bar_arrive_expect_tx(full, kPairStageBytes);
-                            tma_load_window_planar(st.p, &tmap, cur.ic0, cur.jr0, full);
+                            tma_load_window_p(st, &tmap, cur.ic0, cur.jr0, full);
                         } else {
                             bar_arrive(full);
                         }
@@ -128,7 +127,7 @@
 #if ROVER_PAIR_CTX_FROM_PRODUCER
                     if (cur.ok)
                         st.ctx = make_pair_ctx(st.hdr, sm, st, smem_raw, pc.inv_dx, pc.inv_dy, base_offset, max_d, sm.vz[0],
-                                               n_envs >> 31);
+                                               n_envs >> 31, pc.edge_form);
 #endif
                     bar_arrive(full);
                 }
@@ -178,7 +177,7 @@
                 const PairCtx cx = st.ctx;
 #else
                 const PairCtx cx = make_pair_ctx(h, sm, st, smem_raw, pc.inv_dx, pc.inv_dy, base_offset, max_d, sm.vz[0],
-                                                 n_envs >> 31);
+                                                 n_envs >> 31, pc.edge_form);
 #endif
                 const float sz2 = __fmul_rn(h.sz, 2.f);
                 for (int b0 = r_begin; b0 < r_end; b0 += kPairBatch) {
@@ -204,7 +203,7 @@
                             const float tx = -__fmul_rn(sz2, vy), ty = __fmul_rn(sz2, vx);
                             const float X = __fadd_rn(__fadd_rn(__fadd_rn(vx, __fmul_rn(h.cw, tx)), -__fmul_rn(h.sz, ty)), h.px);
                             const float Y = __fadd_rn(__fadd_rn(__fadd_rn(vy, __fmul_rn(h.cw, ty)), __fmul_rn(h.sz, tx)), h.py);
-                            pair_resolve_deferred_ray(&sm, &st, g, pc.inv_dx, pc.inv_dy, X, Y, __fadd_rn(sm.vz[sl], h.pz),
+                            pair_resolve_deferred_ray(&sm, &st, g, pc, X, Y, __fadd_rn(sm.vz[sl], h.pz),
                                                       h.pz, max_d, base_offset, kBf16 == 2 ? nullptr : out_row + rr,
                                                       kBf16 ? bf_row + rr : nullptr);
                         }
@@ -243,12 +242,12 @@
                               const ScanGridDev& g, const RoverPlaneCells* cells, float4 pattern_box, float max_d,
                               float base_offset, float* out, int out_stride, float* hits, uint16_t* obs_bf16,
                               int bf16_stride, int head_cols, cudaStream_t stream, bool bf16_only) {
-    if (obs_bf16 == nullptr && (hits != nullptr || cells->entries_planar == nullptr))
+    if (obs_bf16 == nullptr && (hits != nullptr || cells->cells_p == nullptr))
         return launch_height_scan_pipelined(pos_w, quat_w, n_envs, ray_local, n_rays, g, cells, pattern_box, max_d,
                                             base_offset, out, out_stride, hits, stream);
     ROVER_CHECK(n_rays >= 1 && n_rays <= kPairMaxRays, "height_scan_paired: pattern of %d rays (1..%d supported)", n_rays,
                 kPairMaxRays);
-    ROVER_CHECK(cells->entries_planar != nullptr && hits == nullptr, "height_scan_paired: bf16 mirror needs the planar table");
+    ROVER_CHECK(cells->cells_p != nullptr && hits == nullptr, "height_scan_paired: bf16 mirror needs the staging plane");
     ROVER_CHECK(head_cols >= 0 && head_cols <= 32, "height_scan_paired: head_cols %d out of range", head_cols);
     static int n_sms = 0;
     static bool configured = false;
@@ -265,9 +264,9 @@
         configured = true;
     }
     alignas(64) CUtensorMap tmap;
-    if (const int rc = encode_planar_tensor_map(&tmap, cells, kPairPitch, kPairWin, "height_scan_paired")) return rc;
+    if (const int rc = encode_stage_tensor_map(&tmap, cells, kPairPitch, kPairWin, "height_scan_paired")) return rc;
     PlaneCellsDev pc{cells->xs, cells->ys, reinterpret_cast<const float4*>(cells->entries), cells->nx, cells->ny,
-                     cells->inv_dx, cells->inv_dy};
+                     cells->inv_dx, cells->inv_dy, cells->edge_form};
     const float rx = fmaxf(fabsf(pattern_box.x), fabsf(pattern_box.y)), ry = fmaxf(fabsf(pattern_box.z), fabsf(pattern_box.w));
     const float radius = sqrtf(rx * rx + ry * ry) * 1.0001f + 1.0e-3f;
     const int grid = n_envs < n_sms ? n_envs : n_sms;
diff --git a/isaac_rover_orbit_b200/csrc/height_scan_step.cu b/isaac_rover_orbit_b200/csrc/height_scan_step.cu
--- a/isaac_rover_orbit_b200/csrc/height_scan_step.cu
+++ b/isaac_rover_orbit_b200/csrc/height_scan_step.cu
@@ -13,7 +13,7 @@
 struct StepSmem {
     PairStage stage[kPairStages];
     float vx[kPairMaxRays], vy[kPairMaxRays], vz[kPairMaxRays];
-    LinePair2 xpair[kPairMaxLines], ypair[kPairMaxLines];
+    LineLoW xpair[kPairMaxLines + 1], ypair[kPairMaxLines + 1];
     unsigned long long full_bar[kPairFullBars];
     unsigned long long empty_bar[kPairStages];
     unsigned long long pose_full[kStepMdpWarps], pose_empty[kStepMdpWarps];
@@ -76,7 +76,7 @@
     } else {
         constexpr int kFill = 32 * kStepWorkerWarps;
         constexpr int kPatLoads = (3 * kPairMaxRays + kFill - 1) / kFill;
-        constexpr int kLineLoads = (kPairMaxLines + kFill - 1) / kFill;
+        constexpr int kLineLoads = (kPairMaxLines + 1 + kFill - 1) / kFill;
         const int ct = threadIdx.x - 32;
         float* pat_flat = sm.vx;
         float pat[kPatLoads], xl[kLineLoads], xh[kLineLoads], yl[kLineLoads], yh[kLineLoads];
@@ -91,11 +91,11 @@
 #pragma unroll
         for (int k = 0; k < kLineLoads; ++k) {
             const int i = ct + k * kFill;
-            const bool okx = lines_in_smem && i < pc.nx, oky = lines_in_smem && i < pc.ny;
+            const bool okx = lines_in_smem && i <= pc.nx, oky = lines_in_smem && i <= pc.ny;
             xl[k] = okx ? __ldg(pc.xs + i) : 0.f;
-            xh[k] = okx ? __ldg(pc.xs + i + 1) : 0.f;
+            xh[k] = okx && i < pc.nx ? __ldg(pc.xs + i + 1) : xl[k];
             yl[k] = oky ? __ldg(pc.ys + i) : 0.f;
-            yh[k] = oky ? __ldg(pc.ys + i + 1) : 0.f;
+            yh[k] = oky && i < pc.ny ? __ldg(pc.ys + i + 1) : yl[k];
         }
 #pragma unroll
         for (int k = 0; k < kPatLoads; ++k) {
@@ -105,8 +105,8 @@
 #pragma unroll
         for (int k = 0; k < kLineLoads; ++k) {
             const int i = ct + k * kFill;
-            if (lines_in_smem && i < pc.nx) sm.xpair[i] = {xl[k], xh[k]};
-            if (lines_in_smem && i < pc.ny) sm.ypair[i] = {yl[k], yh[k]};
+            if (lines_in_smem && i <= pc.nx) sm.xpair[i] = {xl[k], __fmul_rn(edge_sign_x(pc.edge_form), __fsub_rn(xh[k], xl[k]))};
+            if (lines_in_smem && i <= pc.ny) sm.ypair[i] = {yl[k], __fmul_rn(edge_sign_y(pc.edge_form), __fsub_rn(yh[k], yl[k]))};
         }
     }
     const bool flat_z = __syncthreads_and(my_flat_z) != 0;
@@ -140,7 +140,7 @@
                     if (it >= kPairStages) bar_wait(&sm.empty_bar[s], ((uint32_t)(it / kPairStages) & 1u) ^ 1u);
                     if (cur.ok) {
                         bar_arrive_expect_tx(full, kPairStageBytes);
-                        tma_load_window_planar(st.p, &tmap, cur.ic0, cur.jr0, full);
+                        tma_load_window_p(st, &tmap, cur.ic0, cur.jr0, full);
                     } else {
                         bar_arrive(full);
                     }
@@ -286,7 +286,7 @@
             if (h.mode == 1) {
                 const float sz2 = __fmul_rn(h.sz, 2.f);
                 const PairCtx cx = make_pair_ctx(h, sm, st, smem_raw, pc.inv_dx, pc.inv_dy, base_offset, max_d, sm.vz[0],
-                                                 n_envs >> 31);
+                                                 n_envs >> 31, pc.edge_form);
                 for (int b0 = r_begin; b0 < r_end; b0 += kPairBatch) {
                     const int r = b0 + lane;
                     float* __restrict__ o = out_row + r;
@@ -307,7 +307,7 @@
                             const float tx = -__fmul_rn(sz2, vy), ty = __fmul_rn(sz2, vx);
                             const float X0 = __fadd_rn(__fadd_rn(__fadd_rn(vx, __fmul_rn(h.cw, tx)), -__fmul_rn(h.sz, ty)), h.px);
                             const float Y0 = __fadd_rn(__fadd_rn(__fadd_rn(vy, __fmul_rn(h.cw, ty)), __fmul_rn(h.sz, tx)), h.py);
-                            pair_resolve_deferred_ray(&sm, &st, g, pc.inv_dx, pc.inv_dy, X0, Y0, __fadd_rn(sm.vz[sl], h.pz), h.pz,
+                            pair_resolve_deferred_ray(&sm, &st, g, pc, X0, Y0, __fadd_rn(sm.vz[sl], h.pz), h.pz,
                                                       max_d, base_offset, out_row + rr, nullptr);
                         }
                     }
@@ -350,8 +350,9 @@
     ROVER_CHECK((reinterpret_cast<uintptr_t>(root_quat_w) & 15) == 0, "rover_step_fused: root_quat_w not 16B aligned");
     ROVER_CHECK(n_rays >= 1 && n_rays <= kPairMaxRays, "rover_step_fused: pattern of %d rays (1..%d supported)", n_rays, kPairMaxRays);
     ROVER_CHECK(obs_stride >= 4 + n_rays, "rover_step_fused: obs_stride %d < 4 + n_rays", obs_stride);
-    ROVER_CHECK(cells->xs && cells->ys && cells->entries && cells->entries_planar && cells->nx > 0 && cells->ny > 0,
-                "rover_step_fused: needs the plane-cell table with its planar copy");
+    ROVER_CHECK(cells->xs && cells->ys && cells->entries && cells->cells_p && cells->nx > 0 &&
+                    cells->ny > 0,
+                "rover_step_fused: needs the plane-cell table with its staging plane");
     ROVER_CHECK(state->action && state->prev_action && state->pos_cmd_w && state->heading_cmd_w && state->pos_cmd_b &&
                     state->heading_cmd_b && state->time_left && state->command_counter && state->episode_length_buf &&
                     state->episode_sums && state->env_origins && state->err_pos && state->err_heading,
@@ -382,9 +383,9 @@
     ScanGridDev g;
     if (int rc = make_dev_grid(grid, g)) return rc;
     alignas(64) CUtensorMap tmap;
-    if (const int rc = encode_planar_tensor_map(&tmap, cells, kPairPitch, kPairWin, "rover_step_fused")) return rc;
+    if (const int rc = encode_stage_tensor_map(&tmap, cells, kPairPitch, kPairWin, "rover_step_fused")) return rc;
     PlaneCellsDev pc{cells->xs, cells->ys, reinterpret_cast<const float4*>(cells->entries), cells->nx, cells->ny,
-                     cells->inv_dx, cells->inv_dy};
+                     cells->inv_dx, cells->inv_dy, cells->edge_form};
     const float rx = fmaxf(fabsf(pattern_box[0]), fabsf(pattern_box[1])), ry = fmaxf(fabsf(pattern_box[2]), fabsf(pattern_box[3]));
     const float radius = sqrtf(rx * rx + ry * ry) * 1.0001f + 1.0e-3f;
     unsigned int* counter = reinterpret_cast<unsigned int*>(scratch + scratch_floats - 1);
diff --git a/isaac_rover_orbit_b200/csrc/scan_common.cuh b/isaac_rover_orbit_b200/csrc/scan_common.cuh
--- a/isaac_rover_orbit_b200/csrc/scan_common.cuh
+++ b/isaac_rover_orbit_b200/csrc/scan_common.cuh
@@ -24,6 +24,7 @@
     const float4* __restrict__ ent;
     int nx, ny;
     float inv_dx, inv_dy;
+    int edge_form;
 };
 
 struct SensorFrame {
diff --git a/isaac_rover_orbit_b200/csrc/scan_paired.cuh b/isaac_rover_orbit_b200/csrc/scan_paired.cuh
--- a/isaac_rover_orbit_b200/csrc/scan_paired.cuh
+++ b/isaac_rover_orbit_b200/csrc/scan_paired.cuh
@@ -50,7 +50,7 @@
 constexpr int kPairWin = 26;
 constexpr int kPairPitch = 27;
 constexpr int kPairPlane = kPairWin * kPairPitch;
-constexpr uint32_t kPairStageBytes = 2u * kPairPlane * 16u;
+constexpr uint32_t kPairStageBytes = kPairPlane * 16u;
 #ifndef ROVER_PAIR_CHUNK
 #define ROVER_PAIR_CHUNK 256
 #endif
@@ -62,6 +62,16 @@
 constexpr float kFloorMagic = 12582912.0f;
 constexpr int kFloorMagicBits = 0x4B400000;
 
+__host__ __device__ __forceinline__ float edge_sign_y(int form) { return (form & 1) ? -1.f : 1.f; }
+__host__ __device__ __forceinline__ float edge_sign_x(int form) { return (form & 2) ? -1.f : 1.f; }
+__host__ __device__ __forceinline__ float edge_c_factor(int form) {
+    return (form & 4) ? ((form & 1) ? 1.f : -1.f) : 0.f;
+}
+
+struct LineLoW {
+    float lo, w;
+};
+
 __host__ __device__ __forceinline__ int ray_of_slot(int s) {
     const int j = s & 127;
     return (s & ~127) + 64 * (j & 1) + 32 * (j >> 6) + ((j & 63) >> 1);
@@ -85,22 +95,20 @@
     float pz, max_d;
     uint32_t xoff, yoff, eoff;
     uint32_t cmax, rmax;
-    uint32_t pad;
+    float cf;
 };
 static_assert(sizeof(PairCtx) == 160, "PairCtx is loaded as ten 16-byte words");
 
 struct __align__(128) PairStage {
     float4 p[kPairPlane];
-    float4 q[kPairPlane];
     PairHeader hdr;
     PairCtx ctx;
 };
-static_assert(offsetof(PairStage, q) == kPairPlane * 16, "planes must be contiguous: one 3-D TMA box fills both");
 
 struct PairSmem {
     PairStage stage[kPairStages];
     float vx[kPairMaxRays], vy[kPairMaxRays], vz[kPairMaxRays];
-    LinePair2 xpair[kPairMaxLines], ypair[kPairMaxLines];
+    LineLoW xpair[kPairMaxLines + 1], ypair[kPairMaxLines + 1];
     unsigned long long full_bar[kPairFullBars];
     unsigned long long empty_bar[kPairStages];
     int next_chunk;
@@ -120,12 +128,12 @@
     *reinterpret_cast<__nv_bfloat16*>(row + (k >> 3) * kOperandLbo + (k & 7) * 2) = v;
 }
 
-__device__ __forceinline__ void tma_load_window_planar(void* dst, const CUtensorMap* tmap, int col, int row,
-                                                       unsigned long long* bar) {
+__device__ __forceinline__ void tma_load_window_p(PairStage& st, const CUtensorMap* tmap, int col, int row,
+                                                  unsigned long long* bar) {
     asm volatile(
-        "cp.async.bulk.tensor.3d.shared::cluster.global.tile.mbarrier::complete_tx::bytes [%0], [%1, {%2, %3, %4}], [%5];" ::
-            "r"(s_addr(dst)),
-        "l"(reinterpret_cast<uint64_t>(tmap)), "r"(col * 4), "r"(row), "r"(0), "r"(s_addr(bar))
+        "cp.async.bulk.tensor.2d.shared::cluster.global.tile.mbarrier::complete_tx::bytes [%0], [%1, {%2, %3}], [%4];" ::
+            "r"(s_addr(st.p)),
+        "l"(reinterpret_cast<uint64_t>(tmap)), "r"(col * 4), "r"(row), "r"(s_addr(bar))
         : "memory");
 }
 
@@ -170,7 +178,7 @@
 template <class SM>
 __device__ __forceinline__ PairCtx make_pair_ctx(const PairHeader& h, const SM& sm, const PairStage& st,
                                                  const unsigned char* smem_base, float inv_dx, float inv_dy, float base_offset,
-                                                 float max_d, float vz0, int opaque_zero) {
+                                                 float max_d, float vz0, int opaque_zero, int edge_form) {
     PairCtx cx;
     const float sz2 = __fmul_rn(h.sz, 2.f);
     const float wx0 = sm.xpair[h.ic0].lo, wy0 = sm.ypair[h.jr0].lo;
@@ -185,31 +193,31 @@
     cx.xoff = (uint32_t)(reinterpret_cast<const unsigned char*>(sm.xpair + h.ic0) - smem_base);
     cx.yoff = (uint32_t)(reinterpret_cast<const unsigned char*>(sm.ypair + h.jr0) - smem_base);
     cx.eoff = (uint32_t)(reinterpret_cast<const unsigned char*>(st.p) - smem_base);
-    cx.pad = 0u;
+    cx.cf = edge_c_factor(edge_form);
     return cx;
 }
 
 template <class SM>
 static __device__ __noinline__ void pair_resolve_deferred_ray(const SM* sm, const PairStage* st, const ScanGridDev& g,
-                                                              float inv_dx, float inv_dy, float X, float Y, float Z, float pz,
+                                                              const PlaneCellsDev& pc, float X, float Y, float Z, float pz,
                                                               float max_d, float base_offset, float* __restrict__ out,
                                                               __nv_bfloat16* __restrict__ out_bf) {
     const PairHeader& h = st->hdr;
     const int cmax = h.ncols - 1, rmax = h.nrows - 1;
-    const LinePair2* xp = sm->xpair + h.ic0;
-    const LinePair2* yp = sm->ypair + h.jr0;
-    const float wx0 = xp[0].lo, wy0 = yp[0].lo, wx1 = xp[cmax].hi, wy1 = yp[rmax].hi;
+    const LineLoW* xp = sm->xpair + h.ic0;
+    const LineLoW* yp = sm->ypair + h.jr0;
+    const float wx0 = xp[0].lo, wy0 = yp[0].lo, wx1 = xp[cmax + 1].lo, wy1 = yp[rmax + 1].lo;
     float zhit = -INFINITY;
     if (X >= wx0 && X <= wx1 && Y >= wy0 && Y <= wy1) {
-        int ci = min(max(__float2int_rd((X - wx0) * inv_dx), 0), cmax);
-        int cj = min(max(__float2int_rd((Y - wy0) * inv_dy), 0), rmax);
+        int ci = min(max(__float2int_rd((X - wx0) * pc.inv_dx), 0), cmax);
+        int cj = min(max(__float2int_rd((Y - wy0) * pc.inv_dy), 0), rmax);
         while (ci > 0 && X < xp[ci].lo) --ci;
-        while (ci < cmax && X >= xp[ci].hi) ++ci;
+        while (ci < cmax && X >= xp[ci + 1].lo) ++ci;
         while (cj > 0 && Y < yp[cj].lo) --cj;
-        while (cj < rmax && Y >= yp[cj].hi) ++cj;
-        const int e = cj * kPairPitch + ci;
-        const float4 q = st->q[e];
-        zhit = (q.w == 0.f) ? eval_cell(st->p[e], q, __fsub_rn(X, xp[ci].lo), __fsub_rn(Y, yp[cj].lo), Z, max_d)
+        while (cj < rmax && Y >= yp[cj + 1].lo) ++cj;
+        const float4* ent = pc.ent + 2 * ((size_t)(h.jr0 + cj) * pc.nx + (h.ic0 + ci));
+        const float4 q = __ldg(ent + 1);
+        zhit = (q.w == 0.f) ? eval_cell(__ldg(ent), q, __fsub_rn(X, xp[ci].lo), __fsub_rn(Y, yp[cj].lo), Z, max_d)
                             : walk_home_grid(g, X, Y, Z, max_d);
     }
     float height;
@@ -266,18 +274,14 @@
         const float2 xp = *reinterpret_cast<const float2*>(smem + (c.xoff + bi * 8u));
         const float2 yp = *reinterpret_cast<const float2*>(smem + (c.yoff + bj * 8u));
 #if ROVER_SCAN_DBG == 5
-        const uint32_t e = c.eoff + ((threadIdx.x & 31) * 16u) + ((bj + bi) & 1u) * 1024u;
-        const float4 q = *reinterpret_cast<const float4*>(smem + e + 512);
-        const float4 p = *reinterpret_cast<const float4*>(smem + e);
-        const bool fast = (x >= xp.x) & (x < xp.y) & (y >= yp.x) & (y < yp.y);
+        const float4 p = *reinterpret_cast<const float4*>(smem + c.eoff + ((threadIdx.x & 31) * 16u) + ((bj + bi) & 1u) * 1024u);
 #else
-        const uint32_t e = c.eoff + bj * (uint32_t)(kPairPitch * 16) + bi * 16u;
-        const float4 q = *reinterpret_cast<const float4*>(smem + e + kPairPlane * 16);
-        const float4 p = *reinterpret_cast<const float4*>(smem + e);
-        const bool fast = (x >= xp.x) & (x < xp.y) & (y >= yp.x) & (y < yp.y) & (q.w == 0.f);
+        const float4 p = *reinterpret_cast<const float4*>(smem + c.eoff + bj * (uint32_t)(kPairPitch * 16) + bi * 16u);
 #endif
         const float lx = __fsub_rn(x, xp.x), ly = __fsub_rn(y, yp.x);
-        const float E = fmaf(q.x, lx, fmaf(q.y, ly, q.z));
+        const bool fast = (lx >= 0.f) & (lx < fabsf(xp.y)) & (ly >= 0.f) & (ly < fabsf(yp.y)) & (p.w == p.w);
+        const float A = yp.y, B = xp.y, C = __fmul_rn(__fmul_rn(A, B), c.cf);
+        const float E = fmaf(A, lx, fmaf(B, ly, C));
         nz[k] = fmaf(-p.w, fminf(E, 0.f), -fmaf(p.x, lx, fmaf(p.y, ly, p.z)));
         const bool valid = k ? valid1 : valid0;
         keep[k] = valid && fast;
@@ -341,12 +345,12 @@
                                                  float radius, bool lines_in_smem) {
     bool ok = lines_in_smem && (e.ncols <= kPairWin) && (e.nrows <= kPairWin);
     if (ok) {
-        const float gx_lo = sm.xpair[0].lo, gx_hi = sm.xpair[pc.nx - 1].hi;
-        const float gy_lo = sm.ypair[0].lo, gy_hi = sm.ypair[pc.ny - 1].hi;
+        const float gx_lo = sm.xpair[0].lo, gx_hi = sm.xpair[pc.nx].lo;
+        const float gy_lo = sm.ypair[0].lo, gy_hi = sm.ypair[pc.ny].lo;
         ok = (sm.xpair[e.ic0].lo <= fmaxf(e.px - radius, gx_lo)) &&
-             (sm.xpair[e.ic0 + e.ncols - 1].hi >= fminf(e.px + radius, gx_hi)) &&
+             (sm.xpair[e.ic0 + e.ncols].lo >= fminf(e.px + radius, gx_hi)) &&
              (sm.ypair[e.jr0].lo <= fmaxf(e.py - radius, gy_lo)) &&
-             (sm.ypair[e.jr0 + e.nrows - 1].hi >= fminf(e.py + radius, gy_hi));
+             (sm.ypair[e.jr0 + e.nrows].lo >= fminf(e.py + radius, gy_hi));
     }
     e.ok = ok;
 }
diff --git a/isaac_rover_orbit_b200/csrc/scan_pipe.cuh b/isaac_rover_orbit_b200/csrc/scan_pipe.cuh
--- a/isaac_rover_orbit_b200/csrc/scan_pipe.cuh
+++ b/isaac_rover_orbit_b200/csrc/scan_pipe.cuh
@@ -141,8 +141,8 @@
     return 0;
 }
 
-inline int encode_planar_tensor_map(CUtensorMap* tmap, const RoverPlaneCells* cells, int win_cols, int win_rows,
-                                    const char* who) {
+inline int encode_stage_tensor_map(CUtensorMap* tmap, const RoverPlaneCells* cells, int win_cols, int win_rows,
+                                   const char* who) {
     static TensorMapEncodeTiledFn encode = nullptr;
     if (encode == nullptr) {
         void* fn = nullptr;
@@ -152,15 +152,15 @@
                     "%s: cuTensorMapEncodeTiled is not available in this driver", who);
         encode = reinterpret_cast<TensorMapEncodeTiledFn>(fn);
     }
-    ROVER_CHECK((reinterpret_cast<uintptr_t>(cells->entries_planar) & 15) == 0, "%s: entries_planar not 16B aligned", who);
-    const cuuint64_t gdim[3] = {(cuuint64_t)cells->nx * 4ull, (cuuint64_t)cells->ny, 2ull};
-    const cuuint64_t gstride[2] = {(cuuint64_t)cells->nx * 16ull, (cuuint64_t)cells->nx * 16ull * (cuuint64_t)cells->ny};
-    const cuuint32_t box[3] = {(cuuint32_t)win_cols * 4u, (cuuint32_t)win_rows, 2u};
-    const cuuint32_t estride[3] = {1u, 1u, 1u};
-    const CUresult rc = encode(tmap, CU_TENSOR_MAP_DATA_TYPE_FLOAT32, 3, const_cast<float*>(cells->entries_planar), gdim,
-                               gstride, box, estride, CU_TENSOR_MAP_INTERLEAVE_NONE, CU_TENSOR_MAP_SWIZZLE_NONE,
+    ROVER_CHECK((reinterpret_cast<uintptr_t>(cells->cells_p) & 15) == 0, "%s: cells_p not 16B aligned", who);
+    const cuuint64_t gdim[2] = {(cuuint64_t)cells->nx * 4ull, (cuuint64_t)cells->ny};
+    const cuuint64_t gstride[1] = {(cuuint64_t)cells->nx * 16ull};
+    const cuuint32_t box[2] = {(cuuint32_t)win_cols * 4u, (cuuint32_t)win_rows};
+    const cuuint32_t estride[2] = {1u, 1u};
+    const CUresult rc = encode(tmap, CU_TENSOR_MAP_DATA_TYPE_FLOAT32, 2, const_cast<float*>(cells->cells_p), gdim, gstride,
+                               box, estride, CU_TENSOR_MAP_INTERLEAVE_NONE, CU_TENSOR_MAP_SWIZZLE_NONE,
                                CU_TENSOR_MAP_L2_PROMOTION_L2_128B, CU_TENSOR_MAP_FLOAT_OOB_FILL_NONE);
-    ROVER_CHECK(rc == CUDA_SUCCESS, "%s: cuTensorMapEncodeTiled (planar) failed (%d)", who, (int)rc);
+    ROVER_CHECK(rc == CUDA_SUCCESS, "%s: cuTensorMapEncodeTiled (staging plane) failed (%d)", who, (int)rc);
     return 0;
 }
 
diff --git a/isaac_rover_orbit_b200/ops.py b/isaac_rover_orbit_b200/ops.py
--- a/isaac_rover_orbit_b200/ops.py
+++ b/isaac_rover_orbit_b200/ops.py
@@ -8,7 +8,7 @@
 
 from . import _lib, torch_ops
 from .config import RoverEnvCfg
-from .plane_cells import PlaneCells, build_plane_cells, build_plane_cells_torch
+from .plane_cells import PlaneCells, build_plane_cells, build_plane_cells_torch, staging_plane
 from .scan_grid import ScanGrid, build_scan_grid
 
 
@@ -31,10 +31,10 @@
             self.cells_xs = cells.xs.to(self.device).contiguous()
             self.cells_ys = cells.ys.to(self.device).contiguous()
             self.cells_entries = cells.entries.to(self.device).contiguous()
-            self.cells_planar = self.cells_entries.view(cells.ny, cells.nx, 2, 4).permute(2, 0, 1, 3).contiguous()
+            self.cells_p = staging_plane(cells).to(self.device).contiguous()
             self.cells_struct = _lib.PlaneCells(self.cells_xs.data_ptr(), self.cells_ys.data_ptr(),
                                                 self.cells_entries.data_ptr(), cells.nx, cells.ny, cells.inv_dx,
-                                                cells.inv_dy, self.cells_planar.data_ptr())
+                                                cells.inv_dy, None, self.cells_p.data_ptr(), cells.edge_form, 0)
         self.struct = _lib.ScanGrid()
         self._upload_home_grid(grid)
         self.desc = torch_ops.descriptor(self.struct)
diff --git a/isaac_rover_orbit_b200/plane_cells.py b/isaac_rover_orbit_b200/plane_cells.py
--- a/isaac_rover_orbit_b200/plane_cells.py
+++ b/isaac_rover_orbit_b200/plane_cells.py
@@ -1,5 +1,6 @@
 from __future__ import annotations
 
+import logging
 from dataclasses import dataclass
 
 import numpy as np
@@ -7,6 +8,11 @@
 
 ENTRY_FLOATS = 8
 MAX_PAIR_CELLS = 64_000_000
+
+FORM_NEG_A, FORM_NEG_B, FORM_HW = 1, 2, 4
+EDGE_FORMS = (FORM_NEG_A, FORM_NEG_B, FORM_HW, FORM_HW | FORM_NEG_A | FORM_NEG_B)
+
+_log = logging.getLogger(__name__)
 
 
 @dataclass
@@ -19,6 +25,8 @@
     n_general: int = 0
     n_empty: int = 0
     lattice: bool = False
+    edge_form: int = FORM_NEG_A
+    n_other_form: int = 0
 
     @property
     def nx(self) -> int:
@@ -30,6 +38,37 @@
 
     def nbytes(self) -> int:
         return self.entries.numel() * 4 + self.xs.numel() * 4 + self.ys.numel() * 4
+
+
+def rebuild_edge(form: int, w: torch.Tensor, h: torch.Tensor):
+    A = -h if form & FORM_NEG_A else h
+    B = -w if form & FORM_NEG_B else w
+    f = (1.0 if form & FORM_NEG_A else -1.0) if form & FORM_HW else 0.0
+    return A, B, (A * B) * f
+
+
+def _rebuilt_by(cells: PlaneCells, form: int) -> torch.Tensor:
+    ent = cells.entries
+    ny, nx = ent.shape[0], ent.shape[1]
+    w = (cells.xs[1:] - cells.xs[:-1]).view(1, nx).expand(ny, nx)
+    h = (cells.ys[1:] - cells.ys[:-1]).view(ny, 1).expand(ny, nx)
+    got = torch.stack(rebuild_edge(form, w, h), -1).contiguous().view(torch.int32)
+    return (got == ent[..., 4:7].contiguous().view(torch.int32)).all(-1) & (ent[..., 7] == 0)
+
+
+def with_edge_form(cells: PlaneCells) -> PlaneCells:
+    counts = [int(_rebuilt_by(cells, f).sum()) for f in EDGE_FORMS]
+    cells.edge_form = EDGE_FORMS[int(np.argmax(counts))]
+    cells.n_other_form = int((cells.entries[..., 7] == 0).sum()) - max(counts)
+    _log.info("plane cells: %d x %d, edge form %d, %d general cells, %d closed-form cells of another form", cells.nx,
+              cells.ny, cells.edge_form, cells.n_general, cells.n_other_form)
+    return cells
+
+
+def staging_plane(cells: PlaneCells) -> torch.Tensor:
+    p = cells.entries[..., :4].clone()
+    p[..., 3][~_rebuilt_by(cells, cells.edge_form)] = float("nan")
+    return p
 
 
 def _lattice_lines(coord: np.ndarray, n_vertices: int):
@@ -71,7 +110,7 @@
         z = torch.zeros
         ent = z(1, 1, ENTRY_FLOATS)
         ent[..., 2] = -float("inf")
-        return PlaneCells(torch.tensor([0.0, 1.0]), torch.tensor([0.0, 1.0]), ent, 1.0, 1.0, 0, 1, False)
+        return with_edge_form(PlaneCells(torch.tensor([0.0, 1.0]), torch.tensor([0.0, 1.0]), ent, 1.0, 1.0, 0, 1, False))
     tri = v[f].astype(np.float64)
     e1 = tri[:, 1, :2] - tri[:, 0, :2]
     e2 = tri[:, 2, :2] - tri[:, 0, :2]
@@ -190,9 +229,9 @@
     ent[general, 7] = 1.0
     ent[general, 2] = -np.inf
     span_x, span_y = float(xs64[-1] - xs64[0]), float(ys64[-1] - ys64[0])
-    return PlaneCells(torch.from_numpy(xs.copy()), torch.from_numpy(ys.copy()),
-                      torch.from_numpy(ent.astype(np.float32).reshape(ny, nx, ENTRY_FLOATS)),
-                      nx / span_x, ny / span_y, int(general.sum()), int((count == 0).sum()), bool(lattice))
+    return with_edge_form(PlaneCells(torch.from_numpy(xs.copy()), torch.from_numpy(ys.copy()),
+                                      torch.from_numpy(ent.astype(np.float32).reshape(ny, nx, ENTRY_FLOATS)),
+                                      nx / span_x, ny / span_y, int(general.sum()), int((count == 0).sum()), bool(lattice)))
 
 
 def _t_edge_fn(p, q):
@@ -347,5 +386,5 @@
     ent[general, 7] = 1.0
     ent[general, 2] = -float("inf")
     span_x, span_y = float(xs64[-1] - xs64[0]), float(ys64[-1] - ys64[0])
-    return PlaneCells(xs.clone(), ys.clone(), ent.to(torch.float32).reshape(ny, nx, ENTRY_FLOATS), nx / span_x, ny / span_y,
-                      int(general.sum()), int((count == 0).sum()), True)
+    return with_edge_form(PlaneCells(xs.clone(), ys.clone(), ent.to(torch.float32).reshape(ny, nx, ENTRY_FLOATS),
+                                      nx / span_x, ny / span_y, int(general.sum()), int((count == 0).sum()), True))
diff --git a/profiles/time_scan_ab.py b/profiles/time_scan_ab.py
--- /dev/null
+++ b/profiles/time_scan_ab.py
@@ -0,0 +1,91 @@
+import argparse
+import sys
+
+import numpy as np
+import torch
+
+sys.path.insert(0, ".")
+from isaac_rover_orbit_b200 import _lib
+
+ap = argparse.ArgumentParser()
+ap.add_argument("libs", nargs="+")
+ap.add_argument("--rounds", type=int, default=7)
+ap.add_argument("--sizes", default="4096,16384,65536")
+ap.add_argument("--launches", type=int, default=25)
+ap.add_argument("--check", action="store_true")
+args = ap.parse_args()
+
+handles = []
+for path in args.libs:
+    _lib._lib, _lib.LIB_PATH = None, path
+    handles.append(_lib.load())
+
+import bench
+from isaac_rover_orbit_b200 import ops, synthetic
+
+dev = torch.device("cuda:0")
+_lib._lib = handles[0]
+v, f, grid, _ = bench.build_world(None, dev, dev)
+planar = grid.cells_entries.view(grid.cells.ny, grid.cells.nx, 2, 4).permute(2, 0, 1, 3).contiguous()
+grid.cells_struct.entries_planar = planar.data_ptr()
+rays = ops.RayPattern.grid(dev)
+flush = torch.empty(256 << 20, dtype=torch.uint8, device=dev)
+print(torch.cuda.get_device_name(0), flush=True)
+
+sizes = [int(s) for s in args.sizes.split(",")]
+inputs = {}
+for n in sizes:
+    gen = torch.Generator().manual_seed(7)
+    p, q = synthetic.make_poses(n, gen, torch.from_numpy(v), bench.TERRAIN["size_m"], bench.TERRAIN["grid_res"])
+    inputs[n] = (p.to(dev), q.to(dev), torch.empty(n, 961, device=dev))
+
+if args.check:
+    for n in sizes:
+        p, q, out = inputs[n]
+        ref = None
+        for k, h in enumerate(handles):
+            _lib._lib = h
+            out.fill_(float("nan"))
+            ops.height_scan(p, q, rays, grid, out=out)
+            got = out.cpu().numpy().view(np.uint32).copy()
+            if ref is None:
+                ref = got
+            else:
+                diff = int((got != ref).sum())
+                print(f"check envs {n}: {args.libs[k]} vs {args.libs[0]}: {diff} of {ref.size} heights differ in their bits")
+
+
+def one_median(h, n):
+    _lib._lib = h
+    p, q, out = inputs[n]
+    for _ in range(3):
+        flush.fill_(1)
+        ops.height_scan(p, q, rays, grid, out=out)
+    ts = []
+    for _ in range(args.launches):
+        flush.fill_(1)
+        a, b = torch.cuda.Event(enable_timing=True), torch.cuda.Event(enable_timing=True)
+        a.record()
+        ops.height_scan(p, q, rays, grid, out=out)
+        b.record()
+        torch.cuda.synchronize()
+        ts.append(a.elapsed_time(b) * 1e3)
+    return float(np.median(ts))
+
+
+med = {(k, n): [] for k in range(len(handles)) for n in sizes}
+for r in range(args.rounds):
+    for n in sizes:
+        order = range(len(handles)) if r % 2 == 0 else reversed(range(len(handles)))
+        for k in order:
+            med[(k, n)].append(one_median(handles[k], n))
+    print(f"round {r}: " + "  ".join(f"{n}:" + "/".join(f"{med[(k, n)][-1]:.1f}" for k in range(len(handles))) for n in sizes),
+          flush=True)
+
+for n in sizes:
+    base = np.median(med[(0, n)])
+    for k in range(len(handles)):
+        m = np.array(med[(k, n)])
+        print(f"envs {n:6d} {args.libs[k]}: median of round medians {np.median(m):7.2f} us  "
+              f"min {m.min():7.2f}  max {m.max():7.2f}  spread {100 * (m.max() - m.min()) / np.median(m):4.1f} %  "
+              f"vs first {100 * (np.median(m) / base - 1):+5.1f} %")
```

New measurement: 185.8 billion, median of 6. 7.5% higher.
